# dmlc/xgboost

Hardware: AMD Instinct MI355X
Metric: boosting_rounds_per_sec (higher is better)
Workload: dtype fp32; 1 GPU; model=higgs-1m-hist, rows_per_gpu=1000000, n_features=28, max_depth=8, max_bin=256, objective=binary:logistic, parallelism=dp1, device=cuda

## Files before the change

xgboost_amd/backend/gpu.py:

```python
from __future__ import annotations

from typing import List, Optional, Sequence, Tuple

import numpy as np
import torch

from .. import collective
from ..data import QuantizedMatrix
from ..params import TrainParam
from ..splits import SplitEntry, feature_set_mask
from .cpu import GradQuantizer

LDS_MAX_GROUP_BINS = 8192
TARGET_HIST_TASKS = 2048
MIN_ROWS_PER_TASK = 1024
HIST_MAX_GROUP_FEATURES = 1024


def _check_bin_dtype(gidx: torch.Tensor) -> None:
    if gidx.dtype not in (torch.uint8, torch.int16):
        raise ValueError(
            f"GPU kernels take uint8 or 16-bit bin matrices, got "
            f"{gidx.dtype}: a feature has more than 65535 local bin ids "
            f"(lower max_bin or the category count, or train on the CPU)")
# ... 172 lines not shown
                   out: Optional[torch.Tensor] = None) -> torch.Tensor:
        k = len(segments)
        if out is not None:
            assert out.is_contiguous()
            out.zero_()
            return self._build_hist_into(qgpair, ridx, segments, out)
        out = torch.zeros((k, self.n_bins, 2), dtype=torch.int64,
                          device=self.device)
        return self._build_hist_into(qgpair, ridx, segments, out)

    def _build_hist_into(self, qgpair, ridx, segments, out):
        tasks_np = _chunk_tasks(segments, target_tasks=512)
        (tasks,) = self.stager.upload([tasks_np])
        p8, p16 = self._gidx_ptrs()
        self.lib.gbt_hist(
            p8, p16, self.qm.n_features, self.hip.ptr(qgpair),
            self.hip.ptr(ridx), self.hip.ptr(tasks), len(tasks_np),
            self.hip.ptr(out), self.n_bins,
            self.hip.ptr(self.feat_group_start),
            self.hip.ptr(self.bin_group_start), self.n_groups,
            self.max_group_bins, self.hip.ptr(self.cut_ptrs),
            self.use_shared, None, self.hip.stream())
        return out

    def allreduce_hist(self, hist: torch.Tensor) -> torch.Tensor:
        collective.allreduce_sum_(hist)
        return hist

    def _mt_grouping(self, T: int):
        cache = self.__dict__.setdefault("_mt_group_cache", {})
        if T in cache:
            return cache[T]
        budget = LDS_MAX_GROUP_BINS // T
        widths = np.diff(self.qm.cuts.ptrs)
        if int(widths.max()) > budget:
            cache[T] = None
            return None
        groups_f, groups_b, acc = [0], [0], 0
        for f, w in enumerate(widths):
            if acc > 0 and (acc + w > budget or
                            f - groups_f[-1] >= HIST_MAX_GROUP_FEATURES):
                groups_f.append(f)
                groups_b.append(int(self.qm.cuts.ptrs[f]))
                acc = 0
            acc += int(w)
        groups_f.append(len(widths))
        groups_b.append(int(self.qm.cuts.ptrs[-1]))
        dev = self.device
        out = (torch.tensor(groups_f, dtype=torch.int32, device=dev),
               torch.tensor(groups_b, dtype=torch.int32, device=dev),
               len(groups_f) - 1,
               int(np.max(np.diff(groups_b))))
        cache[T] = out
        return out

    def build_hist_nodes_mt(self, qg_mt: torch.Tensor, nids):
        T = int(qg_mt.shape[1])
        if T > 8 or not hasattr(self.lib, "gbt_hist_mt"):
            return None
        grouping = self._mt_grouping(T)
        if grouping is None:
            return None
        fg, bg, n_groups, max_gb = grouping
        segs = [self.segments[n] for n in nids]
        tasks_np = _chunk_tasks(segs, target_tasks=512)
        (tasks,) = self.stager.upload([tasks_np])
        k = len(nids)
        out = torch.zeros((T, k, self.n_bins, 2), dtype=torch.int64,
                          device=self.device)
        p8, p16 = self._gidx_ptrs()
        self.lib.gbt_hist_mt(
            p8, p16, self.qm.n_features, self.hip.ptr(qg_mt), T,
            self.hip.ptr(self.ridx), self.hip.ptr(tasks), len(tasks_np),
            self.hip.ptr(out), self.n_bins, k,
            self.hip.ptr(fg), self.hip.ptr(bg), n_groups, max_gb,
            self.hip.ptr(self.cut_ptrs), self.hip.stream())
        return out

    def evaluate_splits(self, hist: torch.Tensor, quantizer: GradQuantizer,
                        parent_sums: Sequence[Tuple[int, int]],
                        nids: Sequence[int], param: TrainParam,
                        feature_sets=None, monotone=None, cat_mask=None,
                        node_bounds=None) -> List[SplitEntry]:
        k = len(nids)
        f = self.qm.n_features
        dev = self.device
        gain = torch.empty((k, f), dtype=torch.float64, device=dev)
        bins = torch.empty((k, f), dtype=torch.int32, device=dev)
        dirs = torch.empty((k, f), dtype=torch.uint8, device=dev)
        lsum = torch.empty((k, f, 2), dtype=torch.int64, device=dev)
        parents_np = np.asarray(parent_sums, dtype=np.int64).reshape(k, 2)
        mono_np = (np.asarray(monotone, np.int8)
                   if monotone is not None else None)
        bounds_np = (np.ascontiguousarray(node_bounds, np.float64)
                     if node_bounds is not None else None)
        mask_np = feature_set_mask(feature_sets, k, f)
        wide_feats = None
        if cat_mask is not None:
            widths = np.diff(self.qm.cuts.ptrs)
            wm = np.asarray(cat_mask, bool) & (
                widths > param.max_cat_to_onehot)
            if wm.any():
                wide_feats = np.nonzero(wm)[0]
                if mask_np is None:
                    mask_np = np.ones((k, f), dtype=np.uint8)
                mask_np[:, wide_feats] = 0
        parents, mono_t, bounds_t, mask_t = self.stager.upload(
            [parents_np, mono_np, bounds_np, mask_np])
        self.lib.gbt_evaluate_masked(
            self.hip.ptr(hist), k, self.n_bins, f,
            self.hip.ptr(self.cut_ptrs), self.hip.ptr(parents), None,
            quantizer.g_scale, quantizer.h_scale,
            param.reg_lambda, param.reg_alpha, param.max_delta_step,
            param.min_child_weight, self.hip.ptr(mono_t),
            self.hip.ptr(bounds_t), f, self.hip.ptr(mask_t),
            self.hip.ptr(self.cat_feature),
            self.hip.ptr(gain), self.hip.ptr(bins), self.hip.ptr(dirs),
            self.hip.ptr(lsum), None,
            8 if f > 4096 else 0,
            self.hip.stream())
        out_best = torch.empty((k, 6), dtype=torch.int64, device=dev)
        self.lib.gbt_select_best(
            self.hip.ptr(gain), self.hip.ptr(bins), self.hip.ptr(dirs),
            self.hip.ptr(lsum), k, f, self.hip.ptr(out_best), None,
            self.hip.stream())
        host = out_best.cpu().numpy()
        sel_gain = host[:, 0].view(np.float64)
        sel_bin = host[:, 1]
        sel_dir = host[:, 2]
        sel_lsum = host[:, 3:5]
        best_f = host[:, 5]
        cuts = self.qm.cuts
        out = []
        for i, nid in enumerate(nids):
            e = SplitEntry(nid=int(nid), g_scale=quantizer.g_scale,
                           h_scale=quantizer.h_scale)
            if np.isfinite(sel_gain[i]) and sel_bin[i] >= 0:
                fidx = int(best_f[i])
                e.gain = float(sel_gain[i])
                e.feature = fidx
                e.split_bin = int(sel_bin[i])
                e.default_left = bool(sel_dir[i])
                e.left_gq = int(sel_lsum[i, 0])
                e.left_hq = int(sel_lsum[i, 1])
                e.right_gq = int(parent_sums[i][0]) - e.left_gq
                e.right_hq = int(parent_sums[i][1]) - e.left_hq
                e.is_cat = bool(cat_mask is not None and cat_mask[fidx])
                if e.is_cat:
                    e.cat_bits = np.array(
                        [e.split_bin - int(cuts.ptrs[fidx])], dtype=np.int32)
            out.append(e)
        if wide_feats is not None:
            self._host_sorted_cat(out, hist, parents_np, quantizer, param,
                                  wide_feats, feature_sets)
        return out

    def _host_sorted_cat(self, out, hist, parents_np, quantizer, param,
                         wide_feats, feature_sets) -> None:
        from ..splits import calc_gain_given_weight, calc_weight
        cuts = self.qm.cuts
        k = len(out)
        inv_g = 1.0 / quantizer.g_scale
        inv_h = 1.0 / quantizer.h_scale
        pgq_v = parents_np[:, 0].astype(np.int64)
        phq_v = parents_np[:, 1].astype(np.int64)
        pw_v = calc_weight(pgq_v * inv_g, phq_v * inv_h, param)
        pgain_v = calc_gain_given_weight(pgq_v * inv_g, phq_v * inv_h,
                                         pw_v, param)
        allowed = [None] * k
        if feature_sets is not None:
            for i, fs in enumerate(feature_sets):
                if fs is not None:
                    allowed[i] = set(int(x) for x in fs)
        mct = param.max_cat_threshold + 1
        for fi in wide_feats:
            b0, b1 = int(cuts.ptrs[fi]), int(cuts.ptrs[fi + 1])
            w = b1 - b0
            Gc = hist[:, b0:b1, 0]
            Hc = hist[:, b0:b1, 1]
            present = Hc != 0
            ratio = torch.where(
                present,
                (Gc.double() * inv_g) / (Hc.double() * inv_h
                                         + param.reg_lambda),
                torch.full_like(Gc, float("inf"), dtype=torch.float64))
            order = torch.argsort(ratio, dim=1, stable=True)
            Gs = Gc.gather(1, order)
            Hs = Hc.gather(1, order)
            cg_t = torch.cumsum(Gs, 1)
            ch_t = torch.cumsum(Hs, 1)
            npres_t = present.sum(1)
            cg = cg_t.cpu().numpy()
            ch = ch_t.cpu().numpy()
            order_h = order.cpu().numpy()
            npres = npres_t.cpu().numpy()
            featG = cg[:, -1]
            featH = ch[:, -1]
            missG = pgq_v - featG
            missH = phq_v - featH
            pos = np.arange(w)[None, :]
            limit = np.minimum(npres, mct)[:, None]
            pos_ok = pos < limit
            for missing_left in (False, True):
                gl = cg + (missG[:, None] if missing_left else 0)
                hl = ch + (missH[:, None] if missing_left else 0)
                gr = pgq_v[:, None] - gl
                hr = phq_v[:, None] - hl
                glf, hlf = gl * inv_g, hl * inv_h
                grf, hrf = gr * inv_g, hr * inv_h
                wl = calc_weight(glf, hlf, param)
                wr = calc_weight(grf, hrf, param)
                gains = (calc_gain_given_weight(glf, hlf, wl, param)
                         + calc_gain_given_weight(grf, hrf, wr, param)
                         - pgain_v[:, None])
                ok = (pos_ok & (hlf >= param.min_child_weight)
                      & (hrf >= param.min_child_weight)
                      & (hl > 0) & (hr > 0))
                gains = np.where(ok, gains, -np.inf)
                for i, e in enumerate(out):
                    if npres[i] < 2:
                        continue
                    if allowed[i] is not None and int(fi) not in allowed[i]:
                        continue
                    row = gains[i]
                    if not np.isfinite(row).any():
                        continue
                    j = int(np.argmax(row))
                    gv = float(row[j])
                    if gv > e.gain:
                        e.gain = gv
                        e.feature = int(fi)
                        e.split_bin = b0
                        e.default_left = missing_left
                        e.left_gq = int(gl[i, j])
                        e.left_hq = int(hl[i, j])
                        e.right_gq = int(pgq_v[i]) - e.left_gq
                        e.right_hq = int(phq_v[i]) - e.left_hq
                        e.is_cat = True
                        left_set = set(int(c) for c in order_h[i, :j + 1])
                        e.cat_bits = np.array(
                            sorted(c for c in range(w)
                                   if c not in left_set), dtype=np.int32)

    def partition(self, ridx: torch.Tensor,
                  segments: Sequence[Tuple[int, int]],
                  splits: Sequence[SplitEntry]
                  ) -> List[Tuple[Tuple[int, int], Tuple[int, int]]]:
        k = len(segments)
        dev = self.device
        cuts = self.qm.cuts
        feat = np.empty(k, np.int32)
        sbin = np.empty(k, np.int32)
        dleft = np.empty(k, np.uint8)
        counters = np.empty((k, 2), np.int32)
        cat_words: List[np.ndarray] = []
        cat_offsets = np.zeros(k + 1, np.int32)
        any_cat = False
        for i, ((s, e), sp) in enumerate(zip(segments, splits)):
            feat[i] = sp.feature
            dleft[i] = 1 if sp.default_left else 0
            counters[i] = (s, e)
            if sp.is_cat:
                any_cat = True
                sbin[i] = -1
                nw = (int(self.qm.cuts.ptrs[sp.feature + 1]
                          - self.qm.cuts.ptrs[sp.feature]) + 31) // 32
                w = np.zeros(nw, np.uint32)
                for c in sp.cat_bits:
                    w[c >> 5] |= np.uint32(1 << (c & 31))
                cat_words.append(w)
                cat_offsets[i + 1] = cat_offsets[i] + nw
            else:
                sbin[i] = sp.split_bin - int(cuts.ptrs[sp.feature])
                cat_words.append(np.zeros(0, np.uint32))
                cat_offsets[i + 1] = cat_offsets[i]
        tasks_np = _chunk_tasks(segments)
        cat_bits_np = (np.concatenate(cat_words).view(np.int32)
                       if any_cat else None)
        cat_off_np = cat_offsets if any_cat else None
        tasks, feat_t, sbin_t, dleft_t, cnt_t, cat_bits_t, cat_off_t = \
            self.stager.upload([tasks_np, feat, sbin, dleft, counters,
                                cat_bits_np, cat_off_np])
        p8, p16 = self._gidx_ptrs()
        c8, c16, cld = self._gidx_col_args()
        self.lib.gbt_partition(
            p8, p16, self.qm.n_features, c8, c16, cld, self.hip.ptr(ridx),
            self.hip.ptr(self._ridx_out), self.hip.ptr(tasks), len(tasks_np),
            self.hip.ptr(feat_t), self.hip.ptr(sbin_t), self.hip.ptr(dleft_t),
            self.hip.ptr(cat_bits_t), self.hip.ptr(cat_off_t),
            self.hip.ptr(self.n_bins_feat), self.hip.ptr(cnt_t),
            self.hip.stream())
        self.lib.gbt_copy_ranges(
            self.hip.ptr(self._ridx_out), self.hip.ptr(ridx),
            self.hip.ptr(tasks), len(tasks_np), self.hip.stream())
        final = cnt_t.cpu().numpy()
        out = []
        for i, (s, e) in enumerate(segments):
            mid = int(final[i, 0])
            assert mid == int(final[i, 1]), (
                f"partition counters disagree: {final[i]}")
            out.append(((s, mid), (mid, e)))
        return out

    def grow_tree_native(self, qgpair: torch.Tensor, tree, param,
                         quantizer, monotone: Optional[np.ndarray],
                         root_sums: torch.Tensor,
                         feature_mask: Optional[np.ndarray] = None):
        import ctypes
        if not hasattr(self.lib, "gbt_grow_tree"):
            return None
        if param.max_depth <= 0 or param.max_depth > 14:
            return None
        n_rows = qgpair.shape[0]
        max_build = max(1, 1 << max(param.max_depth - 2, 0))
        pool_rows = 2 * max_build
        pool_bytes = pool_rows * self.n_bins * 16
        if pool_bytes > (32 << 30):
            return None
        dev = self.device
        ws = getattr(self, "_native_ws", None)
        if ws is None or ws["pool_rows"] < pool_rows or ws["n"] < n_rows:
            ws = {
                "pool_rows": pool_rows, "n": n_rows,
                "ridx": torch.empty(n_rows, dtype=torch.int32, device=dev),
                "ridx_out": torch.empty(n_rows, dtype=torch.int32,
                                        device=dev),
                "pool_a": torch.empty((pool_rows, self.n_bins, 2),
                                      dtype=torch.int64, device=dev),
                "pool_b": torch.empty((pool_rows, self.n_bins, 2),
                                      dtype=torch.int64, device=dev),
                "eval_gain": torch.empty((pool_rows, self.qm.n_features),
                                         dtype=torch.float64, device=dev),
                "eval_bin": torch.empty((pool_rows, self.qm.n_features),
                                        dtype=torch.int32, device=dev),
                "eval_dir": torch.empty((pool_rows, self.qm.n_features),
                                        dtype=torch.uint8, device=dev),
                "eval_lsum": torch.empty((pool_rows, self.qm.n_features, 2),
                                         dtype=torch.int64, device=dev),
                "eval_best": torch.empty((pool_rows, 6), dtype=torch.int64,
                                         device=dev),
                "pos": torch.zeros(n_rows, dtype=torch.int32, device=dev),
                "hist_tasks_cap": 16384 + max_build + 8,
                "hist_tasks": torch.empty((16384 + max_build + 8, 4),
                                          dtype=torch.int32, device=dev),
                "qg_stage": torch.empty((n_rows, 2), dtype=torch.int32,
                                        device=dev),
                "rs_stage": torch.empty(2, dtype=torch.int64, device=dev),
                "ma_stage": torch.empty(2, dtype=torch.float32,
                                        device=dev),
                "fm_stage": torch.empty(self.qm.n_features,
                                        dtype=torch.uint8, device=dev),
                "driver": self.lib.gbt_driver_create(),
            }
            pool = 2 * max_build
            if pool <= 2048:
                mp = n_rows // 1024 + pool + 2
                wt_bytes = self.lib.gbt_wt_arena_bytes(param.max_depth,
                                                       max_build, mp)
                ws["wt_max_ptasks"] = mp
                ws["wt_ws"] = torch.empty(wt_bytes, dtype=torch.uint8,
                                          device=dev)
            else:
                ws["wt_max_ptasks"] = 0
                ws["wt_ws"] = None
            self._native_ws = ws
        cap = 1 << (param.max_depth + 1)
        host = {name: np.zeros(cap, dt) for name, dt in [
            ("left", np.int32), ("right", np.int32), ("parent", np.int32),
            ("split_index", np.int32), ("split_cond", np.float32),
            ("default_left", np.uint8), ("loss_chg", np.float64),
            ("sum_hess", np.float32), ("base_weight", np.float32)]}
        fmask_ptr = None
        if feature_mask is not None:
            fm = np.ascontiguousarray(feature_mask, np.uint8)
            ws["fm_stage"].copy_(
                torch.from_numpy(fm), non_blocking=True)
            fmask_ptr = self.hip.ptr(ws["fm_stage"])
        mono_dev = mono_host = None
        if monotone is not None:
            m8 = np.ascontiguousarray(monotone, np.int8)
            key = m8.tobytes()
            if getattr(self, "_mono_key", None) != key:
                self._mono_dev_t = torch.from_numpy(m8).to(dev)
                self._mono_host = m8
                self._mono_key = key
            mono_dev = self.hip.ptr(self._mono_dev_t)
            mono_host = self._mono_host.ctypes.data_as(ctypes.c_void_p)
        cuts = self.qm.cuts
        cut_ptrs_host = np.ascontiguousarray(cuts.ptrs, np.int32)
        cut_values_host = np.ascontiguousarray(cuts.values, np.float32)
        cb = None
        if collective.is_distributed():
            regions = [(t.data_ptr(), t.numel() * t.element_size(), t)
                       for t in (ws["pool_a"], ws["pool_b"])]
            if ws["wt_ws"] is not None:
                w = ws["wt_ws"]
                regions.append((w.data_ptr(), w.numel(), w))

            def _allreduce(ptr, n_elems):
                addr = ctypes.addressof(ptr.contents)
                for base, nbytes, t in regions:
                    if base <= addr < base + nbytes:
                        off = addr - base
                        i64 = t.view(torch.uint8).view(-1)[
                            off:off + 8 * n_elems].view(torch.int64)
                        collective.allreduce_sum_(i64)
                        return
                raise RuntimeError("allreduce pointer outside workspaces")

            cb = self.hip.ALLREDUCE_FN(_allreduce)
        p8, p16 = self._gidx_ptrs()
        c8, c16, cld = self._gidx_col_args()
        ma = getattr(quantizer, "maxabs_dev", None)
        out_scales = np.zeros(2, dtype=np.float64)
        gsc = quantizer.g_scale if ma is None else 0.0
        hsc = quantizer.h_scale if ma is None else 0.0
        qg_st = ws["qg_stage"][:n_rows]
        qg_st.copy_(qgpair.view(n_rows, 2))
        ws["rs_stage"].copy_(root_sums.view(-1)[:2])
        if ma is not None:
            ws["ma_stage"].copy_(ma.view(-1)[:2])
        rc = self.lib.gbt_grow_tree(
            ws["driver"], p8, p16, self.qm.n_features, c8, c16, n_rows,
            self.hip.ptr(qg_st),
            self.hip.ptr(self.cut_ptrs),
            cut_values_host.ctypes.data_as(ctypes.c_void_p),
            cut_ptrs_host.ctypes.data_as(ctypes.c_void_p),
            self.hip.ptr(self.n_bins_feat),
            self.hip.ptr(self.feat_group_start),
            self.hip.ptr(self.bin_group_start), self.n_groups,
            self.max_group_bins, self.use_shared, self.n_bins,
            self.hip.ptr(ws["ridx"]), self.hip.ptr(ws["ridx_out"]),
            self.hip.ptr(ws["pool_a"]), self.hip.ptr(ws["pool_b"]),
            self.hip.ptr(ws["eval_gain"]), self.hip.ptr(ws["eval_bin"]),
            self.hip.ptr(ws["eval_dir"]), self.hip.ptr(ws["eval_lsum"]),
            self.hip.ptr(ws["eval_best"]), self.hip.ptr(ws["pos"]),
            max_build,
            self.hip.ptr(ws["hist_tasks"]), ws["hist_tasks_cap"],
            self.hip.ptr(ws["wt_ws"]),
            0 if ws["wt_ws"] is None else ws["wt_ws"].numel(),
            ws["wt_max_ptasks"],
            self.hip.ptr(ws["rs_stage"]),
            self.hip.ptr(ws["ma_stage"]) if ma is not None else None,
            out_scales.ctypes.data_as(ctypes.c_void_p),
            gsc, hsc,
            param.reg_lambda, param.reg_alpha, param.max_delta_step,
            param.min_child_weight, param.gamma, param.eta, param.max_depth,
            mono_dev, mono_host, fmask_ptr, cb,
            *[host[k].ctypes.data_as(ctypes.c_void_p) for k in (
                "left", "right", "parent", "split_index", "split_cond",
                "default_left", "loss_chg", "sum_hess", "base_weight")],
            self.hip.stream())
        if rc in (-9998, -9999):
            return None
        if rc <= 0:
            raise RuntimeError(f"gbt_grow_tree failed: rc={rc}")
        if ma is not None:
            quantizer.g_scale = float(out_scales[0])
            quantizer.h_scale = float(out_scales[1])
        n = rc
        tree._ensure(n)
        tree.n_nodes = n
        tree.left[:n] = host["left"][:n]
        tree.right[:n] = host["right"][:n]
        tree.parent[:n] = host["parent"][:n]
        tree.split_index[:n] = host["split_index"][:n]
        tree.split_cond[:n] = host["split_cond"][:n]
        tree.default_left[:n] = host["default_left"][:n]
        tree.loss_chg[:n] = host["loss_chg"][:n]
        tree._gain64 = host["loss_chg"][:n].copy()
        tree.sum_hess[:n] = host["sum_hess"][:n]
        tree.base_weight[:n] = host["base_weight"][:n]
        return tree, ws["pos"]

    def leaf_partition(self, ridx: torch.Tensor,
                       leaf_segments: Sequence[Tuple[int, int, int]],
                       n_rows: int) -> torch.Tensor:
        pos = torch.zeros(n_rows, dtype=torch.int32, device=self.device)
        if not leaf_segments:
            return pos
        segs = [(s, e) for _, s, e in leaf_segments]
        tasks_np = _chunk_tasks(segs)
        leaf_np = np.asarray([nid for nid, _, _ in leaf_segments], np.int32)
        tasks, leaf_ids = self.stager.upload([tasks_np, leaf_np])
        self.lib.gbt_leaf_partition(
            self.hip.ptr(ridx), self.hip.ptr(tasks), len(tasks_np),
            self.hip.ptr(leaf_ids), self.hip.ptr(pos), self.hip.stream())
        return pos




class _ForestArrays:

    def __init__(self, booster, lo: int, hi: int, device, idxs=None,
                 fold_weights: bool = False):
        if idxs is None:
            idxs = range(lo, hi)
        idxs = list(idxs)
        trees = [booster.trees[i] for i in idxs]
        offs = np.zeros(len(trees) + 1, np.int32)
        for i, t in enumerate(trees):
            offs[i + 1] = offs[i] + t.n_nodes
        total = int(offs[-1])
        left = np.empty(total, np.int32)
        right = np.empty(total, np.int32)
        sidx = np.empty(total, np.int32)
        cond = np.empty(total, np.float32)
        dft = np.empty(total, np.uint8)
        stype = np.empty(total, np.uint8)
        hess = np.empty(total, np.float32)
        cat_off = np.zeros(total + 1, np.int32)
        cat_bits: List[np.ndarray] = []
        pos = 0
        for i, t in enumerate(trees):
            n = t.n_nodes
            o = offs[i]
            left[o:o + n] = t.left[:n]
            right[o:o + n] = t.right[:n]
            sidx[o:o + n] = t.split_index[:n]
            cond[o:o + n] = t.split_cond[:n]
            w = (booster._tw(idxs[i])
                 if fold_weights and hasattr(booster, "_tw") else 1.0)
            if w != 1.0:
                leaf_mask = t.left[:n] == -1
                cond[o:o + n][leaf_mask] *= np.float32(w)
            dft[o:o + n] = t.default_left[:n]
            stype[o:o + n] = t.split_type[:n]
            hess[o:o + n] = t.sum_hess[:n]
            for nid in range(n):
                if t.split_type[nid] == 1 and nid in t.cat_segments:
                    cats = t.cat_segments[nid]
                    nw = (int(cats.max()) >> 5) + 1 if len(cats) else 0
                    w = np.zeros(nw, np.uint32)
                    for c in cats:
                        w[c >> 5] |= np.uint32(1 << (c & 31))
                    cat_bits.append(w)
                    pos += nw
                cat_off[o + nid + 1] = pos
        self.tree_offsets = torch.from_numpy(offs).to(device)
        self.left = torch.from_numpy(left).to(device)
        self.right = torch.from_numpy(right).to(device)
        self.split_index = torch.from_numpy(sidx).to(device)
        self.split_cond = torch.from_numpy(cond).to(device)
        self.default_left = torch.from_numpy(dft).to(device)
        self.split_type = torch.from_numpy(stype).to(device)
        self.sum_hess = torch.from_numpy(hess).to(device)
        self.cat_offsets = torch.from_numpy(cat_off).to(device)
        if cat_bits:
            self.cat_bits = torch.from_numpy(
                np.concatenate(cat_bits).view(np.int32)).to(device)
        else:
            self.cat_bits = torch.zeros(1, dtype=torch.int32, device=device)
        self.tree_group = torch.tensor(
            [booster.tree_info[t] for t in idxs],
            dtype=torch.int32, device=device)
        self.n_trees = len(trees)


def shap_gpu(booster, dmat, lo: int, hi: int, phi: np.ndarray) -> np.ndarray:
    from .. import ops as hip_ops
    from ..shap import _expected_value
    lib = hip_ops.load()
    has_cat = any(
        t.split_type[:t.n_nodes].any() for t in booster.trees[lo:hi]
        if hasattr(t, "split_type"))
    if not has_cat and hasattr(lib, "gbt_shap_paths"):
        return _shap_gpu_paths(booster, dmat, lo, hi, phi)
    if not hasattr(lib, "gbt_shap"):
        raise ImportError("gbt_shap kernel not built")
    max_depth = max((t.max_depth() for t in booster.trees[lo:hi]), default=0)
    n, n_groups, n_cols = phi.shape
    if max_depth > 16 or n_cols > 129:
        raise ShapDeviceLimit(
            "GPU SHAP limits exceeded; falling back to CPU")
    device = booster.device
    fa = _ForestArrays(booster, lo, hi, device)
    dd = dmat.device_data() if hasattr(dmat, 'device_data') else None
    X = dd if dd is not None else torch.from_numpy(dmat.raw_data()).to(device)
    expected = torch.tensor(
        [_expected_value(booster.trees[t]) for t in range(lo, hi)],
        dtype=torch.float64, device=device)
    out = torch.from_numpy(
        np.ascontiguousarray(phi, np.float32)).to(device)
    _launch_shap_dfs(fa, X, n, dmat.num_col(), dmat.missing, expected,
                     n_groups, n_cols, out)
    res = out.cpu().numpy()
    if n_groups == 1:
        return res[:, 0, :]
    return res


class ShapDeviceLimit(ImportError):
    """The forest is outside what the SHAP kernels handle (categorical
    splits past the DFS kernel's caps, a path of more than 16 features,
    no room for one row): the caller runs the exact host recursion.  An
    ImportError so that the dense entry points keep catching it."""


def _launch_shap_dfs(fa: _ForestArrays, X: torch.Tensor, n: int,
                     n_features: int, missing: float,
                     expected: torch.Tensor, n_groups: int, n_cols: int,
                     out: torch.Tensor) -> None:
    from .. import ops as hip_ops
    lib = hip_ops.load()
    missing_is_nan = 1 if np.isnan(missing) else 0
    lib.gbt_shap(
        hip_ops.ptr(X), n, n_features,
        float(0.0 if missing_is_nan else missing), missing_is_nan,
        hip_ops.ptr(fa.tree_offsets), hip_ops.ptr(fa.left),
        hip_ops.ptr(fa.right), hip_ops.ptr(fa.split_index),
        hip_ops.ptr(fa.split_cond), hip_ops.ptr(fa.default_left),
        hip_ops.ptr(fa.split_type), hip_ops.ptr(fa.cat_offsets),
        hip_ops.ptr(fa.cat_bits), hip_ops.ptr(fa.sum_hess),
        hip_ops.ptr(fa.tree_group), fa.n_trees, n_groups, n_cols,
        hip_ops.ptr(expected), hip_ops.ptr(out), hip_ops.stream())


class _PathTable:

    def __init__(self, booster, lo: int, hi: int, device, col_map=None):
        from ..shap_paths import build_path_table
        pp, pg, ef, elo, ehi, emiss, ez, pv, bias = build_path_table(
            booster.trees[lo:hi], booster.tree_info[lo:hi])
        self.max_elems = int(np.diff(pp).max()) if len(pg) else 0
        if self.max_elems > 16:
            raise ShapDeviceLimit("GPU SHAP path length > 16; CPU fallback")
        if col_map is not None:
            ef = col_map[ef].astype(np.int32)
        self.n_paths = len(pg)
        self.bias = bias
        rz = np.where(ez > 0, 1.0 / np.maximum(ez, 1e-300), 0.0)
        self.t = {}
        for name, arr in (("pp", pp), ("pg", pg), ("ef", ef), ("elo", elo),
                          ("ehi", ehi), ("emiss", emiss), ("ez", ez),
                          ("rz", rz), ("pv", pv)):
            self.t[name] = torch.from_numpy(
                np.ascontiguousarray(arr)).to(device)

    def args(self):
        from .. import ops as hip_ops
        t = self.t
        return (hip_ops.ptr(t["pp"]), hip_ops.ptr(t["pg"]),
                hip_ops.ptr(t["ef"]), hip_ops.ptr(t["elo"]),
                hip_ops.ptr(t["ehi"]), hip_ops.ptr(t["emiss"]),
                hip_ops.ptr(t["ez"]), hip_ops.ptr(t["rz"]),
                hip_ops.ptr(t["pv"]), self.n_paths)


def _launch_shap_paths(tab: _PathTable, Xt: torch.Tensor, n: int,
                       n_features: int, missing: float, n_groups: int,
                       n_cols: int, out: torch.Tensor) -> None:
    from .. import ops as hip_ops
    lib = hip_ops.load()
    missing_is_nan = 1 if np.isnan(missing) else 0
    fn = lib.gbt_shap_paths if tab.max_elems <= 8 else lib.gbt_shap_paths16
    fn(hip_ops.ptr(Xt), n, n_features,
       float(0.0 if missing_is_nan else missing), missing_is_nan,
       *tab.args(), n_groups, n_cols, hip_ops.ptr(out), hip_ops.stream())


def _launch_shap_ix(tab: _PathTable, Xt: torch.Tensor, n: int,
                    n_features: int, missing: float, n_groups: int,
                    n_cols: int, out: torch.Tensor) -> None:
    from .. import ops as hip_ops
    lib = hip_ops.load()
    missing_is_nan = 1 if np.isnan(missing) else 0
    lib.gbt_shap_ix(
        hip_ops.ptr(Xt), n, n_features,
        float(0.0 if missing_is_nan else missing), missing_is_nan,
        *tab.args(), n_groups, n_cols, hip_ops.ptr(out), hip_ops.stream())


def _complete_diagonal(cube: torch.Tensor, base: torch.Tensor) -> torch.Tensor:
    ix = cube.permute(3, 0, 1, 2)
    off_sum = ix.sum(dim=-1) - torch.diagonal(ix, dim1=-2, dim2=-1)
    diag = base - off_sum
    res = ix.clone()
    res.diagonal(dim1=-2, dim2=-1).copy_(diag)
    return res


def _shap_gpu_paths(booster, dmat, lo: int, hi: int,
                    phi: np.ndarray) -> np.ndarray:
    n, n_groups, n_cols = phi.shape
    device = booster.device
    tab = _PathTable(booster, lo, hi, device)
    dd = dmat.device_data() if hasattr(dmat, "device_data") else None
    X = dd if dd is not None else torch.from_numpy(dmat.raw_data()).to(device)
    X = X.t().contiguous()
    out = torch.from_numpy(
        np.ascontiguousarray(phi, np.float64)).to(device)
    for grp in range(n_groups):
        out[:, grp, n_cols - 1] += (float(tab.bias[grp])
                                    if grp < len(tab.bias) else 0.0)
    out = out.permute(1, 2, 0).contiguous()
    _launch_shap_paths(tab, X, n, dmat.num_col(), dmat.missing, n_groups,
                       n_cols, out)
    res = out.permute(2, 0, 1).contiguous().cpu().numpy()
    if n_groups == 1:
        return res[:, 0, :]
    return res


def shap_interactions_gpu(booster, dmat, lo: int, hi: int,
                          iteration_range=(0, 0)) -> np.ndarray:
    from .. import ops as hip_ops
    from ..shap import shap_values
    lib = hip_ops.load()
    if not hasattr(lib, "gbt_shap_ix"):
        raise ImportError("gbt_shap_ix kernel not built")
    if _has_categorical(booster, lo, hi):
        raise ShapDeviceLimit("GPU SHAP interactions: categorical fallback")
    n = dmat.num_row()
    f = dmat.num_col()
    n_groups = booster.n_outputs
    C = f + 1
    device = booster.device
    tab = _PathTable(booster, lo, hi, device)
    out_bytes = n * n_groups * C * C * 8
    free, _total = torch.cuda.mem_get_info()
    if out_bytes > free - (2 << 30):
        raise ShapDeviceLimit("GPU SHAP interactions: output exceeds HBM")
    dd = dmat.device_data() if hasattr(dmat, "device_data") else None
    X = dd if dd is not None else torch.from_numpy(dmat.raw_data()).to(device)
    X = X.t().contiguous()
    out = torch.zeros((n_groups, C, C, n), dtype=torch.float64,
                      device=device)
    _launch_shap_ix(tab, X, n, f, dmat.missing, n_groups, C, out)
    base = shap_values(booster, dmat, iteration_range)
    base_t = torch.as_tensor(np.ascontiguousarray(base, np.float64),
                             device=device)
    if n_groups == 1:
        base_t = base_t[:, None, :]
    res = _complete_diagonal(out, base_t).cpu().numpy()
    if n_groups == 1:
        return res[:, 0].astype(np.float32)
    return res.astype(np.float32)


def _has_categorical(booster, lo: int, hi: int) -> bool:
    return any(
        t.split_type[:t.n_nodes].any() for t in booster.trees[lo:hi]
        if hasattr(t, "split_type"))



_SHAP_CSR_CHUNK_ROWS: Optional[int] = None


def _shap_csr_chunk_rows(n: int, bytes_per_row: int) -> int:
# ... 428 lines not shown
```

xgboost_amd/core.py:

```python
from __future__ import annotations

import json
import os
from typing import Any, Dict, List, Optional, Sequence, Tuple

import numpy as np
import torch

from . import collective
from .backend.cpu import CpuOps, GradQuantizer
from .data import DMatrix
from .grower import TreeGrower
from .metrics import create_metric
from .objectives import Objective, create_objective
from .params import (TrainParam, canonicalize, check_unknown,
                     make_train_param)
from .tree_model import RegTree

VERSION = (3, 5, 0)


def _resolve_device(params: Dict[str, Any]) -> torch.device:
    dev = str(params.get("device", "cpu"))
    if "device" not in params and params.get("gpu_id") is not None:
# ... 201 lines not shown
    def _dart_configured(self) -> bool:
        dp = self.dart_params
        return dp["rate_drop"] != 0.0 or dp["one_drop"] or \
            dp["skip_drop"] != 0.0

    def _dart_track(self) -> bool:
        return bool(self.weight_drop) or self._dart_configured()

    def _tw(self, t: int) -> float:
        return self.weight_drop[t] if t < len(self.weight_drop) else 1.0

    def _dart_drop_trees(self) -> List[int]:
        dp = self.dart_params
        self._idx_drop = []
        if not self._dart_configured() or not self.trees:
            return []
        if not self.weight_drop:
            self.weight_drop = [1.0] * len(self.trees)
        elif len(self.weight_drop) < len(self.trees):
            self.weight_drop.extend(
                [1.0] * (len(self.trees) - len(self.weight_drop)))
        rng = self._dart_rng
        if dp["skip_drop"] > 0.0 and rng.uniform() < dp["skip_drop"]:
            return []
        wd = self.weight_drop
        if dp["sample_type"] == "weighted":
            sw = float(sum(wd))
            for i, w in enumerate(wd):
                if rng.uniform() < dp["rate_drop"] * len(wd) * w / sw:
                    self._idx_drop.append(i)
            if dp["one_drop"] and not self._idx_drop and wd:
                p = np.asarray(wd, np.float64)
                self._idx_drop.append(int(rng.choice(len(wd), p=p / p.sum())))
        else:
            for i in range(len(wd)):
                if rng.uniform() < dp["rate_drop"]:
                    self._idx_drop.append(i)
            if dp["one_drop"] and not self._idx_drop and wd:
                self._idx_drop.append(int(rng.randint(len(wd))))
        return list(self._idx_drop)

    def _dart_new_weight(self) -> float:
        if not self._dart_track():
            return 1.0
        k = len(self._idx_drop)
        if k == 0:
            return 1.0
        lr = float(self.tparam.eta)
        if self.dart_params["normalize_type"] == "forest":
            return 1.0 / (1.0 + lr)
        return 1.0 / (k + lr)

    def _dart_commit(self, margin: torch.Tensor, n_new: int) -> None:
        if not self._dart_track():
            return
        n_old = len(self.trees) - n_new
        if len(self.weight_drop) < n_old:
            self.weight_drop.extend([1.0] * (n_old - len(self.weight_drop)))
        k = len(self._idx_drop)
        lr = float(self.tparam.eta)
        if k == 0:
            self.weight_drop.extend([1.0] * n_new)
        else:
            factor = (1.0 / (1.0 + lr)
                      if self.dart_params["normalize_type"] == "forest"
                      else k / (k + lr))
            for i in self._idx_drop:
                self.weight_drop[i] *= factor
            if self._dart_dc is not None:
                margin += (factor - 1.0) * self._dart_dc
            self.weight_drop.extend([self._dart_new_weight()] * n_new)
        self._idx_drop = []
        self._dart_dc = None
        self._forest_dev_cache = {}

    def _predict_tree_subset(self, dmat: DMatrix,
                             idxs: List[int]) -> torch.Tensor:
        n = dmat.num_row()
        out = torch.zeros((n, self.n_outputs), dtype=torch.float32,
                          device=self.device)
        if getattr(dmat, "_sparse_data", None) is not None:
            if self.device.type == "cuda" and len(idxs) > 0:
                from .backend.gpu import predict_margin_csr_gpu
                return predict_margin_csr_gpu(self, dmat, out, 0, 0,
                                              idxs=list(idxs))
            return self._sparse_margin_add(dmat, out, list(idxs))
        from .extmem import ExtMemQuantileDMatrix
        if isinstance(dmat, ExtMemQuantileDMatrix):
            if self.device.type == "cuda":
                from .backend.gpu import (predict_margin_q_gpu,
                                          predict_q_supported)
                if predict_q_supported(dmat):
                    return predict_margin_q_gpu(self, dmat, out, 0, 0,
                                                idxs=list(idxs))
            for pi in range(len(dmat.pages)):
                qm = dmat.page_qm(pi)
                s, e = dmat.page_offsets[pi], dmat.page_offsets[pi + 1]
                gg = qm.global_gidx().cpu().numpy()
                for t in idxs:
                    tree = self.trees[t]
                    pos = tree.predict_leaf_bins(gg, dmat.cuts)
                    if tree.leaf_values is not None:
                        out[s:e] += self._tw(t) * torch.as_tensor(
                            tree.leaf_values[:tree.n_nodes][pos],
                            device=out.device)
                        continue
                    vals = tree.split_cond[:tree.n_nodes][pos] * self._tw(t)
                    out[s:e, self.tree_info[t]] += torch.as_tensor(
                        vals, device=out.device)
            return out
        if self.device.type == "cuda" and not any(
                self.trees[t].leaf_values is not None for t in idxs):
            from .backend.gpu import predict_subset_gpu
            return predict_subset_gpu(self, dmat, idxs, out)
        X = dmat.raw_data()
        for t in idxs:
            tree = self.trees[t]
            pos = tree.predict_leaf_np(X, dmat.missing)
            if tree.leaf_values is not None:
                out += self._tw(t) * torch.as_tensor(
                    tree.leaf_values[:tree.n_nodes][pos],
                    device=out.device)
            else:
                vals = tree.split_cond[:tree.n_nodes][pos] * self._tw(t)
                out[:, self.tree_info[t]] += torch.as_tensor(
                    vals, device=out.device)
        return out

    def update(self, dtrain: DMatrix, iteration: int,
               fobj=None) -> None:
        self._maybe_set_meta(dtrain)
        self._init_base_score(dtrain)
        if self.tparam.process_type == "update":
            self._update_existing(dtrain, iteration)
            return
        margin = self._cached_margin(dtrain)
        from .monitor import TrainingObserver
        if TrainingObserver.enabled():
            TrainingObserver.observe_predictions(iteration, margin)
        use_margin = margin
        if self.booster_kind != "gblinear" and self._dart_configured():
            dropped = self._dart_drop_trees()
            if dropped:
                self._dart_dc = self._predict_tree_subset(dtrain, dropped)
                use_margin = margin - self._dart_dc
        elif fobj is None and self._boost_fused(dtrain, margin, iteration):
            if TrainingObserver.enabled():
                TrainingObserver.observe_tree(iteration, self.trees[-1])
            return
        if fobj is not None:
            preds = use_margin.detach().cpu().numpy()
            from .objective import Objective as _ClsObj, TreeObjective
            if isinstance(fobj, TreeObjective):
                vgrad, vhess = fobj(iteration, preds, dtrain)
                sg = fobj.split_grad(iteration, vgrad, vhess)
                if sg is not None:
                    self._boost_split_grad(dtrain, sg[0], sg[1], vgrad,
                                           vhess, iteration)
                    return
                grad, hess = vgrad, vhess
            elif isinstance(fobj, _ClsObj):
                grad, hess = fobj(iteration, preds, dtrain)
            else:
                grad, hess = fobj(np.squeeze(preds), dtrain)
            grad = torch.as_tensor(np.asarray(grad, np.float32),
                                   device=margin.device).view(margin.shape)
            hess = torch.as_tensor(np.asarray(hess, np.float32),
                                   device=margin.device).view(margin.shape)
        else:
            grad, hess = self.objective.get_gradient(use_margin, dtrain.info,
                                                     iteration)
            TrainingObserver.observe_gradient(iteration, grad, hess)
        self.boost_gpair(dtrain, grad, hess, iteration)

    def boost(self, dtrain: DMatrix, iteration: int = 0, grad=None, hess=None) -> None:
        self._maybe_set_meta(dtrain)
        if self.base_score is None:
            self.base_score = 0.5
            self._base_score_estimated = True
        dev = self.device
        g = torch.as_tensor(np.asarray(grad, np.float32), device=dev)
        h = torch.as_tensor(np.asarray(hess, np.float32), device=dev)
        n = dtrain.num_row()
        g = g.view(n, -1)
        h = h.view(n, -1)
        self.boost_gpair(dtrain, g, h, iteration)

    def boost_gpair(self, dtrain: DMatrix, grad: torch.Tensor,
                    hess: torch.Tensor, iteration: int) -> None:
        if self.booster_kind == "gblinear":
            self._boost_linear(dtrain, grad, hess, iteration)
            return
        from .data import QuantileDMatrix as _QDM
        if self.tparam.tree_method in ("exact", "approx") and \
                type(dtrain) is _QDM:
            raise ValueError(
                f"tree_method={self.tparam.tree_method} does not support "
                "QuantileDMatrix; use hist or a plain DMatrix")
        if self.tparam.tree_method == "exact":
            if str(self.raw_params.get(
                    "multi_strategy", "one_output_per_tree")) ==                     "multi_output_tree" and                     (grad.dim() > 1 and grad.shape[1] > 1):
                raise ValueError(
                    "Only the hist tree method is supported for building "
                    "multi-target trees with vector leaf.")
            self._boost_exact(dtrain, grad, hess, iteration)
            return
        ops = self._ops_for(dtrain)
        n = dtrain.num_row()
        n_out = grad.shape[1] if grad.dim() > 1 else 1
        grad = grad.view(n, n_out)
        hess = hess.view(n, n_out)
        margin, version = self._cache[id(dtrain)]
        seed = (self.seed + iteration if not self.seed_per_iteration
                else self.seed + iteration * 2654435761)
        new_trees = 0
        eta_scale = 1.0 / max(1, self.tparam.num_parallel_tree)
        multi_strategy = str(self.raw_params.get("multi_strategy",
                                                 "one_output_per_tree"))
        if multi_strategy == "multi_output_tree" and n_out > 1:
            if self.tparam.tree_method not in ("auto", "hist"):
                raise ValueError(
                    "Only the hist tree method is supported for building "
                    "multi-target trees with vector leaf.")
            self._boost_multi_target(dtrain, ops, grad, hess, margin, seed)
            return
        is_approx = self.tparam.tree_method == "approx"
        w_new = self._dart_new_weight()
        for k in range(n_out):
            if is_approx:
                ops = self._ops_for(
                    dtrain, hess=hess[:, k].detach())
            for ptree in range(self.tparam.num_parallel_tree):
                gpair = torch.stack([grad[:, k], hess[:, k]], dim=1).contiguous()
                gpair = self._subsample(gpair, seed + 7919 * ptree + 104729 * k)
                gpair = gpair.to(ops.device)
                quantizer = GradQuantizer(gpair)
                qg = quantizer.quantize(gpair)
                tree = RegTree(self.n_features)
                grower = TreeGrower(
                    ops, self._scaled_param(eta_scale), quantizer, n,
                    seed=seed + 31 * ptree + 17 * k,
                    monotone=self._monotone_array(),
                    interaction=self.tparam.interaction_constraints,
                    feature_weights=dtrain.info.feature_weights)
                tree, positions = grower.grow(qg, tree)
                self.trees.append(tree)
                self.tree_info.append(k)
                new_trees += 1
                leaf_np = tree.split_cond[:tree.n_nodes].copy()
                if hasattr(ops, "stager"):
                    (leaf_vals,) = ops.stager.upload([leaf_np])
                else:
                    leaf_vals = torch.as_tensor(leaf_np, device=margin.device)
                add = leaf_vals[positions.to(margin.device).long()]
                margin[:, k] += add if w_new == 1.0 else w_new * add
        self._dart_commit(margin, new_trees)
        self.iteration_indptr.append(self.iteration_indptr[-1] + new_trees)
        self._cache[id(dtrain)] = (margin, len(self.trees))
        from .monitor import TrainingObserver
        if TrainingObserver.enabled() and self.trees:
            TrainingObserver.observe_tree(iteration, self.trees[-1])
        if self.tparam.debug_synchronize:
            collective.check_synchronized(
                json.dumps(self.trees[-1].to_json()).encode(), "tree")

    def _boost_fused(self, dtrain: DMatrix, margin: torch.Tensor,
                     iteration: int) -> bool:
        if self.device.type != "cuda":
            return False
        obj_id = {"binary:logistic": 0, "reg:squarederror": 1}.get(
            self.objective.name)
        if obj_id is None or self.n_outputs != 1:
            return False
        tp = self.tparam
        if (tp.subsample < 1.0 or tp.num_parallel_tree != 1
                or tp.tree_method not in ("auto", "hist")
                or self.booster_kind == "gblinear"
                or tp.process_type == "update"
                or str(self.raw_params.get("multi_strategy",
                                           "one_output_per_tree"))
                != "one_output_per_tree"):
            return False
        from . import ops as hip_ops
        try:
            lib = hip_ops.load()
        except RuntimeError:
            return False
        if not hasattr(lib, "gbt_gpair_fused"):
            return False
        ops = self._ops_for(dtrain)
        n = dtrain.num_row()
        key = self._pin(dtrain)
        fc = self.__dict__.setdefault("_fused_cache", {})
        ent = fc.get(key)
        if ent is None:
            dev = self.device
            labels = torch.as_tensor(
                np.ascontiguousarray(dtrain.get_label(), np.float32),
                device=dev)
            w = dtrain.info.weights
            weights = (torch.as_tensor(np.ascontiguousarray(w, np.float32),
                                       device=dev) if w is not None else None)
            ent = {"labels": labels, "weights": weights,
                   "gh": torch.empty((n, 2), dtype=torch.float32, device=dev),
                   "qg": torch.empty((n, 2), dtype=torch.int32, device=dev),
                   "maxabs": torch.zeros(2, dtype=torch.float32, device=dev)}
            fc[key] = ent
        ent["maxabs"].zero_()
        spw = float(self.raw_params.get("scale_pos_weight", 1.0))
        lib.gbt_gpair_fused(
            obj_id, hip_ops.ptr(margin.contiguous().view(-1)),
            hip_ops.ptr(ent["labels"]), hip_ops.ptr(ent["weights"]),
            spw, n, hip_ops.ptr(ent["gh"]), hip_ops.ptr(ent["maxabs"]),
            hip_ops.stream())
        m = ent["maxabs"]
        if collective.is_distributed():
            collective.allreduce_max_(m)
        quantizer = GradQuantizer.__new__(GradQuantizer)
        quantizer.g_scale = None
        quantizer.h_scale = None
        quantizer.maxabs_dev = m
        if "rootsum" not in ent:
            ent["rootsum"] = torch.zeros(2, dtype=torch.int64,
                                         device=margin.device)
        else:
            ent["rootsum"].zero_()
        lib.gbt_quantize(hip_ops.ptr(ent["gh"]), n, 0.0, 0.0,
                         hip_ops.ptr(m), hip_ops.ptr(ent["qg"]),
                         hip_ops.ptr(ent["rootsum"]), hip_ops.stream())
        if collective.is_distributed():
            collective.allreduce_sum_(ent["rootsum"])
        quantizer.root_sums_dev = ent["rootsum"]
        seed = (self.seed + iteration if not self.seed_per_iteration
                else self.seed + iteration * 2654435761)
        tree = RegTree(self.n_features)
        grower = TreeGrower(ops, self.tparam, quantizer, n, seed=seed,
                            monotone=self._monotone_array(),
                            interaction=tp.interaction_constraints,
                            feature_weights=dtrain.info.feature_weights)
        tree, positions = grower.grow(ent["qg"], tree)
        self.trees.append(tree)
        self.tree_info.append(0)
        self.iteration_indptr.append(self.iteration_indptr[-1] + 1)
        leaf_np = tree.split_cond[:tree.n_nodes].copy()
        if hasattr(ops, "stager") and hasattr(lib, "gbt_margin_add") \
                and positions.device == margin.device:
            (leaf_vals,) = ops.stager.upload([leaf_np])
            mc = margin.contiguous()
            lib.gbt_margin_add(hip_ops.ptr(mc), hip_ops.ptr(positions),
                               hip_ops.ptr(leaf_vals), n,
                               mc.stride(0), 0, hip_ops.stream())
            if mc.data_ptr() != margin.data_ptr():
                margin.copy_(mc)
        else:
            leaf_vals = torch.as_tensor(leaf_np, device=margin.device)
            margin[:, 0] += leaf_vals[positions.to(margin.device).long()]
        self._cache[key] = (margin, len(self.trees))
        if self.tparam.debug_synchronize:
            collective.check_synchronized(
                json.dumps(self.trees[-1].to_json()).encode(), "tree")
        return True

    def _boost_linear(self, dtrain: DMatrix, grad: torch.Tensor,
                      hess: torch.Tensor, iteration: int) -> None:
        from .linear import GBLinearModel
        ft = dtrain.feature_types or []
        if any(t in ("c", "categorical") for t in ft) or \
                getattr(dtrain, "categories_", None):
            raise ValueError("`gblinear` does not support categorical data")
        if self._linear is None:
            self._linear = GBLinearModel(self.n_features, self.n_outputs,
                                         self.raw_params, self.device)
        X = torch.as_tensor(dtrain.raw_data(), device=self.device)
        siw = float(np.sum(dtrain.get_weight()))
        self._linear.update(X, grad, hess, iteration, siw)
        margin = self._linear.predict_margin(X) + self._base_margin_value()
        self.iteration_indptr.append(self.iteration_indptr[-1])
        self._cache[id(dtrain)] = (margin, len(self.trees))

    def _boost_multi_target(self, dtrain: DMatrix, ops, grad, hess,
                            margin, seed: int) -> None:
        from .grower import MultiTargetGrower
        n, n_out = grad.shape
        qgpairs, quantizers = [], []
        for k in range(n_out):
            gp = torch.stack([grad[:, k], hess[:, k]], dim=1).contiguous()
            gp = gp.to(ops.device)
            q = GradQuantizer(gp)
            quantizers.append(q)
            qgpairs.append(q.quantize(gp))
        tree = RegTree(self.n_features, n_out)
        grower = MultiTargetGrower(
            ops, self.tparam, quantizers, n, seed,
            feature_weights=dtrain.info.feature_weights)
        tree, positions = grower.grow(qgpairs, tree)
        self.trees.append(tree)
        self.tree_info.append(0)
        self.iteration_indptr.append(self.iteration_indptr[-1] + 1)
        leaf_vals = torch.as_tensor(
            tree.leaf_values[:tree.n_nodes].copy(), device=margin.device)
        w_new = self._dart_new_weight()
        add = leaf_vals[positions.to(margin.device).long()]
        margin += add if w_new == 1.0 else w_new * add
        self._dart_commit(margin, 1)
        self._cache[id(dtrain)] = (margin, len(self.trees))

    def _boost_split_grad(self, dtrain: DMatrix, sgrad, shess, vgrad,
                          vhess, iteration: int) -> None:
        dev = self.device
        n = dtrain.num_row()

        def t2(a):
            return torch.as_tensor(np.asarray(a, np.float32),
                                   device=dev).view(n, -1)

        sg, sh = t2(sgrad), t2(shess)
        vg, vh = t2(vgrad), t2(vhess)
        if vg.shape[1] < 2:
            raise ValueError(
                "split_grad requires vector-leaf trees: configure the "
                "booster with num_target matching the full gradient "
                "width (reference gbtree.cc:192)")
        if vg.shape[1] != self.n_outputs:
            raise ValueError(
                f"value gradient width {vg.shape[1]} != model outputs "
                f"{self.n_outputs}")
        if self.tparam.monotone_constraints:
            raise ValueError("monotone constraints are not supported "
                             "with reduced gradients (gbtree.cc:194)")
        margin, _ = self._cache[id(dtrain)]
        ops = self._ops_for(dtrain)
        seed = self.seed + iteration
        if sg.shape[1] == 1:
            gpair = torch.stack([sg[:, 0], sh[:, 0]],
                                dim=1).contiguous().to(ops.device)
            quant = GradQuantizer(gpair)
            qg = quant.quantize(gpair)
            tree = RegTree(self.n_features)
            grower = TreeGrower(ops, self.tparam, quant, n, seed=seed,
                                feature_weights=dtrain.info.feature_weights)
            tree, positions = grower.grow(qg, tree)
        else:
            from .grower import MultiTargetGrower
            qgpairs, quantizers = [], []
            for k in range(sg.shape[1]):
                gp = torch.stack([sg[:, k], sh[:, k]],
                                 dim=1).contiguous().to(ops.device)
                q = GradQuantizer(gp)
                quantizers.append(q)
                qgpairs.append(q.quantize(gp))
            tree = RegTree(self.n_features, sg.shape[1])
            grower = MultiTargetGrower(
                ops, self.tparam, quantizers, n, seed,
                feature_weights=dtrain.info.feature_weights)
            tree, positions = grower.grow(qgpairs, tree)
        C = vg.shape[1]
        nn = tree.n_nodes
        pos = positions.to(dev).long()
        ps, pperm = torch.sort(pos)
        bnd = torch.searchsorted(ps, torch.arange(nn + 1, device=dev))
        Gv = torch.zeros((nn, C), dtype=torch.float64, device=dev)
        Hv = torch.zeros((nn, C), dtype=torch.float64, device=dev)
        cs = torch.zeros(n + 1, dtype=torch.float64, device=dev)
        for c in range(C):
            torch.cumsum(vg[:, c].double()[pperm], 0, out=cs[1:])
            Gv[:, c] = cs[bnd[1:]] - cs[bnd[:-1]]
            torch.cumsum(vh[:, c].double()[pperm], 0, out=cs[1:])
            Hv[:, c] = cs[bnd[1:]] - cs[bnd[:-1]]
        lam = self.tparam.reg_lambda
        alpha = self.tparam.reg_alpha
        w = -torch.sign(Gv) * torch.clamp(Gv.abs() - alpha, min=0.0) \
            / (Hv + lam)
        mds = self.tparam.max_delta_step
        if mds > 0:
            w = w.clamp(-mds, mds)
        w = (w * self.tparam.eta).float()
        leaf_mask = torch.as_tensor(tree.left[:nn] == -1, device=dev)
        w = torch.where(leaf_mask[:, None], w, torch.zeros_like(w))
        lv = np.zeros((len(tree.split_cond), C), dtype=np.float32)
        lv[:nn] = w.cpu().numpy()
        tree.n_targets = C
        tree.leaf_values = lv
        self.trees.append(tree)
        self.tree_info.append(0)
        self.iteration_indptr.append(self.iteration_indptr[-1] + 1)
        w_new = self._dart_new_weight()
        add = torch.as_tensor(lv[:nn], device=margin.device)[pos]
        margin += add if w_new == 1.0 else w_new * add
        self._dart_commit(margin, 1)
        self._cache[id(dtrain)] = (margin, len(self.trees))

    def _update_existing(self, dtrain: DMatrix, iteration: int) -> None:
        from .updaters import prune_tree, refresh_tree
        if iteration >= self.num_boosted_rounds():
            raise ValueError(
                "process_type=update requires an existing model with at "
                f"least {iteration + 1} boosted rounds")
        updater_seq = (self.tparam.updater or "refresh").split(",")
        margin = self._cached_margin(dtrain)
        grad, hess = self.objective.get_gradient(margin, dtrain.info,
                                                 iteration)
        lo, hi = (self.iteration_indptr[iteration],
                  self.iteration_indptr[iteration + 1])
        X = dtrain.raw_data()
        for t in range(lo, hi):
            k = self.tree_info[t]
            gpair = torch.stack([grad[:, k], hess[:, k]],
                                dim=1).cpu().numpy()
            for upd in updater_seq:
                upd = upd.strip()
                if upd == "prune":
                    self.trees[t] = prune_tree(self.trees[t], self.tparam)
                elif upd == "refresh":
                    refresh_tree(self.trees[t], X, gpair, self.tparam,
                                 dtrain.missing,
                                 refresh_leaf=self.tparam.refresh_leaf)
                else:
                    raise ValueError(
                        f"unsupported updater for process_type=update: {upd}")
        self._cache.clear()

    def _boost_exact(self, dtrain: DMatrix, grad: torch.Tensor,
                     hess: torch.Tensor, iteration: int) -> None:
        from .exact import grow_exact
        if self.device.type == "cuda":
            raise ValueError("tree_method=exact is CPU-only; use hist on GPU")
        ft = dtrain.feature_types or []
        if any(t in ("c", "categorical") for t in ft) or \
                getattr(dtrain, "categories_", None):
            raise ValueError(
                "Updater `grow_colmaker` or `exact` tree method does not"
                " support categorical data")
        from .extmem import ExtMemQuantileDMatrix
        if isinstance(dtrain, ExtMemQuantileDMatrix):
            raise ValueError(
                "Updater `grow_colmaker` or `exact` tree method doesn't "
                "support external memory training")
        if self.tparam.colsample_bynode != 1.0:
            raise ValueError("column sample by node is not yet supported "
                             "by the exact tree method")
        n = dtrain.num_row()
        n_out = grad.shape[1]
        margin, _ = self._cache[id(dtrain)]
        seed = self.seed + iteration
        cache = self.__dict__.setdefault("_exact_cache", {}).setdefault(
            id(dtrain), {})
        new_trees = 0
        w_new = self._dart_new_weight()
        for k in range(n_out):
            for ptree in range(self.tparam.num_parallel_tree):
                gpair = torch.stack([grad[:, k], hess[:, k]], dim=1)
                gpair = self._subsample(gpair, seed + 7919 * ptree + 11 * k)
                tree = RegTree(self.n_features)
                positions = grow_exact(dtrain.raw_data(),
                                       gpair.cpu().numpy(),
                                       self._scaled_param(
                                           1.0 / max(1, self.tparam.num_parallel_tree)),
                                       tree, dtrain.missing, cache)
                self.trees.append(tree)
                self.tree_info.append(k)
                new_trees += 1
                leaf_vals = torch.as_tensor(
                    tree.split_cond[:tree.n_nodes].copy(), device=margin.device)
                pos_t = torch.as_tensor(positions.astype(np.int64),
                                        device=margin.device)
                add = leaf_vals[pos_t]
                margin[:, k] += add if w_new == 1.0 else w_new * add
        self._dart_commit(margin, new_trees)
        self.iteration_indptr.append(self.iteration_indptr[-1] + new_trees)
        self._cache[id(dtrain)] = (margin, len(self.trees))

    def _scaled_param(self, eta_scale: float) -> TrainParam:
        if eta_scale == 1.0:
            return self.tparam
        import dataclasses as dc
        p = dc.replace(self.tparam)
        p.eta = self.tparam.eta * eta_scale
        return p

    def _monotone_array(self) -> Optional[np.ndarray]:
        mc = self.tparam.monotone_constraints
        if mc is None:
            return None
        if isinstance(mc, str):
            mc = [int(x) for x in mc.strip("()[] ").split(",") if x.strip()]
        arr = np.zeros(self.n_features, dtype=np.int64)
        arr[:len(mc)] = np.asarray(list(mc), dtype=np.int64)[:self.n_features]
        return arr

    def _subsample(self, gpair: torch.Tensor, seed: int) -> torch.Tensor:
        p = self.tparam.subsample
        if p >= 1.0:
            return gpair
        gen = torch.Generator(device="cpu").manual_seed(seed & 0x7FFFFFFF)
        if self.tparam.sampling_method == "gradient_based":
            g = gpair[:, 0].cpu()
            h = gpair[:, 1].cpu()
            score = torch.sqrt(g * g + self.tparam.reg_lambda * h * h)
            n = g.numel()
            threshold = _sample_rate_threshold(score, p)
            u = torch.rand(n, generator=gen)
            keep_prob = torch.clamp(score / threshold, max=1.0)
            keep = u < keep_prob
            out = gpair.clone()
            scale = (1.0 / keep_prob.clamp(min=1e-16)).to(gpair.device)
            out[:, 0] = torch.where(keep.to(gpair.device),
                                    gpair[:, 0] * scale, torch.zeros_like(gpair[:, 0]))
            out[:, 1] = torch.where(keep.to(gpair.device),
                                    gpair[:, 1] * scale, torch.zeros_like(gpair[:, 1]))
            return out
        mask = (torch.rand(gpair.shape[0], generator=gen) < p).to(gpair.device)
        out = gpair.clone()
        out[~mask] = 0.0
        return out

    def _cached_margin(self, dmat: DMatrix) -> torch.Tensor:
        key = self._pin(dmat)
        n = dmat.num_row()
        entry = self._cache.get(key)
        if entry is not None and entry[1] == len(self.trees):
            return entry[0]
        margin = self._predict_margin(dmat)
        self._cache[key] = (margin, len(self.trees))
        return margin

    def _predict_margin(self, dmat: DMatrix,
                        iteration_range: Tuple[int, int] = (0, 0)
                        ) -> torch.Tensor:
        n = dmat.num_row()
        out = torch.full((n, self.n_outputs), self._base_margin_value(),
                         dtype=torch.float32, device=self.device)
        if dmat.info.base_margin is not None:
            bm = torch.as_tensor(dmat.info.base_margin, dtype=torch.float32,
                                 device=self.device)
            out = bm.view(n, -1).expand(n, self.n_outputs).clone()
        if self.booster_kind == "gblinear":
            if self._linear is not None:
                X = torch.as_tensor(dmat.raw_data(), device=self.device)
                out = out + self._linear.predict_margin(X)
            return out
        lo, hi = self._tree_range(iteration_range)
        from .extmem import ExtMemQuantileDMatrix
        if isinstance(dmat, ExtMemQuantileDMatrix):
# ... 688 lines not shown
```

xgboost_amd/grower.py:

```python
from __future__ import annotations

import dataclasses
import heapq
from typing import Dict, List, Optional, Sequence, Tuple

import numpy as np
import torch

from .backend.cpu import GradQuantizer
from .params import TrainParam
from .splits import SplitEntry, calc_weight, feature_set_mask
from .tree_model import RegTree


class ColumnSampler:

    def __init__(self, n_features: int, param: TrainParam, seed: int,
                 feature_weights: Optional[np.ndarray] = None):
        self.rng = np.random.RandomState(seed & 0x7FFFFFFF)
        self.n_features = n_features
        self.param = param
        self.weights = (np.asarray(feature_weights, dtype=np.float64)
                        if feature_weights is not None else None)
        feats = np.arange(n_features)
        if param.colsample_bytree < 1.0:
            k = max(1, int(round(param.colsample_bytree * n_features)))
            feats = self._sample(feats, k)
        self.tree_set = feats
        self._level_cache: Dict[int, np.ndarray] = {}

    def _sample(self, feats: np.ndarray, k: int) -> np.ndarray:
        if self.weights is None:
            return np.sort(self.rng.choice(feats, size=k, replace=False))
        w = self.weights[feats]
        pos = w > 0
        feats, w = feats[pos], w[pos]
        if feats.size == 0:
            raise ValueError("all sampled feature_weights are zero")
        k = min(k, feats.size)
        keys = self.rng.random_sample(feats.size) ** (1.0 / w)
        return np.sort(feats[np.argsort(-keys)[:k]])

    def level_set(self, depth: int) -> np.ndarray:
        if self.param.colsample_bylevel >= 1.0:
            return self.tree_set
        if depth not in self._level_cache:
            k = max(1, int(round(self.param.colsample_bylevel * len(self.tree_set))))
            self._level_cache[depth] = self._sample(self.tree_set, k)
        return self._level_cache[depth]

    def node_set(self, depth: int) -> Optional[np.ndarray]:
        base = self.level_set(depth)
        if self.param.colsample_bynode >= 1.0:
            if (self.param.colsample_bytree >= 1.0
                    and self.param.colsample_bylevel >= 1.0):
                return None
            return base
        k = max(1, int(round(self.param.colsample_bynode * len(base))))
        return self._sample(base, k)


class InteractionConstraints:

    def __init__(self, spec: Sequence[Sequence[int]], n_features: int):
        self.sets = [frozenset(int(f) for f in s) for s in spec]
        self.n_features = n_features
        self.node_path: Dict[int, frozenset] = {0: frozenset()}

    def split(self, nid: int, left: int, right: int, feature: int) -> None:
        path = self.node_path.get(nid, frozenset()) | {int(feature)}
        self.node_path[left] = path
        self.node_path[right] = path

    def allowed(self, nid: int) -> Optional[np.ndarray]:
        path = self.node_path.get(nid, frozenset())
        if not path:
            return None
        allowed = set(path)
        for s in self.sets:
            if path <= s:
                allowed |= s
        return np.array(sorted(allowed), dtype=np.int64)


@dataclasses.dataclass(order=True)
class _QueueEntry:
    sort_key: float
    seq: int
    nid: int = dataclasses.field(compare=False)
    depth: int = dataclasses.field(compare=False)
    split: SplitEntry = dataclasses.field(compare=False)


class TreeGrower:

    def __init__(self, ops, param: TrainParam, quantizer: GradQuantizer,
                 n_rows: int, seed: int = 0,
                 monotone: Optional[np.ndarray] = None,
                 interaction: Optional[Sequence[Sequence[int]]] = None,
                 feature_weights: Optional[np.ndarray] = None):
        self.ops = ops
        self.param = param
        self.quantizer = quantizer
        self.n_rows = n_rows
        self.col_sampler = ColumnSampler(ops.qm.n_features, param, seed,
                                         feature_weights)
        self.monotone = monotone
        self.interaction = (InteractionConstraints(interaction, ops.qm.n_features)
                            if interaction else None)
        cuts = ops.qm.cuts
        if cuts.feature_types is not None:
            self.cat_mask = np.array([t == "c" for t in cuts.feature_types])
            if not self.cat_mask.any():
                self.cat_mask = None
        else:
            self.cat_mask = None

    _monitor = None

    @classmethod
    def monitor(cls):
        if cls._monitor is None:
            from .monitor import Monitor
            cls._monitor = Monitor("TreeGrower")
        return cls._monitor

    def grow(self, qgpair: torch.Tensor, tree: RegTree
             ) -> Tuple[RegTree, torch.Tensor]:
        mon = self.monitor()
        mon.start("grow")
        try:
            native = self._try_native(qgpair, tree)
            if native is not None:
                return native
            return self._grow(qgpair, tree)
        finally:
            mon.stop("grow")

    def _try_native(self, qgpair, tree):
        p = self.param
        ops = self.ops
        if not hasattr(ops, "grow_tree_native"):
            return None
        if (self.cat_mask is not None or self.interaction is not None
                or p.colsample_bylevel < 1.0 or p.colsample_bynode < 1.0):
            return None
        fmask = None
        if p.colsample_bytree < 1.0:
            fmask = np.zeros(ops.qm.n_features, np.uint8)
            fmask[self.col_sampler.tree_set] = 1
        needs_replay = p.grow_policy == "lossguide" or p.max_leaves > 0
        if needs_replay:
            if p.max_depth <= 0 or p.max_depth > 14:
                return None
            if p.max_leaves > 0 and (1 << p.max_depth) > 16 * p.max_leaves:
                return None
        rs = getattr(self.quantizer, "root_sums_dev", None)
        if rs is None:
            from . import collective
            rs = qgpair.to(torch.int64).sum(dim=0).contiguous()
            if collective.is_distributed():
                collective.allreduce_sum_(rs)
        out = ops.grow_tree_native(qgpair, tree, p, self.quantizer,
                                   self.monotone, rs, feature_mask=fmask)
        if out is None or not needs_replay:
            return out
        dtree, pos = out
        return self._policy_replay(dtree, pos, p)

    def _policy_replay(self, dt: RegTree, pos: torch.Tensor,
                       param) -> Tuple[RegTree, torch.Tensor]:
        import heapq
        n = dt.n_nodes
        internal = dt.left[:n] >= 0
        gains = getattr(dt, "_gain64", None)
        if gains is None:
            gains = dt.loss_chg[:n].astype(np.float64)
        nt = RegTree(dt.n_features)
        nt._ensure(n)
        new_of = np.full(n, -1, np.int32)
        new_of[0] = 0
        nt.base_weight[0] = dt.base_weight[0]
        nt.sum_hess[0] = dt.sum_hess[0]
        nt.left[0] = nt.right[0] = nt.parent[0] = -1
        state = {"n_new": 1, "n_leaves": 1, "seq": 0}
        heap: List[Tuple[float, int, int, int]] = []

        def push(dnid: int, depth: int) -> None:
            if not internal[dnid]:
                return
            if param.max_depth > 0 and depth >= param.max_depth:
                return
            if param.max_leaves > 0 and state["n_leaves"] >= param.max_leaves:
                return
            key = (float(depth) if param.grow_policy == "depthwise"
                   else -float(gains[dnid]))
            heapq.heappush(heap, (key, state["seq"], dnid, depth))
            state["seq"] += 1

        push(0, 0)
        while heap:
            batch = [heapq.heappop(heap)]
            if param.grow_policy == "depthwise":
                while heap and heap[0][0] == batch[0][0]:
                    batch.append(heapq.heappop(heap))
            if param.max_leaves > 0:
                batch = batch[:max(0, param.max_leaves - state["n_leaves"])]
            if not batch:
                continue
            for _key, _sq, dnid, _depth in batch:
                nn = int(new_of[dnid])
                l, r = state["n_new"], state["n_new"] + 1
                state["n_new"] += 2
                dl, dr = int(dt.left[dnid]), int(dt.right[dnid])
                new_of[dl], new_of[dr] = l, r
                nt.left[nn], nt.right[nn] = l, r
                nt.parent[l] = nt.parent[r] = nn
                nt.split_index[nn] = dt.split_index[dnid]
                nt.split_cond[nn] = dt.split_cond[dnid]
                nt.default_left[nn] = dt.default_left[dnid]
                nt.loss_chg[nn] = dt.loss_chg[dnid]
                nt.sum_hess[nn] = dt.sum_hess[dnid]
                for c_new, c_d in ((l, dl), (r, dr)):
                    nt.base_weight[c_new] = dt.base_weight[c_d]
                    nt.sum_hess[c_new] = dt.sum_hess[c_d]
                    nt.left[c_new] = nt.right[c_new] = -1
                state["n_leaves"] += 1
            for _key, _sq, dnid, depth in batch:
                push(int(dt.left[dnid]), depth + 1)
                push(int(dt.right[dnid]), depth + 1)
        nt.n_nodes = state["n_new"]
        for i in range(nt.n_nodes):
            if nt.left[i] == -1:
                nt.split_cond[i] = np.float32(
                    float(nt.base_weight[i]) * param.eta)
        lut = np.zeros(n, np.int32)
        stack = [(0, -1)]
        while stack:
            dnid, cover = stack.pop()
            if cover < 0:
                nn = int(new_of[dnid])
                if nn >= 0 and nt.left[nn] == -1:
                    cover = nn
            lut[dnid] = cover if cover >= 0 else 0
            if internal[dnid]:
                stack.append((int(dt.left[dnid]), cover))
                stack.append((int(dt.right[dnid]), cover))
        lut_t = torch.from_numpy(lut).to(pos.device)
        return nt, lut_t[pos.long()].to(torch.int32)

    def _grow(self, qgpair: torch.Tensor, tree: RegTree
              ) -> Tuple[RegTree, torch.Tensor]:
        param = self.param
        ops = self.ops
        if getattr(self.quantizer, "g_scale", 1.0) is None:
            ma = self.quantizer.maxabs_dev.cpu()
            mg, mh = float(ma[0]), float(ma[1])
            self.quantizer.g_scale = (1 << 30) / mg if mg > 0 else 1.0
            self.quantizer.h_scale = (1 << 30) / mh if mh > 0 else 1.0
        ops.reset(self.n_rows)
        node_sums: Dict[int, Tuple[int, int]] = {}
        node_bounds: Dict[int, Tuple[float, float]] = {0: (-np.inf, np.inf)}
        hists: Dict[int, torch.Tensor] = {}

        qg, qh = ops.root_sum(qgpair)
        root_g = qg / self.quantizer.g_scale
        root_h = qh / self.quantizer.h_scale
        node_sums[0] = (qg, qh)
        root_w = float(calc_weight(root_g, root_h, param))
        tree.base_weight[0] = root_w
        tree.sum_hess[0] = root_h
        hist = ops.build_hist_nodes(qgpair, [0])
        ops.allreduce_hist(hist)
        hists[0] = hist[0]
        root_entry = self._evaluate([0], node_sums, hists, node_bounds, depth=0)[0]

        n_leaves = 1
        seq = 0
        heap: List[_QueueEntry] = []

        def push(nid, depth, split):
            nonlocal seq
            if not self._expandable(split, depth, n_leaves):
                return
            key = (float(depth) if param.grow_policy == "depthwise"
                   else -split.gain)
            heapq.heappush(heap, _QueueEntry(key, seq, nid, depth, split))
            seq += 1

        push(0, 0, root_entry)

        while heap:
            batch = [heapq.heappop(heap)]
            if param.grow_policy == "depthwise":
                while heap and heap[0].sort_key == batch[0].sort_key:
                    batch.append(heapq.heappop(heap))
            batch = [b for b in batch
                     if self._expandable(b.split, b.depth, n_leaves + 0)]
            if param.max_leaves > 0:
                keep = []
                for b in batch:
                    if n_leaves + len(keep) + 1 <= param.max_leaves:
                        keep.append(b)
                batch = keep
            if not batch:
                continue

            children = []
            for b in batch:
                sp = b.split
                cuts = ops.qm.cuts
                if sp.is_cat:
                    cond = np.nan
                    cats_right = sp.cat_bits
                else:
                    cond = float(cuts.values[sp.split_bin])
                    cats_right = None
                wl = float(calc_weight(sp.left_g, sp.left_h, param))
                wr = float(calc_weight(sp.right_g, sp.right_h, param))
                lo, hi = node_bounds.get(b.nid, (-np.inf, np.inf))
                wl, wr = self._clip_bounds(wl, wr, lo, hi)
                l, r = tree.add_split(
                    b.nid, sp.feature, cond, sp.default_left, sp.gain,
                    float(tree.base_weight[b.nid]), wl, wr,
                    sp.left_h + sp.right_h, sp.left_h, sp.right_h,
                    categories_go_right=cats_right)
                node_sums[l] = (sp.left_gq, sp.left_hq)
                node_sums[r] = (sp.right_gq, sp.right_hq)
                self._propagate_bounds(node_bounds, b.nid, l, r, sp, wl, wr)
                if self.interaction is not None:
                    self.interaction.split(b.nid, l, r, sp.feature)
                children.append((b, l, r))
                n_leaves += 1

            parents = [b.nid for b, _, _ in children]
            splits = [b.split for b, _, _ in children]
            child_pairs = [(l, r) for _, l, r in children]
            ops.partition_nodes(parents, splits, child_pairs)

            build_nodes = []
            for (b, l, r) in children:
                expand_more = (b.depth + 1 < (param.max_depth or 10 ** 9)
                               or param.grow_policy == "lossguide")
                if not expand_more and param.max_depth > 0:
                    continue
                if node_sums[l][1] <= node_sums[r][1]:
                    build_nodes.append((l, b.nid, r))
                else:
                    build_nodes.append((r, b.nid, l))
            if build_nodes:
                kb = len(build_nodes)
                stack = (ops.alloc_hist(2 * kb)
                         if hasattr(ops, "alloc_hist") else None)
                bnids = [n for n, _, _ in build_nodes]
                if stack is None:
                    bh = ops.build_hist_nodes(qgpair, bnids)
                else:
                    bh = ops.build_hist_nodes(qgpair, bnids,
                                              out=stack[:kb])
                ops.allreduce_hist(bh)
                parent_stack = torch.stack(
                    [hists[p] for _, p, _ in build_nodes])
                if stack is None:
                    sib_stack = parent_stack - bh
                    hist_stack = torch.cat([bh, sib_stack], dim=0)
                else:
                    torch.sub(parent_stack, bh, out=stack[kb:])
                    sib_stack = stack[kb:]
                    hist_stack = stack
                for i, (n, parent, sib) in enumerate(build_nodes):
                    hists[n] = bh[i]
                    hists[sib] = sib_stack[i]
                    del hists[parent]
                eval_nids = ([n for n, _, _ in build_nodes]
                             + [s for _, _, s in build_nodes])
                depth = children[0][0].depth + 1
                entries = self._evaluate(eval_nids, node_sums, hists,
                                         node_bounds, depth,
                                         hist_stack=hist_stack)
                entry_of = dict(zip(eval_nids, entries))
                for (b, l, r) in children:
                    if l in entry_of:
                        push(l, depth, entry_of[l])
                    if r in entry_of:
                        push(r, depth, entry_of[r])

        leaf_nids = []
        for nid in range(tree.n_nodes):
            if tree.is_leaf(nid):
                w = float(tree.base_weight[nid])
                tree.set_leaf(nid, w * param.eta)
                leaf_nids.append(nid)
        positions = ops.leaf_positions(leaf_nids)
        return tree, positions

    def _expandable(self, split: SplitEntry, depth: int, n_leaves: int) -> bool:
        param = self.param
        if not split.is_valid or split.gain < param.gamma:
            return False
        if param.max_depth > 0 and depth >= param.max_depth:
            return False
        if param.max_leaves > 0 and n_leaves >= param.max_leaves:
            return False
        return True

    def _evaluate(self, nids, node_sums, hists, node_bounds, depth,
                  hist_stack: Optional[torch.Tensor] = None
                  ) -> List[SplitEntry]:
        param = self.param
        hist = (hist_stack if hist_stack is not None
                else torch.stack([hists[n] for n in nids]))
        parent_sums = [node_sums[n] for n in nids]
        feature_sets = None
        node_feats = self.col_sampler.node_set(depth)
        inter_sets = ([self.interaction.allowed(n) for n in nids]
                      if self.interaction is not None else None)
        if node_feats is not None or inter_sets is not None:
            feature_sets = []
            for i, n in enumerate(nids):
                fs = node_feats
                if self.param.colsample_bynode < 1.0:
                    fs = self.col_sampler.node_set(depth)
                if inter_sets is not None and inter_sets[i] is not None:
                    fs = (np.intersect1d(fs, inter_sets[i]) if fs is not None
                          else inter_sets[i])
                feature_sets.append(fs)
        bounds = (np.array([node_bounds.get(n, (-np.inf, np.inf)) for n in nids])
                  if self.monotone is not None else None)
        return self.ops.evaluate_splits(
            hist, self.quantizer,
            [(g, h) for g, h in parent_sums], nids, param,
            feature_sets=feature_sets, monotone=self.monotone,
            cat_mask=self.cat_mask, node_bounds=bounds)

    def _clip_bounds(self, wl, wr, lo, hi):
        return float(np.clip(wl, lo, hi)), float(np.clip(wr, lo, hi))

    def _propagate_bounds(self, node_bounds, nid, l, r, sp, wl, wr) -> None:
        lo, hi = node_bounds.get(nid, (-np.inf, np.inf))
        node_bounds[l] = (lo, hi)
        node_bounds[r] = (lo, hi)
        if self.monotone is None:
            return
        c = int(self.monotone[sp.feature]) if sp.feature < len(self.monotone) else 0
        if c == 0:
            return
        mid = (wl + wr) / 2.0
        if c > 0:
            node_bounds[l] = (lo, min(hi, mid))
            node_bounds[r] = (max(lo, mid), hi)
        else:
            node_bounds[l] = (max(lo, mid), hi)
            node_bounds[r] = (lo, min(hi, mid))


class MultiTargetGrower:

    def __init__(self, ops, param: TrainParam, quantizers, n_rows: int,
                 seed: int = 0,
                 feature_weights: Optional[np.ndarray] = None):
        self.ops = ops
        self.param = param
        self.quantizers = quantizers
        self.n_rows = n_rows
        self.col_sampler = ColumnSampler(ops.qm.n_features, param, seed,
                                         feature_weights)

# ... 205 lines not shown
```

xgboost_amd/ops/__init__.py:

```python
from __future__ import annotations

import ctypes
import os
from typing import Optional

import torch

_HERE = os.path.dirname(os.path.abspath(__file__))
_LIB_PATH = os.path.join(_HERE, "libgbt_hip.so")
_lib: Optional[ctypes.CDLL] = None

_c = ctypes
_p = _c.c_void_p
_i = _c.c_int
_i64 = _c.c_int64
_f = _c.c_float
_d = _c.c_double

_SIGS = {
    "gbt_hist": [_p, _p, _i, _p, _p, _p, _i, _p, _i, _p, _p, _i, _i, _p, _i, _p, _p],
    "gbt_partition": [_p, _p, _i, _p, _p, _i64, _p, _p, _p, _i, _p, _p, _p,
                      _p, _p, _p, _p, _p],
    "gbt_evaluate_masked": [_p, _i, _i, _i, _p, _p, _p, _d, _d, _d, _d, _d,
                            _d, _p, _p, _i, _p, _p, _p, _p, _p, _p, _p, _i,
                            _p],
    "gbt_evaluate_ref": [_p, _i, _i, _i, _p, _p, _p, _d, _d, _d, _d, _d,
                         _d, _p, _p, _i, _p, _p, _p, _p, _p, _p, _p, _i,
                         _p],
    "gbt_compress": [_p, _i64, _i, _p, _p, _p, _f, _i, _p, _p, _p],
    "gbt_predict": [_p, _i64, _i, _f, _i, _p, _p, _p, _p, _p, _p, _p, _p,
                    _p, _p, _i, _i, _p, _p, _p],
    "gbt_predict_q": [_p, _i, _i64, _i, _f, _i, _p, _p, _p, _p, _p, _p, _p,
                      _p, _i, _i, _p, _p, _p],
    "gbt_predict_csr": [_p, _p, _p, _i64, _i, _p, _p, _p, _p, _p, _p, _p,
                        _i, _i, _p, _p, _i, _i, _p],
    "gbt_leaf_partition": [_p, _p, _i, _p, _p, _p],
    "gbt_leaf_decide": [_p, _p, _i, _p, _p, _i64, _p, _p, _i, _p, _p, _p,
                        _p, _p, _p, _p],
    "gbt_copy_ranges": [_p, _p, _p, _i, _p],
    "gbt_select_best": [_p, _p, _p, _p, _i, _i, _p, _p, _p],
    "gbt_mt_evaluate": [_p, _i, _i, _i, _i, _p, _p, _p, _p,
                        _d, _d, _d, _d, _p, _p, _p, _p, _p],
    "gbt_gpair_fused": [_i, _p, _p, _p, _f, _i64, _p, _p, _p],
    "gbt_quantize": [_p, _i64, _d, _d, _p, _p, _p, _p],
    "gbt_margin_add": [_p, _p, _p, _i64, _i, _i, _p],
    "gbt_hist_cpu": [_p, _p, _i, _p, _p, _p, _p, _i, _p, _p, _i],
    "gbt_partition_cpu": [_p, _p, _i, _p, _i64, _i64, _i, _i, _i, _p, _i,
                          _i, _p],
    "gbt_evaluate_cpu": [_p, _i, _i, _i, _p, _p, _d, _d, _d, _d, _d, _d,
                         _p, _p, _p, _p],
    "gbt_hist_csr": [_p, _p, _p, _p, _p, _i, _p, _i, _p],
    "gbt_partition_csr": [_p, _p, _p, _p, _p, _i, _p, _p, _p, _p, _p, _p],
    "gbt_driver_create": [],
    "gbt_driver_destroy": [_p],
    "gbt_root_tasks_check": [_i64, _i64, _i64, _p],
    "gbt_wt_arena_bytes": [_i, _i, _i],
    "gbt_grow_tree": [
        _p,
        _p, _p, _i,
        _p, _p,
        _i64, _p,
        _p, _p, _p, _p,
        _p, _p, _i, _i, _i, _i,
        _p, _p, _p, _p,
        _p, _p, _p, _p, _p, _p,
        _i,
        _p, _i,
        _p, _i64, _i,
        _p,
        _p, _p,
        _d, _d,
        _d, _d, _d, _d, _d, _d,
        _i,
        _p, _p,
        _p,
        _p,
        _p, _p, _p, _p, _p, _p, _p, _p, _p,
        _p,
    ],
    "gbt_shap": [_p, _i64, _i, _f, _i, _p, _p, _p, _p, _p, _p, _p, _p, _p,
                 _p, _p, _i, _i, _i, _p, _p, _p],
    "gbt_shap_paths": [_p, _i64, _i, _f, _i, _p, _p, _p, _p, _p, _p,
                       _p, _p, _p, _i64, _i, _i, _p, _p],
    "gbt_shap_paths16": [_p, _i64, _i, _f, _i, _p, _p, _p, _p, _p, _p,
                         _p, _p, _p, _i64, _i, _i, _p, _p],
    "gbt_shap_ix": [_p, _i64, _i, _f, _i, _p, _p, _p, _p, _p, _p, _p, _p,
                    _p, _i64, _i, _i, _p, _p],
    "gbt_csr_gather_columns": [_p, _p, _p, _i64, _i64, _p, _i, _i, _p, _p],
    "gbt_hist_mt": [_p, _p, _i, _p, _i, _p, _p, _i, _p, _i, _i,
                    _p, _p, _i, _i, _p, _p],
}


def load() -> ctypes.CDLL:
    global _lib
    if _lib is not None:
        return _lib
    if not os.path.exists(_LIB_PATH):
        try:
            from .build_ext import build
            build()
        except Exception as e:
            raise RuntimeError(
                f"HIP kernel library missing and build failed: {e}. "
                f"Run `python {os.path.join(_HERE, 'build_ext.py')}`."
            ) from e
    _lib = ctypes.CDLL(_LIB_PATH)
    for name, argtypes in _SIGS.items():
        try:
            fn = getattr(_lib, name)
        except AttributeError:
            continue
        fn.argtypes = argtypes
        fn.restype = None
    if hasattr(_lib, "gbt_driver_create"):
        _lib.gbt_driver_create.restype = _p
        _lib.gbt_grow_tree.restype = _c.c_int
    if hasattr(_lib, "gbt_root_tasks_check"):
        _lib.gbt_root_tasks_check.restype = _c.c_int
    if hasattr(_lib, "gbt_wt_arena_bytes"):
        _lib.gbt_wt_arena_bytes.restype = _c.c_longlong
    if hasattr(_lib, "gbt_partition_cpu"):
        _lib.gbt_partition_cpu.restype = _c.c_longlong
    return _lib


ALLREDUCE_FN = _c.CFUNCTYPE(None, _c.POINTER(_c.c_longlong), _c.c_longlong)


def available() -> bool:
    try:
        load()
        return True
    except RuntimeError:
        return False


def ptr(t: Optional[torch.Tensor]):
    if t is None:
        return None
    assert t.is_contiguous(), "kernel arg tensors must be contiguous"
    return _c.c_void_p(t.data_ptr())


def stream() -> _c.c_void_p:
    return _c.c_void_p(torch.cuda.current_stream().cuda_stream)
```

xgboost_amd/ops/cpp/driver.hip:

```cpp
#include "gbt_kernels.h"

#include <hip/hip_runtime.h>

#include <algorithm>
#include <cmath>
#include <cstdio>
#include <cstdlib>
#include <cstring>
#include <vector>

namespace {

#define HIP_CHECK(x)                                    \
  do {                                                  \
    hipError_t err__ = (x);                             \
    if (err__ != hipSuccess) return -(int)err__;        \
  } while (0)

constexpr int kErrReplayDiverged = -9991;
constexpr int kErrRootTasksCap = -9996;
constexpr int kErrArenaTooSmall = -9997;
constexpr int kCapacityTaskGenLds = -9998;
constexpr int kCapacityHistPool = -9999;

bool WtGraphDebug() {
  static int v = [] {
    const char* e = getenv("GBT_WT_GRAPH_DEBUG");
    return e ? atoi(e) : 0;
  }();
  return v != 0;
}

struct PinnedRing {
  static constexpr int kSlots = 6;
  void* host[kSlots] = {};
  void* dev[kSlots] = {};
  size_t cap[kSlots] = {};
  int cur = 0;

  int ensure(int slot, size_t bytes) {
    if (cap[slot] >= bytes) return 0;
    size_t want = 4096;
    while (want < bytes) want <<= 1;
    if (host[slot]) hipHostFree(host[slot]);
    if (dev[slot]) hipFree(dev[slot]);
    HIP_CHECK(hipHostMalloc(&host[slot], want));
    HIP_CHECK(hipMalloc(&dev[slot], want));
    cap[slot] = want;
    return 0;
  }
  int next() {
    int s = cur;
    cur = (cur + 1) % kSlots;
    return s;
  }
};

typedef std::vector<unsigned long long> GraphKey;

struct DriverCtx {
  PinnedRing ring;
  void* readback_host = nullptr;
  size_t readback_cap = 0;

  hipGraphExec_t wt_graph = nullptr;
  GraphKey wt_key;
  GraphKey wt_seen_key;
  hipStream_t gstream = nullptr;
  hipEvent_t gevent = nullptr;

  int ensure_gstream() {
    if (gstream == nullptr)
      HIP_CHECK(hipStreamCreateWithFlags(&gstream, hipStreamNonBlocking));
    if (gevent == nullptr)
      HIP_CHECK(hipEventCreateWithFlags(&gevent, hipEventDisableTiming));
    return 0;
  }

  int wait_for(hipStream_t caller) {
    HIP_CHECK(hipEventRecord(gevent, caller));
    HIP_CHECK(hipEventSynchronize(gevent));
    return 0;
  }

  void drop_graph() {
    if (wt_graph) (void)hipGraphExecDestroy(wt_graph);
    wt_graph = nullptr;
    wt_key.clear();
  }

  bool try_replay(const GraphKey& key) {
    if (wt_graph == nullptr || key != wt_key) return false;
    if (hipGraphLaunch(wt_graph, gstream) == hipSuccess) {
      if (WtGraphDebug()) fprintf(stderr, "[wtgraph] replay\n");
      return true;
    }
    (void)hipGetLastError();
    drop_graph();
    return false;
  }

  template <typename Enqueue>
  int capture_and_launch(const GraphKey& key, Enqueue&& enqueue,
                         bool* launched) {
    *launched = false;
    if (key != wt_seen_key) {
      wt_seen_key = key;
    } else if (hipStreamBeginCapture(gstream, hipStreamCaptureModeRelaxed) !=
               hipSuccess) {
      (void)hipGetLastError();
    } else {
      int ec = enqueue(gstream);
      hipGraph_t g = nullptr;
      hipError_t ce = hipStreamEndCapture(gstream, &g);
      if (WtGraphDebug())
        fprintf(stderr, "[wtgraph] capture ec=%d end=%d\n", ec, (int)ce);
      if (ec != 0) {
        if (g) (void)hipGraphDestroy(g);
        return ec;
      }
      if (ce == hipSuccess && g != nullptr) {
        drop_graph();
        hipError_t ie = hipGraphInstantiate(&wt_graph, g, nullptr, nullptr, 0);
        hipError_t le = ie == hipSuccess ? hipGraphLaunch(wt_graph, gstream)
                                         : hipErrorUnknown;
        if (WtGraphDebug())
          fprintf(stderr, "[wtgraph] inst=%d launch=%d\n", (int)ie, (int)le);
        if (ie == hipSuccess && le == hipSuccess) {
          wt_key = key;
          *launched = true;
        } else {
          drop_graph();
        }
        (void)hipGraphDestroy(g);
      } else {
        (void)hipGetLastError();
      }
    }
    if (!*launched) {
      hipStreamCaptureStatus st = hipStreamCaptureStatusNone;
      if (hipStreamIsCapturing(gstream, &st) == hipSuccess &&
          st != hipStreamCaptureStatusNone) {
        hipGraph_t junk = nullptr;
        (void)hipStreamEndCapture(gstream, &junk);
        if (junk) (void)hipGraphDestroy(junk);
      }
    }
    return 0;
  }

  int ensure_readback(size_t bytes) {
    if (readback_cap >= bytes) return 0;
    size_t want = 4096;
    while (want < bytes) want <<= 1;
    if (readback_host) hipHostFree(readback_host);
    HIP_CHECK(hipHostMalloc(&readback_host, want));
    readback_cap = want;
    return 0;
  }
  ~DriverCtx() {
    for (int i = 0; i < PinnedRing::kSlots; ++i) {
      if (ring.host[i]) hipHostFree(ring.host[i]);
      if (ring.dev[i]) hipFree(ring.dev[i]);
    }
    if (readback_host) hipHostFree(readback_host);
    if (wt_graph) (void)hipGraphExecDestroy(wt_graph);
    if (gstream) (void)hipStreamDestroy(gstream);
    if (gevent) (void)hipEventDestroy(gevent);
  }
};

bool WtGraphEnabled() {
  static int v = [] {
    const char* e = getenv("GBT_WT_GRAPH");
    return e ? atoi(e) : 1;
  }();
  return v != 0;
}

constexpr long long kHistMinRows = 2048;
long long HistTasksTarget() {
  static long long v = [] {
    const char* e = getenv("GBT_HIST_TASKS");
    long long t = e ? atoll(e) : 256;
    return t >= 64 && t <= 16384 ? t : 256;
  }();
  return v;
}

long long PartMinRows() {
  static long long v = [] {
    const char* e = getenv("GBT_PART_ROWS");
    long long r = e ? atoll(e) : 4096;
    return r >= 1024 && r <= 65536 && (r & (r - 1)) == 0 ? r : 4096;
  }();
  return v;
}

struct Node {
  int nid;
  int seg_begin, seg_end;
  long long gq, hq;
  int hist_slot;
  double lo, hi;
  double gain;
  int bin, dir, feature;
  long long lgq, lhq;
};

__host__ __device__ inline double CalcWeight(double g, double h, double lam,
                                             double alpha, double mds) {
  double t = g;
  if (alpha != 0.0) {
    double s = (g > 0.0) ? 1.0 : ((g < 0.0) ? -1.0 : 0.0);
    double m = fabs(g) - alpha;
    if (m < 0.0) m = 0.0;
    t = s * m;
  }
  double w = -t / (h + lam);
  if (mds > 0.0) w = fmin(fmax(w, -mds), mds);
  return w;
}

__host__ __device__ inline double ScaleFromMaxAbs(float maxabs) {
  return maxabs > 0.f ? 1073741824.0 / (double)maxabs : 1.0;
}

bool ShouldExpand(double gain, double gamma) {
  return gain > 0.0 && gain >= gamma && std::isfinite(gain);
}
__device__ inline bool DevShouldExpand(long long bin, double gain,
                                       double gamma) {
  return bin >= 0 && isfinite(gain) && gain > 0.0 && gain >= gamma;
}

void DecodeBest(const int64_t rec[6], Node* nd) {
  double gain;
  memcpy(&gain, &rec[0], sizeof(double));
  nd->bin = (int)rec[1];
  nd->dir = (int)rec[2];
  nd->lgq = rec[3];
  nd->lhq = rec[4];
  nd->feature = (int)rec[5];
  nd->gain = (nd->bin >= 0 && std::isfinite(gain)) ? gain : -INFINITY;
}

void ChunkTasks(const std::vector<Node*>& nodes, std::vector<BlockTask>* out,
                long long min_rows = 1024, long long target_tasks = 2048) {
  out->clear();
  long long total = 0;
  for (auto* n : nodes) total += n->seg_end - n->seg_begin;
  long long rows_per_task =
      std::max<long long>(min_rows, (total + target_tasks - 1) / target_tasks);
  for (size_t i = 0; i < nodes.size(); ++i) {
    int b = nodes[i]->seg_begin;
    while (b < nodes[i]->seg_end) {
      int e = (int)std::min<long long>(b + rows_per_task, nodes[i]->seg_end);
      out->push_back(BlockTask{(int)i, b, e, 0});
      b = e;
    }
  }
  if (out->empty()) out->push_back(BlockTask{0, 0, 0, 0});
}

__global__ void ZeroI64Kernel(int64_t* p, long long n) {
  long long i = (long long)blockIdx.x * blockDim.x + threadIdx.x;
  long long stride = (long long)gridDim.x * blockDim.x;
  for (; i < n; i += stride) p[i] = 0;
}

__global__ void IotaKernel(int32_t* r, long long n) {
  long long i = (long long)blockIdx.x * blockDim.x + threadIdx.x;
  for (; i < n; i += (long long)gridDim.x * blockDim.x) r[i] = (int)i;
}

long long RootRowsPerTask(long long n_rows, long long min_rows,
                          long long target_tasks) {
  return std::max<long long>(min_rows,
                             (n_rows + target_tasks - 1) / target_tasks);
}
int RootTaskCount(long long n_rows, long long rpt) {
  return (int)std::max<long long>(1, (n_rows + rpt - 1) / rpt);
}

__global__ void WtInitKernel(int32_t* r, long long n, int64_t* zero,
                             long long zero_n, int32_t* kn, int32_t* kp,
                             int32_t* seg, BlockTask* root_tasks,
                             int n_root_tasks, long long rpt,
                             const int64_t* __restrict__ root_sums,
                             const float* __restrict__ maxabs,
                             int64_t* rs_out ) {
  const long long stride = (long long)gridDim.x * blockDim.x;
  const long long i0 = (long long)blockIdx.x * blockDim.x + threadIdx.x;
  for (long long i = i0; i < n; i += stride) r[i] = (int)i;
  for (long long i = i0; i < zero_n; i += stride) zero[i] = 0;
  if (blockIdx.x != 0) return;
  if (threadIdx.x == 0) {
    kn[0] = 1;
    kp[0] = 0;
    seg[0] = 0;
    seg[1] = (int)n;
    rs_out[0] = root_sums[0];
    rs_out[1] = root_sums[1];
    float* ma = (float*)(rs_out + 2);
    ma[0] = maxabs[0];
    ma[1] = maxabs[1];
  }
  for (int t = threadIdx.x; t < n_root_tasks; t += blockDim.x) {
    const long long b = (long long)t * rpt;
    root_tasks[t] =
        BlockTask{0, (int)b, (int)std::min<long long>(b + rpt, n), 0};
  }
}

__global__ void SubtractHistKernel(const int64_t* __restrict__ parents,
                                   const int64_t* __restrict__ built,
                                   int64_t* __restrict__ out,
                                   const int32_t* __restrict__ parent_slot,
                                   int n_bins2, int k,
                                   int64_t* __restrict__ ps,
                                   const int64_t* __restrict__ parent_ps,
                                   const int32_t* __restrict__ kp_dev) {
  if (kp_dev != nullptr) {
    k = *kp_dev;
    out += (long long)k * n_bins2;
  }
  const long long idx = (long long)blockIdx.x * blockDim.x + threadIdx.x;
  if (ps != nullptr && idx < k) {
    ps[2 * (k + idx)] = parent_ps[2 * idx] - ps[2 * idx];
    ps[2 * (k + idx) + 1] = parent_ps[2 * idx + 1] - ps[2 * idx + 1];
  }
  const long long total = (long long)k * n_bins2;
  for (long long i = idx; i < total; i += (long long)gridDim.x * blockDim.x) {
    const int row = (int)(i / n_bins2);
    const int col = (int)(i % n_bins2);
    out[(long long)row * n_bins2 + col] =
        parents[(long long)parent_slot[row] * n_bins2 + col] -
        built[(long long)row * n_bins2 + col];
  }
}

constexpr int kMaxSplitNodes = 2048;

__device__ inline void SplitSegmentsIntoTasks(
    const int* s_begin, const int* s_end, int k, long long min_rows,
    long long target_tasks, int max_tasks, BlockTask* __restrict__ out_tasks) {
  __shared__ int s_pref[kMaxSplitNodes];
  __shared__ long long s_rpt;
  __shared__ int s_total_tasks;
  __syncthreads();
  if (threadIdx.x == 0) {
    long long total = 0;
    for (int j = 0; j < k; ++j) total += s_end[j] - s_begin[j];
    long long rpt0 =
        std::max(min_rows, (total + target_tasks - 1) / target_tasks);
    int shift = 0;
    while ((1LL << shift) < rpt0) ++shift;
    for (;;) {
      long long need = 0;
      for (int j = 0; j < k; ++j) {
        const long long sz = s_end[j] - s_begin[j];
        need += (sz + (1LL << shift) - 1) >> shift;
      }
      if (need <= max_tasks) break;
      ++shift;
    }
    const long long rpt = 1LL << shift;
    int pref = 0;
    for (int j = 0; j < k; ++j) {
      s_pref[j] = pref;
      const long long sz = s_end[j] - s_begin[j];
      pref += (int)((sz + rpt - 1) >> shift);
    }
    s_rpt = rpt;
    s_total_tasks = pref;
  }
  __syncthreads();
  const long long rpt = s_rpt;
  const int total_tasks = s_total_tasks;
  for (int t = threadIdx.x; t < max_tasks; t += blockDim.x) {
    if (t >= total_tasks) {
      out_tasks[t] = BlockTask{0, 0, 0, 0};
      continue;
    }
    int lo = 0, hi = k - 1;
    while (lo < hi) {
      const int mid = (lo + hi + 1) >> 1;
      if (s_pref[mid] <= t) lo = mid; else hi = mid - 1;
    }
    const int j = lo;
    const long long idx = t - s_pref[j];
    const int b = s_begin[j] + (int)(idx * rpt);
    const int e = (int)std::min<long long>((long long)b + rpt,
                                           (long long)s_end[j]);
    out_tasks[t] = BlockTask{j, b, e, 0};
  }
}

__global__ void HistTaskGenKernel(const int32_t* __restrict__ counters,
                                  const int32_t* __restrict__ desc, int k,
                                  long long min_rows, long long target_tasks,
                                  int max_tasks,
                                  BlockTask* __restrict__ out_tasks,
                                  int64_t* __restrict__ ps ,
                                  const int32_t* __restrict__ kp_dev,
                                  int32_t* __restrict__ seg_out,
                                  int zero_n,
                                  uint8_t* __restrict__ mode_out
                                  ) {
  if (kp_dev != nullptr) k = *kp_dev;
  if (ps != nullptr) {
    const int zn = max(4 * k, zero_n);
    for (int i = threadIdx.x; i < zn; i += blockDim.x) ps[i] = 0;
  }
  __shared__ int s_begin[kMaxSplitNodes], s_end[kMaxSplitNodes];
  for (int j = threadIdx.x; j < k; j += blockDim.x) {
    const int pb = desc[4 * j], pe = desc[4 * j + 1];
    const int split = counters[2 * desc[4 * j + 2]];
    int mode = desc[4 * j + 3];
    if (mode == 2) mode = (split - pb) <= (pe - split) ? 1 : 0;
    s_begin[j] = mode ? pb : split;
    s_end[j] = mode ? split : pe;
    if (mode_out != nullptr) mode_out[j] = (uint8_t)mode;
    if (seg_out != nullptr) {
      seg_out[2 * j] = s_begin[j];
      seg_out[2 * j + 1] = s_end[j];
      seg_out[2 * (k + j)] = mode ? split : pb;
      seg_out[2 * (k + j) + 1] = mode ? pe : split;
    }
  }
  SplitSegmentsIntoTasks(s_begin, s_end, k, min_rows, target_tasks, max_tasks,
                         out_tasks);
}

__global__ __launch_bounds__(256) void ApplyKernel(
    const int64_t* __restrict__ best,
    const int32_t* __restrict__ segs,
    const int32_t* __restrict__ kn_dev,
    const int32_t* __restrict__ kp_prev_dev,
    const int64_t* __restrict__ ps_prev,
    double gamma_, const int32_t* __restrict__ cut_ptrs,
    long long min_rows, long long target_tasks, int max_ptasks,
    int32_t* __restrict__ kn_out, int32_t* __restrict__ kp_out,
    int32_t* __restrict__ feat, int32_t* __restrict__ sbin,
    uint8_t* __restrict__ dl, int32_t* __restrict__ cnt,
    BlockTask* __restrict__ out_tasks, int32_t* __restrict__ desc,
    int64_t* __restrict__ parent_ps, int32_t* __restrict__ parent_slot,
    int choice_global,
    const float* __restrict__ maxabs,
    const int8_t* __restrict__ monotone,
    double lam, double alpha, double mds,
    const double* __restrict__ bounds_prev,
    double* __restrict__ bounds_out,
    const uint8_t* __restrict__ mode_prev) {
  __shared__ int s_order[kMaxSplitNodes];
  __shared__ uint8_t s_flag[kMaxSplitNodes];
  __shared__ int s_exp[kMaxSplitNodes];
  __shared__ int s_b[kMaxSplitNodes], s_e[kMaxSplitNodes];
  __shared__ int s_kb;
  const int kn = *kn_dev;
  const int kp_prev = *kp_prev_dev;
  if (kp_prev == 0) {
    if (threadIdx.x == 0) s_order[0] = 0;
  } else {
    for (int p = threadIdx.x; p < kp_prev; p += blockDim.x) {
      const int a = p, b = kp_prev + p;
      const bool a_left = mode_prev != nullptr
                              ? (mode_prev[p] != 0)
                              : (segs[2 * a + 1] == segs[2 * b]);
      s_order[2 * p] = a_left ? a : b;
      s_order[2 * p + 1] = a_left ? b : a;
    }
  }
  __syncthreads();
  for (int i = threadIdx.x; i < kn; i += blockDim.x) {
    const int slot = s_order[i];
    s_flag[i] = DevShouldExpand(best[6 * slot + 1],
                                __longlong_as_double(best[6 * slot]), gamma_)
                    ? 1 : 0;
  }
  __syncthreads();
  if (threadIdx.x == 0) {
    int kb = 0;
    for (int i = 0; i < kn; ++i) {
      if (s_flag[i]) s_exp[kb++] = s_order[i];
    }
    s_kb = kb;
    *kp_out = kb;
    *kn_out = 2 * kb;
  }
  __syncthreads();
  const int kb = s_kb;
  for (int j = threadIdx.x; j < kb; j += blockDim.x) {
    const int e = s_exp[j];
    const int f = (int)best[6 * e + 5];
    const int sb = segs[2 * e], se = segs[2 * e + 1];
    feat[j] = f;
    sbin[j] = (int)best[6 * e + 1] - cut_ptrs[f];
    dl[j] = (uint8_t)best[6 * e + 2];
    cnt[2 * j] = sb;
    cnt[2 * j + 1] = se;
    desc[4 * j] = sb;
    desc[4 * j + 1] = se;
    desc[4 * j + 2] = j;
    const long long pgq = ps_prev[2 * e], phq = ps_prev[2 * e + 1];
    const long long lgq = best[6 * e + 3], lhq = best[6 * e + 4];
    int mode = 2;
    if (choice_global) {
      mode = (lhq <= phq - lhq) ? 1 : 0;
    }
    desc[4 * j + 3] = mode;
    parent_ps[2 * j] = pgq;
    parent_ps[2 * j + 1] = phq;
    parent_slot[j] = e;
    s_b[j] = sb;
    s_e[j] = se;
    if (bounds_out != nullptr) {
      double lo = bounds_prev ? bounds_prev[2 * e] : -INFINITY;
      double hi = bounds_prev ? bounds_prev[2 * e + 1] : INFINITY;
      double llo = lo, lhi = hi, rlo = lo, rhi = hi;
      const int c = monotone ? (int)monotone[f] : 0;
      if (c != 0) {
        const double ig = 1.0 / ScaleFromMaxAbs(maxabs[0]);
        const double ih = 1.0 / ScaleFromMaxAbs(maxabs[1]);
        double wl = CalcWeight(lgq * ig, lhq * ih, lam, alpha, mds);
        double wr = CalcWeight((pgq - lgq) * ig, (phq - lhq) * ih, lam,
                               alpha, mds);
        wl = fmin(fmax(wl, lo), hi);
        wr = fmin(fmax(wr, lo), hi);
        const double mid = (wl + wr) / 2.0;
        if (c > 0) {
          lhi = fmin(hi, mid);
          rlo = fmax(lo, mid);
        } else {
          llo = fmax(lo, mid);
          rhi = fmin(hi, mid);
        }
      }
      const bool built_left = (mode == 1);
      bounds_out[2 * j] = built_left ? llo : rlo;
      bounds_out[2 * j + 1] = built_left ? lhi : rhi;
      bounds_out[2 * (kb + j)] = built_left ? rlo : llo;
      bounds_out[2 * (kb + j) + 1] = built_left ? rhi : lhi;
    }
  }
  SplitSegmentsIntoTasks(s_b, s_e, kb, min_rows, target_tasks, max_ptasks,
                         out_tasks);
}

struct LeafSeg {
  int nid, begin, end;
  int parity;
};

typedef void (*AllreduceFn)(long long* dev_ptr, long long n_elems);

struct GrowArgs {
  DriverCtx* ctx;
  const uint8_t* gidx8;
  const uint16_t* gidx16;
  int n_features;
  const uint8_t* gidx8_col;
  const uint16_t* gidx16_col;
  long long n_rows;
  const int32_t* qgpair;
  const int32_t* cut_ptrs_dev;
  const float* cut_values_host;
  const int32_t* cut_ptrs_host;
  const int32_t* n_bins_feat_dev;
  const int32_t* feat_group_start_dev;
  const int32_t* bin_group_start_dev;
  int n_groups, max_group_bins, use_shared, n_bins;
  int32_t* ridx;
  int32_t* ridx_out;
  int64_t* hist_pool_a;
  int64_t* hist_pool_b;
  double* eval_gain;
  int32_t* eval_bin;
  uint8_t* eval_dir;
  int64_t* eval_lsum;
  int64_t* eval_best;
  int32_t* pos_out;
  int max_nodes_level;
  BlockTask* hist_tasks_dev;
  int hist_tasks_cap;
  void* wt_ws;
  long long wt_ws_bytes;
  int wt_max_ptasks;
  const int64_t* root_sums_dev;
  const float* maxabs_dev;
  double* out_scales;
  double g_scale, h_scale;
  double reg_lambda, reg_alpha, max_delta_step, min_child_weight, gamma, eta;
  int max_depth;
  const int8_t* monotone_dev;
  const int8_t* monotone_host;
  const uint8_t* fmask_dev;
  AllreduceFn allreduce;
  hipStream_t stream;

  bool has_mono() const { return monotone_host != nullptr; }
  long long hist_row() const { return (long long)n_bins * 2; }
};

struct TreeOut {
  int32_t* left;
  int32_t* right;
  int32_t* parent;
  int32_t* split_index;
  float* split_cond;
  uint8_t* default_left;
  double* loss_chg;
  float* sum_hess;
  float* base_weight;
  int n_tree_nodes;
};

struct Scales {
  double g, h, inv_g, inv_h;
  Scales(double g_scale, double h_scale)
      : g(g_scale), h(h_scale), inv_g(1.0 / g_scale), inv_h(1.0 / h_scale) {}
};

void FinishRoot(const GrowArgs& a, const int64_t* root_sums,
                const float* maxabs , const int64_t* best,
                Scales* sc, Node* root, TreeOut* out) {
  if (maxabs != nullptr) {
    *sc = Scales(ScaleFromMaxAbs(maxabs[0]), ScaleFromMaxAbs(maxabs[1]));
    if (a.out_scales != nullptr) {
      a.out_scales[0] = sc->g;
      a.out_scales[1] = sc->h;
    }
  }
  root->gq = root_sums[0];
  root->hq = root_sums[1];
  out->base_weight[0] =
      (float)CalcWeight(root->gq * sc->inv_g, root->hq * sc->inv_h,
                        a.reg_lambda, a.reg_alpha, a.max_delta_step);
  out->sum_hess[0] = (float)(root->hq * sc->inv_h);
  DecodeBest(best, root);
}

void ApplySplitHost(const GrowArgs& a, const Scales& sc, const Node& nd,
                    TreeOut* out, Node* ln, Node* rn) {
  const int l = out->n_tree_nodes, r = out->n_tree_nodes + 1;
  out->n_tree_nodes += 2;
  out->left[nd.nid] = l;
  out->right[nd.nid] = r;
  out->left[l] = out->right[l] = -1;
  out->left[r] = out->right[r] = -1;
  out->parent[l] = nd.nid;
  out->parent[r] = nd.nid;
  out->split_index[nd.nid] = nd.feature;
  out->split_cond[nd.nid] = a.cut_values_host[nd.bin];
  out->default_left[nd.nid] = (uint8_t)nd.dir;
  out->loss_chg[nd.nid] = nd.gain;
  const long long rgq = nd.gq - nd.lgq, rhq = nd.hq - nd.lhq;
  double wl = CalcWeight(nd.lgq * sc.inv_g, nd.lhq * sc.inv_h, a.reg_lambda,
                         a.reg_alpha, a.max_delta_step);
  double wr = CalcWeight(rgq * sc.inv_g, rhq * sc.inv_h, a.reg_lambda,
                         a.reg_alpha, a.max_delta_step);
  wl = std::fmin(std::fmax(wl, nd.lo), nd.hi);
  wr = std::fmin(std::fmax(wr, nd.lo), nd.hi);
  out->sum_hess[nd.nid] = (float)((nd.lhq + rhq) * sc.inv_h);
  out->base_weight[l] = (float)wl;
  out->base_weight[r] = (float)wr;
  out->sum_hess[l] = (float)(nd.lhq * sc.inv_h);
  out->sum_hess[r] = (float)(rhq * sc.inv_h);
  *ln = Node{};
  *rn = Node{};
  ln->nid = l;
  rn->nid = r;
  ln->gq = nd.lgq;
  ln->hq = nd.lhq;
  rn->gq = rgq;
  rn->hq = rhq;
  ln->seg_begin = ln->seg_end = -1;
  rn->seg_begin = rn->seg_end = -1;
  ln->lo = rn->lo = nd.lo;
  ln->hi = rn->hi = nd.hi;
  ln->gain = rn->gain = -INFINITY;
  ln->bin = rn->bin = -1;
  if (a.has_mono() && nd.feature < a.n_features) {
    const int c = a.monotone_host[nd.feature];
    if (c != 0) {
      const double mid = (wl + wr) / 2.0;
      if (c > 0) {
        ln->hi = std::fmin(nd.hi, mid);
        rn->lo = std::fmax(nd.lo, mid);
      } else {
        ln->lo = std::fmax(nd.lo, mid);
        rn->hi = std::fmin(nd.hi, mid);
      }
    }
  }
}

void ExpandLevel(const GrowArgs& a, const Scales& sc,
                 std::vector<Node>& level_nodes, int parity, TreeOut* out,
                 std::vector<LeafSeg>* leaves, std::vector<Node*>* expand,
                 std::vector<Node>* next_level) {
  expand->clear();
  for (auto& nd : level_nodes) {
    if (ShouldExpand(nd.gain, a.gamma)) {
      expand->push_back(&nd);
    } else {
      leaves->push_back({nd.nid, nd.seg_begin, nd.seg_end, parity});
    }
  }
  next_level->assign(2 * expand->size(), Node{});
  for (size_t i = 0; i < expand->size(); ++i) {
    ApplySplitHost(a, sc, *(*expand)[i], out, &(*next_level)[2 * i],
                   &(*next_level)[2 * i + 1]);
  }
}

int StageLeafDecide(const GrowArgs& a, const int32_t* cur_ridx,
                    const std::vector<Node*>& expand,
                    const std::vector<Node>& next_level) {
  const int k = (int)expand.size();
  std::vector<BlockTask> tasks;
  ChunkTasks(expand, &tasks);
  PinnedRing& ring = a.ctx->ring;
  const int slot = ring.next();
  size_t off_feat = (tasks.size() * sizeof(BlockTask) + 7) & ~7ULL;
  size_t off_sbin = (off_feat + (size_t)k * 4 + 7) & ~7ULL;
  size_t off_dl = (off_sbin + (size_t)k * 4 + 7) & ~7ULL;
  size_t off_kids = (off_dl + (size_t)k + 7) & ~7ULL;
  size_t bytes = off_kids + (size_t)k * 8;
  if (int e = ring.ensure(slot, bytes)) return e;
  char* h = (char*)ring.host[slot];
  memcpy(h, tasks.data(), tasks.size() * sizeof(BlockTask));
  int32_t* feat = (int32_t*)(h + off_feat);
  int32_t* sbin = (int32_t*)(h + off_sbin);
  uint8_t* dl = (uint8_t*)(h + off_dl);
  int32_t* kids = (int32_t*)(h + off_kids);
  for (int j = 0; j < k; ++j) {
    const Node* nd = expand[j];
    feat[j] = nd->feature;
    sbin[j] = nd->bin - a.cut_ptrs_host[nd->feature];
    dl[j] = (uint8_t)nd->dir;
    kids[2 * j] = next_level[2 * j].nid;
    kids[2 * j + 1] = next_level[2 * j + 1].nid;
  }
  HIP_CHECK(hipMemcpyAsync(ring.dev[slot], h, bytes, hipMemcpyHostToDevice,
                           a.stream));
  char* d = (char*)ring.dev[slot];
  gbt_leaf_decide(a.gidx8, a.gidx16, a.n_features, a.gidx8_col, a.gidx16_col,
                  a.n_rows, cur_ridx, (const BlockTask*)d, (int)tasks.size(),
                  (const int32_t*)(d + off_feat),
                  (const int32_t*)(d + off_sbin),
                  (const uint8_t*)(d + off_dl),
                  (const int32_t*)(d + off_kids), a.n_bins_feat_dev,
                  a.pos_out, a.stream);
  return 0;
}


struct WtArena {
  int pool;
  size_t o_best, o_seg, o_kp, o_mode, o_rs, r_total;
  size_t o_kn, o_desc, o_feat, o_sbin, o_dl, o_cnt, o_ptasks, o_pps, o_pslot;
  size_t o_ps[2], o_bnd[2];
  size_t total;

  size_t rec(int L) const { return 1 + (size_t)L * pool; }
};

WtArena MakeWtArena(int max_depth, int pool, int wt_max_ptasks,
                    bool has_mono) {
  WtArena ar{};
  ar.pool = pool;
  const size_t rec_slots = ar.rec(max_depth);
  size_t off = 0;
  auto carve = [&](size_t bytes) {
    size_t o = off;
    off = (off + bytes + 255) & ~255ULL;
    return o;
  };
  ar.o_best = carve(rec_slots * 6 * 8);
  ar.o_seg = carve(rec_slots * 2 * 4);
  ar.o_kp = carve((size_t)(max_depth + 2) * 4);
  ar.o_mode = carve((size_t)max_depth * pool);
  ar.o_rs = carve(24);
  ar.r_total = ar.o_rs + 24;
  ar.o_kn = carve((size_t)(max_depth + 2) * 4);
  ar.o_desc = carve((size_t)pool * 16);
  ar.o_feat = carve((size_t)pool * 4);
  ar.o_sbin = carve((size_t)pool * 4);
  ar.o_dl = carve((size_t)pool);
  ar.o_cnt = carve((size_t)pool * 8);
  ar.o_ptasks = carve((size_t)wt_max_ptasks * sizeof(BlockTask));
  ar.o_pps = carve((size_t)pool * 16);
  ar.o_pslot = carve((size_t)pool * 4);
  ar.o_ps[0] = carve((size_t)pool * 16);
  ar.o_ps[1] = carve((size_t)pool * 16);
  ar.o_bnd[0] = has_mono ? carve((size_t)pool * 16) : 0;
  ar.o_bnd[1] = has_mono ? carve((size_t)pool * 16) : 0;
  ar.total = off;
  return ar;
}

struct WtChain {
  WtArena ar;
  char* w;
  int n_root_tasks;
  long long root_rpt;
  int wt_max_htasks;
  int n_ptasks;
  template <typename T>
  T* at(size_t off) const { return (T*)(w + off); }
};

int EnqueueChain(const GrowArgs& a, const WtChain& c, hipStream_t cs) {
  const WtArena& ar = c.ar;
  const bool has_mono = a.has_mono();
  const int choice_global = (a.allreduce != nullptr || has_mono) ? 1 : 0;
  const long long hist_row = a.hist_row();
  const int pool = ar.pool;
  int64_t* best_rec = c.at<int64_t>(ar.o_best);
  int32_t* seg_rec = c.at<int32_t>(ar.o_seg);
  int32_t* kn_arr = c.at<int32_t>(ar.o_kn);
  int32_t* kp_arr = c.at<int32_t>(ar.o_kp);
  int32_t* d_desc = c.at<int32_t>(ar.o_desc);
  int32_t* d_feat = c.at<int32_t>(ar.o_feat);
  int32_t* d_sbin = c.at<int32_t>(ar.o_sbin);
  uint8_t* d_dl = c.at<uint8_t>(ar.o_dl);
  int32_t* d_cnt = c.at<int32_t>(ar.o_cnt);
  BlockTask* d_pt = c.at<BlockTask>(ar.o_ptasks);
  int64_t* d_pps = c.at<int64_t>(ar.o_pps);
  int32_t* d_pslot = c.at<int32_t>(ar.o_pslot);
  uint8_t* d_mode = c.at<uint8_t>(ar.o_mode);
  int64_t* ps_bufs[2] = {c.at<int64_t>(ar.o_ps[0]), c.at<int64_t>(ar.o_ps[1])};
  double* bnd_bufs[2] = {has_mono ? c.at<double>(ar.o_bnd[0]) : nullptr,
                         has_mono ? c.at<double>(ar.o_bnd[1]) : nullptr};
  const int8_t* mono = has_mono ? a.monotone_dev : nullptr;
  int32_t* cr = a.ridx;
  int32_t* alt = a.ridx_out;
  int64_t* cp = a.hist_pool_a;
  int64_t* np2 = a.hist_pool_b;
  {
    int blocks = (int)std::min<long long>((a.n_rows + 255) / 256, 4096);
    hipLaunchKernelGGL(WtInitKernel, dim3(std::max(blocks, 1)), dim3(256), 0,
                       cs, cr, a.n_rows, cp, hist_row, kn_arr, kp_arr,
                       seg_rec, a.hist_tasks_dev, c.n_root_tasks, c.root_rpt,
                       a.root_sums_dev, a.maxabs_dev,
                       c.at<int64_t>(ar.o_rs));
  }
  gbt_hist(a.gidx8, a.gidx16, a.n_features, a.qgpair, cr, a.hist_tasks_dev,
           c.n_root_tasks, cp, a.n_bins, a.feat_group_start_dev,
           a.bin_group_start_dev, a.n_groups, a.max_group_bins,
           a.cut_ptrs_dev, a.use_shared, nullptr, cs);
  if (a.allreduce) a.allreduce((long long*)cp, hist_row);
  gbt_evaluate_masked(cp, 1, a.n_bins, a.n_features, a.cut_ptrs_dev,
                      a.root_sums_dev, a.maxabs_dev, 0.0, 0.0, a.reg_lambda,
                      a.reg_alpha, a.max_delta_step, a.min_child_weight, mono,
                      nullptr, 0 , a.fmask_dev, nullptr,
                      a.eval_gain, a.eval_bin, a.eval_dir, a.eval_lsum,
                      nullptr, 0, cs);
  gbt_select_best(a.eval_gain, a.eval_bin, a.eval_dir, a.eval_lsum, 1,
                  a.n_features, best_rec, nullptr, cs);
  const int64_t* ps_prev = a.root_sums_dev;
  for (int L = 0; L + 1 < a.max_depth; ++L) {
    const size_t rec_in = L == 0 ? 0 : ar.rec(L - 1);
    const int64_t* bl = best_rec + rec_in * 6;
    const int32_t* sl = seg_rec + rec_in * 2;
    int64_t* bo = best_rec + ar.rec(L) * 6;
    int32_t* so = seg_rec + ar.rec(L) * 2;
    int64_t* ps_next = ps_bufs[L & 1];
    const int cap_kids = (int)std::min<long long>(2LL << L, (long long)pool);
    hipLaunchKernelGGL(ApplyKernel, dim3(1), dim3(256), 0, cs, bl, sl,
                       kn_arr + L, kp_arr + L, ps_prev, a.gamma,
                       a.cut_ptrs_dev, PartMinRows(), (long long)2048,
                       c.n_ptasks, kn_arr + L + 1, kp_arr + L + 1, d_feat,
                       d_sbin, d_dl, d_cnt, d_pt, d_desc, d_pps, d_pslot,
                       choice_global, a.maxabs_dev, mono, a.reg_lambda,
                       a.reg_alpha, a.max_delta_step,
                       (L == 0 || !has_mono) ? nullptr
                                             : bnd_bufs[(L - 1) & 1],
                       bnd_bufs[L & 1],
                       L == 0 ? nullptr : d_mode + (size_t)(L - 1) * pool);
    gbt_partition(a.gidx8, a.gidx16, a.n_features, a.gidx8_col, a.gidx16_col,
                  a.n_rows, cr, alt, d_pt, c.n_ptasks, d_feat, d_sbin,
                  d_dl, nullptr, nullptr, a.n_bins_feat_dev, d_cnt, cs);
    std::swap(cr, alt);
    hipLaunchKernelGGL(HistTaskGenKernel, dim3(1), dim3(256), 0, cs, d_cnt,
                       d_desc, 0, kHistMinRows, HistTasksTarget(),
                       c.wt_max_htasks, a.hist_tasks_dev, ps_next,
                       kp_arr + L + 1, so,
                       a.allreduce != nullptr ? 2 * cap_kids : 0,
                       d_mode + (size_t)L * pool);
    {
      const long long zn = (long long)cap_kids * hist_row;
      int zb = (int)std::min<long long>((zn + 255) / 256, 4096);
      hipLaunchKernelGGL(ZeroI64Kernel, dim3(zb), dim3(256), 0, cs, np2, zn);
    }
    gbt_hist(a.gidx8, a.gidx16, a.n_features, a.qgpair, cr, a.hist_tasks_dev,
             c.wt_max_htasks, np2, a.n_bins, a.feat_group_start_dev,
             a.bin_group_start_dev, a.n_groups, a.max_group_bins,
             a.cut_ptrs_dev, a.use_shared, ps_next, cs);
    if (a.allreduce) {
      a.allreduce((long long*)np2, (long long)(cap_kids / 2) * hist_row);
      a.allreduce((long long*)ps_next, (long long)cap_kids);
    }
    {
      const long long total = (long long)(cap_kids / 2 + 1) * hist_row;
      int blocks = (int)std::min<long long>((total + 255) / 256, 4096);
      hipLaunchKernelGGL(SubtractHistKernel, dim3(blocks), dim3(256), 0, cs,
                         cp, np2, np2, d_pslot, (int)hist_row, 0, ps_next,
                         d_pps, kp_arr + L + 1);
    }
    gbt_evaluate_masked(np2, cap_kids, a.n_bins, a.n_features, a.cut_ptrs_dev,
                        ps_next, a.maxabs_dev, 0.0, 0.0, a.reg_lambda,
                        a.reg_alpha, a.max_delta_step, a.min_child_weight,
                        mono, bnd_bufs[L & 1], 0 , a.fmask_dev,
                        nullptr, a.eval_gain, a.eval_bin, a.eval_dir,
                        a.eval_lsum, kn_arr + L + 1, 0, cs);
    gbt_select_best(a.eval_gain, a.eval_bin, a.eval_dir, a.eval_lsum,
                    cap_kids, a.n_features, bo, kn_arr + L + 1, cs);
    ps_prev = ps_next;
    std::swap(cp, np2);
  }
  return 0;
}

GraphKey ChainKey(const GrowArgs& a, const WtChain& c) {
  typedef unsigned long long U;
  auto db = [](double d) {
    U u;
    memcpy(&u, &d, 8);
    return u;
  };
  return {(U)a.gidx8, (U)a.gidx16, (U)a.gidx8_col, (U)a.gidx16_col,
          (U)a.qgpair, (U)a.cut_ptrs_dev, (U)a.n_bins_feat_dev,
          (U)a.feat_group_start_dev, (U)a.bin_group_start_dev, (U)a.ridx,
          (U)a.ridx_out, (U)a.hist_pool_a, (U)a.hist_pool_b, (U)a.eval_gain,
          (U)a.eval_bin, (U)a.eval_dir, (U)a.eval_lsum, (U)a.hist_tasks_dev,
          (U)a.wt_ws, (U)a.root_sums_dev, (U)a.maxabs_dev, (U)a.monotone_dev,
          (U)a.fmask_dev, (U)a.ctx->readback_host, (U)a.n_rows,
          (U)a.n_features, (U)a.n_bins, (U)a.use_shared, (U)a.n_groups,
          (U)a.max_group_bins, (U)a.max_depth, (U)a.max_nodes_level,
          (U)a.wt_max_ptasks, (U)a.hist_tasks_cap, (U)c.n_root_tasks,
          (U)c.root_rpt, (U)PartMinRows(), (U)c.n_ptasks, (U)c.wt_max_htasks,
          (U)a.has_mono(), db(a.reg_lambda), db(a.reg_alpha),
          db(a.max_delta_step), db(a.min_child_weight), db(a.gamma)};
}

int GrowWholeTree(const GrowArgs& a, TreeOut* out,
                  std::vector<LeafSeg>* leaves) {
  DriverCtx* ctx = a.ctx;
  WtChain c{};
  c.ar = MakeWtArena(a.max_depth, 2 * a.max_nodes_level, a.wt_max_ptasks,
                     a.has_mono());
  const WtArena& ar = c.ar;
  if ((long long)ar.total > a.wt_ws_bytes) return kErrArenaTooSmall;
  c.w = (char*)a.wt_ws;
  c.root_rpt = RootRowsPerTask(a.n_rows, kHistMinRows, HistTasksTarget());
  c.n_root_tasks = RootTaskCount(a.n_rows, c.root_rpt);
  if (c.n_root_tasks > a.hist_tasks_cap) return kErrRootTasksCap;
  c.wt_max_htasks = (int)std::min<long long>(
      std::min<long long>(a.n_rows / kHistMinRows, HistTasksTarget()) +
          a.max_nodes_level + 1,
      (long long)a.hist_tasks_cap);
  c.n_ptasks = (int)std::min<long long>(
      a.n_rows / PartMinRows() + ar.pool + 2, (long long)a.wt_max_ptasks);
  if (int e = ctx->ensure_readback(ar.r_total)) return e;
  char* rb = (char*)ctx->readback_host;

  bool on_gstream = false;
  if (a.allreduce == nullptr && WtGraphEnabled() &&
      ctx->ensure_gstream() == 0) {
    const GraphKey key = ChainKey(a, c);
    if (int e = ctx->wait_for(a.stream)) return e;
    on_gstream = ctx->try_replay(key);
    if (!on_gstream) {
      auto enqueue = [&](hipStream_t cs) { return EnqueueChain(a, c, cs); };
      if (int e = ctx->capture_and_launch(key, enqueue, &on_gstream)) return e;
    }
  }
  hipStream_t chain_stream = on_gstream ? ctx->gstream : a.stream;
  if (!on_gstream) {
    if (WtGraphDebug()) fprintf(stderr, "[wtgraph] direct enqueue\n");
    if (int e = EnqueueChain(a, c, a.stream)) return e;
  }
  HIP_CHECK(hipMemcpyAsync(rb, c.w + ar.o_best, ar.r_total,
                           hipMemcpyDeviceToHost, chain_stream));
  if (on_gstream) HIP_CHECK(hipStreamSynchronize(ctx->gstream));
  HIP_CHECK(hipStreamSynchronize(a.stream));

  const int64_t* h_best = (const int64_t*)(rb + ar.o_best);
  const int32_t* h_seg = (const int32_t*)(rb + ar.o_seg);
  const int32_t* h_kp = (const int32_t*)(rb + ar.o_kp);
  const uint8_t* h_mode = (const uint8_t*)(rb + ar.o_mode);
  Scales sc(a.g_scale, a.h_scale);
  Node root{};
  root.seg_end = (int)a.n_rows;
  root.lo = -INFINITY;
  root.hi = INFINITY;
  FinishRoot(a, (const int64_t*)(rb + ar.o_rs),
             (const float*)(rb + ar.o_rs + 16), h_best, &sc, &root, out);
  std::vector<Node> level_nodes{root}, next_level;
  std::vector<Node*> expand;
  for (int depth = 0; depth < a.max_depth && !level_nodes.empty(); ++depth) {
    ExpandLevel(a, sc, level_nodes, depth & 1, out, leaves, &expand,
                &next_level);
    if (expand.empty()) break;
    const int kb = (int)expand.size();
    if (depth + 1 >= a.max_depth) {
      return StageLeafDecide(a, (depth & 1) ? a.ridx_out : a.ridx, expand,
                             next_level);
    }
    if (h_kp[depth + 1] != kb) return kErrReplayDiverged;
    const int64_t* bo = h_best + ar.rec(depth) * 6;
    const int32_t* so = h_seg + ar.rec(depth) * 2;
    const uint8_t* mo = h_mode + (size_t)depth * ar.pool;
    for (int j = 0; j < kb; ++j) {
      const bool built_left = mo[j] != 0;
      Node& built = next_level[2 * j + (built_left ? 0 : 1)];
      Node& subtracted = next_level[2 * j + (built_left ? 1 : 0)];
      built.seg_begin = so[2 * j];
      built.seg_end = so[2 * j + 1];
      subtracted.seg_begin = so[2 * (kb + j)];
      subtracted.seg_end = so[2 * (kb + j) + 1];
      DecodeBest(bo + 6 * j, &built);
      DecodeBest(bo + 6 * (kb + j), &subtracted);
    }
    level_nodes.swap(next_level);
  }
  return 0;
}


int EvaluateEnqueue(const GrowArgs& a, const Scales& sc, int k,
                    const std::vector<Node*>* nodes, const int64_t* hists,
                    const int64_t* ps_dev, const float* maxabs_eval) {
  const double* bounds_dev = nullptr;
  if (ps_dev == nullptr) {
    const bool has_mono = a.has_mono();
    PinnedRing& ring = a.ctx->ring;
    const int slot = ring.next();
    size_t off_bd = ((size_t)k * 2 * sizeof(int64_t) + 7) & ~7ULL;
    size_t bytes = off_bd + (has_mono ? (size_t)k * 2 * sizeof(double) : 0);
    if (int e = ring.ensure(slot, bytes)) return e;
    char* h = (char*)ring.host[slot];
    int64_t* ps = (int64_t*)h;
    for (int i = 0; i < k; ++i) {
      ps[2 * i] = (*nodes)[i]->gq;
      ps[2 * i + 1] = (*nodes)[i]->hq;
    }
    if (has_mono) {
      double* bd = (double*)(h + off_bd);
      for (int i = 0; i < k; ++i) {
        bd[2 * i] = (*nodes)[i]->lo;
        bd[2 * i + 1] = (*nodes)[i]->hi;
      }
    }
    HIP_CHECK(hipMemcpyAsync(ring.dev[slot], h, bytes, hipMemcpyHostToDevice,
                             a.stream));
    char* d = (char*)ring.dev[slot];
    ps_dev = (const int64_t*)d;
    if (has_mono) bounds_dev = (const double*)(d + off_bd);
  }
  gbt_evaluate_masked(hists, k, a.n_bins, a.n_features, a.cut_ptrs_dev,
                      ps_dev, maxabs_eval, sc.g, sc.h, a.reg_lambda,
                      a.reg_alpha, a.max_delta_step, a.min_child_weight,
                      a.monotone_dev, bounds_dev, 0 ,
                      a.fmask_dev, nullptr, a.eval_gain, a.eval_bin,
                      a.eval_dir, a.eval_lsum, nullptr, 0, a.stream);
  gbt_select_best(a.eval_gain, a.eval_bin, a.eval_dir, a.eval_lsum, k,
                  a.n_features, a.eval_best, nullptr, a.stream);
  return 0;
}

int LevelSync(const GrowArgs& a, int n_eval, int n_expand,
              const int32_t* cnt_dev, const int64_t** best_out,
              const int32_t** cnt_out) {
  size_t off_cnt = ((size_t)n_eval * 6 * sizeof(int64_t) + 63) & ~63ULL;
  size_t bytes = off_cnt + (size_t)n_expand * 2 * sizeof(int32_t);
  if (int e = a.ctx->ensure_readback(bytes)) return e;
  char* h = (char*)a.ctx->readback_host;
  if (n_eval > 0) {
    HIP_CHECK(hipMemcpyAsync(h, a.eval_best,
                             (size_t)n_eval * 6 * sizeof(int64_t),
                             hipMemcpyDeviceToHost, a.stream));
  }
  if (n_expand > 0) {
    HIP_CHECK(hipMemcpyAsync(h + off_cnt, cnt_dev,
                             (size_t)n_expand * 2 * sizeof(int32_t),
                             hipMemcpyDeviceToHost, a.stream));
  }
  HIP_CHECK(hipStreamSynchronize(a.stream));
  *best_out = (const int64_t*)h;
  *cnt_out = (const int32_t*)(h + off_cnt);
  return 0;
}

int GrowPerLevel(const GrowArgs& a, TreeOut* out,
                 std::vector<LeafSeg>* leaves) {
  DriverCtx* ctx = a.ctx;
  PinnedRing& ring = ctx->ring;
  hipStream_t stream = a.stream;
  const long long hist_row = a.hist_row();
  const long long hist_tasks = HistTasksTarget();
  const bool has_mono = a.has_mono();
  Scales sc(a.g_scale, a.h_scale);
  {
    int blocks = (int)std::min<long long>((a.n_rows + 255) / 256, 4096);
    hipLaunchKernelGGL(IotaKernel, dim3(blocks), dim3(256), 0, stream, a.ridx,
                       a.n_rows);
  }
  int32_t* cur_ridx = a.ridx;
  int32_t* alt_ridx = a.ridx_out;
  int64_t* cur_pool = a.hist_pool_a;
  int64_t* next_pool = a.hist_pool_b;

  Node root{};
  root.seg_end = (int)a.n_rows;
  root.lo = -INFINITY;
  root.hi = INFINITY;
  {
    std::vector<Node*> nodes{&root};
    std::vector<BlockTask> tasks;
    ChunkTasks(nodes, &tasks, kHistMinRows, hist_tasks);
    const int slot = ring.next();
    size_t bytes = tasks.size() * sizeof(BlockTask);
    if (int e = ring.ensure(slot, bytes)) return e;
    memcpy(ring.host[slot], tasks.data(), bytes);
    HIP_CHECK(hipMemcpyAsync(ring.dev[slot], ring.host[slot], bytes,
                             hipMemcpyHostToDevice, stream));
    HIP_CHECK(hipMemsetAsync(a.hist_pool_a, 0, hist_row * sizeof(int64_t),
                             stream));
    gbt_hist(a.gidx8, a.gidx16, a.n_features, a.qgpair, a.ridx,
             (const BlockTask*)ring.dev[slot], (int)tasks.size(),
             a.hist_pool_a, a.n_bins, a.feat_group_start_dev,
             a.bin_group_start_dev, a.n_groups, a.max_group_bins,
             a.cut_ptrs_dev, a.use_shared, nullptr, stream);
    if (a.allreduce) a.allreduce((long long*)a.hist_pool_a, hist_row);
  }
  {
    if (int e = EvaluateEnqueue(a, sc, 1, nullptr, a.hist_pool_a,
                                a.root_sums_dev, a.maxabs_dev))
      return e;
    const int rslot = ring.next();
    if (int e = ring.ensure(rslot, 4 * sizeof(int64_t))) return e;
    char* rh = (char*)ring.host[rslot];
    HIP_CHECK(hipMemcpyAsync(rh, a.root_sums_dev, 2 * sizeof(int64_t),
                             hipMemcpyDeviceToHost, stream));
    if (a.maxabs_dev != nullptr) {
      HIP_CHECK(hipMemcpyAsync(rh + 2 * sizeof(int64_t), a.maxabs_dev,
                               2 * sizeof(float), hipMemcpyDeviceToHost,
                               stream));
    }
    const int64_t* best;
    const int32_t* cnt;
    if (int e = LevelSync(a, 1, 0, nullptr, &best, &cnt)) return e;
    FinishRoot(a, (const int64_t*)rh,
               a.maxabs_dev != nullptr
                   ? (const float*)(rh + 2 * sizeof(int64_t))
                   : nullptr,
               best, &sc, &root, out);
  }

  std::vector<Node> level_nodes{root}, next_level;
  std::vector<Node*> expand;
  for (int depth = 0; depth < a.max_depth && !level_nodes.empty(); ++depth) {
    ExpandLevel(a, sc, level_nodes, (cur_ridx == a.ridx) ? 0 : 1, out, leaves,
                &expand, &next_level);
    if (expand.empty()) {
      level_nodes.clear();
      break;
    }
    if (depth + 1 >= a.max_depth) {
      if (int e = StageLeafDecide(a, cur_ridx, expand, next_level)) return e;
      level_nodes.clear();
      break;
    }
    const int kb = (int)expand.size();
    if (2 * kb > 2 * a.max_nodes_level) return kCapacityHistPool;
    if (kb > kMaxSplitNodes) return kCapacityTaskGenLds;
    const bool dev_choice = (a.allreduce == nullptr) && !has_mono;
    std::vector<Node*> eval_nodes(2 * kb);
    std::vector<int32_t> parent_slots;
    std::vector<int32_t> desc;
    desc.reserve(4 * kb);
    for (int i = 0; i < kb; ++i) {
      Node& ln = next_level[2 * i];
      Node& rn = next_level[2 * i + 1];
      parent_slots.push_back(expand[i]->hist_slot);
      desc.push_back(expand[i]->seg_begin);
      desc.push_back(expand[i]->seg_end);
      desc.push_back(i);
      if (dev_choice) {
        desc.push_back(2);
      } else {
        Node* small = (ln.hq <= rn.hq) ? &ln : &rn;
        eval_nodes[i] = small;
        eval_nodes[kb + i] = (small == &ln) ? &rn : &ln;
        desc.push_back(small == &ln ? 1 : 0);
      }
    }

    std::vector<BlockTask> ptasks;
    ChunkTasks(expand, &ptasks);
    const int slot = ring.next();
    size_t off_feat = (ptasks.size() * sizeof(BlockTask) + 7) & ~7ULL;
    size_t off_sbin = (off_feat + (size_t)kb * 4 + 7) & ~7ULL;
    size_t off_dl = (off_sbin + (size_t)kb * 4 + 7) & ~7ULL;
    size_t off_cnt = (off_dl + (size_t)kb + 7) & ~7ULL;
    size_t off_desc = (off_cnt + (size_t)kb * 8 + 7) & ~7ULL;
    size_t off_pslots = (off_desc + desc.size() * 4 + 7) & ~7ULL;
    size_t off_pps = (off_pslots + parent_slots.size() * 4 + 63) & ~63ULL;
    size_t upload_bytes =
        off_pps + (dev_choice ? (size_t)kb * 2 * sizeof(int64_t) : 0);
    size_t off_ps = (upload_bytes + 63) & ~63ULL;
    size_t total_bytes =
        off_ps + (dev_choice ? (size_t)kb * 4 * sizeof(int64_t) : 0);
    if (int e = ring.ensure(slot, total_bytes)) return e;
    char* h = (char*)ring.host[slot];
    memcpy(h, ptasks.data(), ptasks.size() * sizeof(BlockTask));
    {
      int32_t* feat = (int32_t*)(h + off_feat);
      int32_t* sbin = (int32_t*)(h + off_sbin);
      uint8_t* dl = (uint8_t*)(h + off_dl);
      int32_t* cnt = (int32_t*)(h + off_cnt);
      for (int i = 0; i < kb; ++i) {
        Node* nd = expand[i];
        feat[i] = nd->feature;
        sbin[i] = nd->bin - a.cut_ptrs_host[nd->feature];
        dl[i] = (uint8_t)nd->dir;
        cnt[2 * i] = nd->seg_begin;
        cnt[2 * i + 1] = nd->seg_end;
      }
      memcpy(h + off_desc, desc.data(), desc.size() * 4);
      memcpy(h + off_pslots, parent_slots.data(), parent_slots.size() * 4);
      if (dev_choice) {
        int64_t* pp = (int64_t*)(h + off_pps);
        for (int i = 0; i < kb; ++i) {
          pp[2 * i] = expand[i]->gq;
          pp[2 * i + 1] = expand[i]->hq;
        }
      }
    }
    HIP_CHECK(hipMemcpyAsync(ring.dev[slot], h, upload_bytes,
                             hipMemcpyHostToDevice, stream));
    char* d = (char*)ring.dev[slot];
    int32_t* cnt_dev = (int32_t*)(d + off_cnt);
    int64_t* eval_ps = dev_choice ? (int64_t*)(d + off_ps) : nullptr;
    const int64_t* parent_ps_dev =
        dev_choice ? (const int64_t*)(d + off_pps) : nullptr;

    gbt_partition(a.gidx8, a.gidx16, a.n_features, a.gidx8_col, a.gidx16_col,
                  a.n_rows, cur_ridx, alt_ridx, (const BlockTask*)d,
                  (int)ptasks.size(), (const int32_t*)(d + off_feat),
                  (const int32_t*)(d + off_sbin),
                  (const uint8_t*)(d + off_dl), nullptr, nullptr,
                  a.n_bins_feat_dev, cnt_dev, stream);
    std::swap(cur_ridx, alt_ridx);
    long long bound_total = 0;
    for (Node* nd : expand) bound_total += nd->seg_end - nd->seg_begin;
    int max_tasks = (int)std::min<long long>(
        std::min<long long>(bound_total / kHistMinRows, hist_tasks) + kb + 1,
        a.hist_tasks_cap);
    hipLaunchKernelGGL(HistTaskGenKernel, dim3(1), dim3(256), 0, stream,
                       cnt_dev, (const int32_t*)(d + off_desc), kb,
                       kHistMinRows, hist_tasks, max_tasks, a.hist_tasks_dev,
                       eval_ps, nullptr, nullptr, 0, nullptr);
    HIP_CHECK(hipMemsetAsync(next_pool, 0,
                             (size_t)kb * hist_row * sizeof(int64_t), stream));
    gbt_hist(a.gidx8, a.gidx16, a.n_features, a.qgpair, cur_ridx,
             a.hist_tasks_dev, max_tasks, next_pool, a.n_bins,
             a.feat_group_start_dev, a.bin_group_start_dev, a.n_groups,
             a.max_group_bins, a.cut_ptrs_dev, a.use_shared, eval_ps, stream);
    if (a.allreduce) {
      a.allreduce((long long*)next_pool, (long long)kb * hist_row);
    }
    {
      int64_t* sub_out = next_pool + (long long)kb * hist_row;
      const long long total = (long long)kb * hist_row;
      int blocks = (int)std::min<long long>((total + 255) / 256, 4096);
      hipLaunchKernelGGL(SubtractHistKernel, dim3(blocks), dim3(256), 0,
                         stream, cur_pool, next_pool, sub_out,
                         (const int32_t*)(d + off_pslots), (int)hist_row, kb,
                         eval_ps, parent_ps_dev, nullptr);
    }
    if (int e = EvaluateEnqueue(a, sc, 2 * kb,
                                dev_choice ? nullptr : &eval_nodes, next_pool,
                                eval_ps, nullptr))
      return e;
    const int64_t* best;
    const int32_t* cnt;
    if (int e = LevelSync(a, 2 * kb, kb, cnt_dev, &best, &cnt)) return e;
    for (int i = 0; i < kb; ++i) {
      Node& ln = next_level[2 * i];
      Node& rn = next_level[2 * i + 1];
      ln.seg_begin = expand[i]->seg_begin;
      ln.seg_end = cnt[2 * i];
      rn.seg_begin = ln.seg_end;
      rn.seg_end = expand[i]->seg_end;
      if (dev_choice) {
        const int nl = ln.seg_end - ln.seg_begin;
        const int nr = rn.seg_end - rn.seg_begin;
        Node* small = (nl <= nr) ? &ln : &rn;
        eval_nodes[i] = small;
        eval_nodes[kb + i] = (small == &ln) ? &rn : &ln;
      }
    }
    for (int s = 0; s < 2 * kb; ++s) {
      eval_nodes[s]->hist_slot = s;
      DecodeBest(best + 6 * s, eval_nodes[s]);
    }
    level_nodes.swap(next_level);
    std::swap(cur_pool, next_pool);
  }
  const int parity = (cur_ridx == a.ridx) ? 0 : 1;
  for (auto& nd : level_nodes) {
    leaves->push_back({nd.nid, nd.seg_begin, nd.seg_end, parity});
  }
  return 0;
}

int FinishLeaves(const GrowArgs& a, const TreeOut& out,
                 const std::vector<LeafSeg>& leaves) {
  for (int nid = 0; nid < out.n_tree_nodes; ++nid) {
    if (out.left[nid] == -1) {
      out.split_cond[nid] = (float)(out.base_weight[nid] * a.eta);
    }
  }
  PinnedRing& ring = a.ctx->ring;
  for (int par = 0; par < 2; ++par) {
    std::vector<const LeafSeg*> group;
    for (const auto& lf : leaves) {
      if (lf.parity == par) group.push_back(&lf);
    }
    if (group.empty()) continue;
    std::vector<BlockTask> tasks;
    std::vector<Node> lnodes(group.size());
    std::vector<Node*> lptrs(group.size());
    for (size_t i = 0; i < group.size(); ++i) {
      lnodes[i].seg_begin = group[i]->begin;
      lnodes[i].seg_end = group[i]->end;
      lptrs[i] = &lnodes[i];
    }
    ChunkTasks(lptrs, &tasks);
    const int slot = ring.next();
    size_t off_ids = (tasks.size() * sizeof(BlockTask) + 7) & ~7ULL;
    size_t bytes = off_ids + group.size() * sizeof(int32_t);
    if (int e = ring.ensure(slot, bytes)) return e;
    char* h = (char*)ring.host[slot];
    memcpy(h, tasks.data(), tasks.size() * sizeof(BlockTask));
    int32_t* ids = (int32_t*)(h + off_ids);
    for (size_t i = 0; i < group.size(); ++i) ids[i] = group[i]->nid;
    HIP_CHECK(hipMemcpyAsync(ring.dev[slot], h, bytes, hipMemcpyHostToDevice,
                             a.stream));
    char* d = (char*)ring.dev[slot];
    gbt_leaf_partition(par == 0 ? a.ridx : a.ridx_out, (const BlockTask*)d,
                       (int)tasks.size(), (const int32_t*)(d + off_ids),
                       a.pos_out, a.stream);
  }
  return 0;
}

}

extern "C" {

void* gbt_driver_create() { return new DriverCtx(); }
void gbt_driver_destroy(void* ctx) { delete (DriverCtx*)ctx; }

int gbt_root_tasks_check(long long n_rows, long long min_rows,
                         long long target_tasks, void* stream_v) {
  hipStream_t stream = (hipStream_t)stream_v;
  Node root{};
  root.seg_end = (int)n_rows;
  std::vector<Node*> nodes{&root};
  std::vector<BlockTask> want;
  ChunkTasks(nodes, &want, min_rows, target_tasks);
  const long long rpt = RootRowsPerTask(n_rows, min_rows, target_tasks);
  const int nt = RootTaskCount(n_rows, rpt);
  const size_t o_tasks = 192;
  const size_t o_ridx = o_tasks + (size_t)nt * sizeof(BlockTask);
  const size_t bytes = o_ridx + (size_t)std::max<long long>(n_rows, 1) * 4;
  char* d = nullptr;
  HIP_CHECK(hipMalloc((void**)&d, bytes));
  int rc = 0;
  std::vector<BlockTask> got(nt);
  hipError_t e = hipMemsetAsync(d, 0, o_tasks, stream);
  if (e == hipSuccess) {
    int32_t* sc = (int32_t*)d;
    hipLaunchKernelGGL(WtInitKernel, dim3(2), dim3(256), 0, stream,
                       (int32_t*)(d + o_ridx), n_rows, (int64_t*)nullptr,
                       0LL, sc, sc + 1, sc + 2, (BlockTask*)(d + o_tasks),
                       nt, rpt, (const int64_t*)(d + 64),
                       (const float*)(d + 80), (int64_t*)(d + 128));
    e = hipMemcpyAsync(got.data(), d + o_tasks,
                       (size_t)nt * sizeof(BlockTask), hipMemcpyDeviceToHost,
                       stream);
  }
  if (e == hipSuccess) e = hipStreamSynchronize(stream);
  (void)hipFree(d);
  if (e != hipSuccess) return -(int)e;
  if (want.size() != got.size()) return (int)std::max(want.size(), got.size());
  for (size_t i = 0; i < want.size(); ++i) {
    if (want[i].out_slot != got[i].out_slot ||
        want[i].row_begin != got[i].row_begin ||
        want[i].row_end != got[i].row_end)
      ++rc;
  }
  return rc;
}

long long gbt_wt_arena_bytes(int max_depth, int max_nodes_level,
                             int wt_max_ptasks) {
  return (long long)MakeWtArena(max_depth, 2 * max_nodes_level, wt_max_ptasks,
                                true).total;
}

int gbt_grow_tree(
    void* vctx, const uint8_t* gidx8, const uint16_t* gidx16, int n_features,
    const uint8_t* gidx8_col, const uint16_t* gidx16_col,
    long long n_rows, const int32_t* qgpair, const int32_t* cut_ptrs_dev,
    const float* cut_values_host, const int32_t* cut_ptrs_host,
    const int32_t* n_bins_feat_dev, const int32_t* feat_group_start_dev,
    const int32_t* bin_group_start_dev, int n_groups, int max_group_bins,
    int use_shared, int n_bins,
    int32_t* ridx, int32_t* ridx_out, int64_t* hist_pool_a,
    int64_t* hist_pool_b, double* eval_gain, int32_t* eval_bin,
    uint8_t* eval_dir, int64_t* eval_lsum, int64_t* eval_best,
    int32_t* pos_out, int max_nodes_level,
    BlockTask* hist_tasks_dev,
    int hist_tasks_cap,
    void* wt_ws,
    long long wt_ws_bytes, int wt_max_ptasks,
    const int64_t* root_sums_dev,
    const float* maxabs_dev,
    double* out_scales,
    double g_scale, double h_scale,
    double reg_lambda, double reg_alpha, double max_delta_step,
    double min_child_weight, double gamma, double eta, int max_depth,
    const int8_t* monotone_dev, const int8_t* monotone_host,
    const uint8_t* fmask_dev,
    AllreduceFn allreduce,
    int32_t* out_left, int32_t* out_right, int32_t* out_parent,
    int32_t* out_split_index, float* out_split_cond,
    uint8_t* out_default_left,
    double* out_loss_chg,
    float* out_sum_hess,
    float* out_base_weight, void* stream_v) {
  const GrowArgs a{
      (DriverCtx*)vctx, gidx8, gidx16, n_features, gidx8_col, gidx16_col,
      n_rows, qgpair, cut_ptrs_dev, cut_values_host, cut_ptrs_host,
      n_bins_feat_dev, feat_group_start_dev, bin_group_start_dev, n_groups,
      max_group_bins, use_shared, n_bins, ridx, ridx_out, hist_pool_a,
      hist_pool_b, eval_gain, eval_bin, eval_dir, eval_lsum, eval_best,
      pos_out, max_nodes_level, hist_tasks_dev, hist_tasks_cap, wt_ws,
      wt_ws_bytes, wt_max_ptasks, root_sums_dev, maxabs_dev, out_scales,
      g_scale, h_scale, reg_lambda, reg_alpha, max_delta_step,
      min_child_weight, gamma, eta, max_depth, monotone_dev, monotone_host,
      fmask_dev, allreduce, (hipStream_t)stream_v};
  TreeOut out{out_left, out_right, out_parent, out_split_index,
              out_split_cond, out_default_left, out_loss_chg, out_sum_hess,
              out_base_weight, 1};
  out.left[0] = -1;
  out.right[0] = -1;
  out.parent[0] = -1;
  const bool whole_tree = wt_ws != nullptr && maxabs_dev != nullptr &&
                          max_nodes_level <= 1024 && max_depth >= 2 &&
                          wt_max_ptasks > 0;
  std::vector<LeafSeg> leaves;
  if (int e = whole_tree ? GrowWholeTree(a, &out, &leaves)
                         : GrowPerLevel(a, &out, &leaves))
    return e;
  if (int e = FinishLeaves(a, out, leaves)) return e;
  return out.n_tree_nodes;
}

}
```

xgboost_amd/ops/cpp/gbt_kernels.h:

```cpp
#pragma once
#include <hip/hip_runtime.h>
#include <cstdint>

struct BlockTask {
  int32_t out_slot;
  int32_t row_begin;
  int32_t row_end;
  int32_t pad;
};

extern "C" {

void gbt_hist(const uint8_t* gidx8, const uint16_t* gidx16,
              int n_features, const int32_t* qgpair ,
              const int32_t* ridx, const BlockTask* tasks, int n_tasks,
              int64_t* out_hist , int n_bins,
              const int32_t* feat_group_start,
              const int32_t* bin_group_start,
              int n_groups, int max_group_bins,
              const int32_t* cut_ptrs,
              int use_shared,
              int64_t* node_sums,
              hipStream_t stream);

void gbt_partition(const uint8_t* gidx8, const uint16_t* gidx16,
                   int n_features,
                   const uint8_t* gidx8_col,
                   const uint16_t* gidx16_col,
                   int64_t col_ld,
                   const int32_t* ridx_in, int32_t* ridx_out,
                   const BlockTask* tasks, int n_tasks,
                   const int32_t* split_feature,
                   const int32_t* split_bin_local,
                   const uint8_t* default_left,
                   const uint32_t* cat_bits,
                   const int32_t* cat_bits_offset,
                   const int32_t* n_bins_feat,
                   int32_t* counters,
                   hipStream_t stream);

void gbt_evaluate_masked(
    const int64_t* hist , int n_nodes, int n_bins,
    int n_features, const int32_t* cut_ptrs, const int64_t* parent_sums,
    const float* maxabs,
    double g_scale, double h_scale, double reg_lambda, double reg_alpha,
    double max_delta_step, double min_child_weight,
    const int8_t* monotone,
    const double* node_bounds,
    int mask_stride,
    const uint8_t* feature_mask,
    const uint8_t* cat_feature,
    double* out_gain,
    int32_t* out_bin,
    uint8_t* out_dir,
    int64_t* out_lsum,
    const int32_t* k_dev,
    int narrow_max,
    hipStream_t stream);

void gbt_evaluate_ref(const int64_t* hist, int n_nodes, int n_bins,
                      int n_features, const int32_t* cut_ptrs,
                      const int64_t* parent_sums, const float* maxabs,
                      double g_scale, double h_scale, double reg_lambda,
                      double reg_alpha, double max_delta_step,
                      double min_child_weight, const int8_t* monotone,
                      const double* node_bounds, int mask_stride,
                      const uint8_t* feature_mask,
                      const uint8_t* cat_feature, double* out_gain,
                      int32_t* out_bin, uint8_t* out_dir,
                      int64_t* out_lsum, const int32_t* k_dev,
                      int narrow_max, hipStream_t stream);

void gbt_compress(const float* X, int64_t n_rows, int n_features,
                  const float* cut_values, const int32_t* cut_ptrs,
                  const uint8_t* cat_feature, float missing_value,
                  int missing_is_nan,
                  uint8_t* out8, uint16_t* out16, hipStream_t stream);

void gbt_predict(const float* X, int64_t n_rows, int n_features,
                 float missing_value, int missing_is_nan,
                 const int32_t* tree_offsets,
                 const int32_t* left, const int32_t* right,
                 const int32_t* split_index, const float* split_cond,
                 const uint8_t* default_left, const uint8_t* split_type,
                 const int32_t* cat_offsets,
                 const uint32_t* cat_bits,
                 const int32_t* tree_group,
                 int n_trees, int n_groups,
                 float* out_margin,
                 int32_t* out_leaf,
                 hipStream_t stream);

void gbt_predict_q(const void* X, int kind, int64_t n_rows, int n_features,
                   float missing_value, int missing_is_nan,
                   const int32_t* n_bins,
                   const void* nodes,
                   const int32_t* tree_offsets,
                   const int32_t* cat_offsets,
                   const uint32_t* cat_bits,
                   const int32_t* tree_group,
                   const int32_t* vec_offset,
                   const float* leaf_vec,
                   int n_trees, int n_groups,
                   float* out_margin,
                   int32_t* out_leaf,
                   hipStream_t stream);

void gbt_predict_csr(const int64_t* indptr,
                     const int32_t* indices,
                     const float* values,
                     int64_t n_rows, int n_features, const void* nodes,
                     const int32_t* tree_offsets, const int32_t* cat_offsets,
                     const uint32_t* cat_bits, const int32_t* tree_group,
                     const int32_t* vec_offset, const float* leaf_vec,
                     int n_trees, int n_groups, float* out_margin,
                     int32_t* out_leaf, int force_search, int grid_cap,
                     hipStream_t stream);

void gbt_leaf_decide(const uint8_t* gidx8, const uint16_t* gidx16,
                     int n_features,
                     const uint8_t* gidx8_col, const uint16_t* gidx16_col,
                     int64_t col_ld,
                     const int32_t* ridx,
                     const BlockTask* tasks, int n_tasks,
                     const int32_t* split_feature,
                     const int32_t* split_bin_local,
                     const uint8_t* default_left, const int32_t* kids,
                     const int32_t* n_bins_feat, int32_t* out_pos,
                     hipStream_t stream);

void gbt_leaf_partition(const int32_t* ridx, const BlockTask* tasks,
                        int n_tasks, const int32_t* leaf_ids,
                        int32_t* out_pos, hipStream_t stream);

void gbt_copy_ranges(const int32_t* src, int32_t* dst,
                     const BlockTask* tasks, int n_tasks,
                     hipStream_t stream);

void gbt_select_best(const double* gain, const int32_t* bins,
                     const uint8_t* dirs, const int64_t* lsum, int n_nodes,
                     int n_features, int64_t* out_best,
                     const int32_t* k_dev, hipStream_t stream);

}
```

xgboost_amd/ops/cpp/gpair.hip:

```cpp
#include "gbt_kernels.h"

#include <hip/hip_runtime.h>

#include <algorithm>

namespace {

__device__ inline void AtomicMaxAbsF(float* addr, float v) {
  const unsigned int bits = __float_as_uint(fabsf(v));
  atomicMax((unsigned int*)addr, bits);
}

template <int kObj>
__global__ __launch_bounds__(256) void GpairKernel(
    const float* __restrict__ margin, const float* __restrict__ label,
    const float* __restrict__ weight, float scale_pos_weight, long long n,
    float* __restrict__ out_gh ,
    float* __restrict__ out_maxabs ) {
  __shared__ float smax_g, smax_h;
  if (threadIdx.x == 0) {
    smax_g = 0.0f;
    smax_h = 0.0f;
  }
  __syncthreads();
  float mg = 0.0f, mh = 0.0f;
  const long long i0 = (long long)blockIdx.x * blockDim.x + threadIdx.x;
  for (long long i = i0; i < n; i += (long long)gridDim.x * blockDim.x) {
    const float y = label[i];
    float g, h;
    if (kObj == 0) {
      const float p = 1.0f / (1.0f + expf(-margin[i]));
      g = p - y;
      h = fmaxf(p * (1.0f - p), 1e-16f);
      if (scale_pos_weight != 1.0f && y == 1.0f) {
        g *= scale_pos_weight;
        h *= scale_pos_weight;
      }
    } else {
      g = margin[i] - y;
      h = 1.0f;
    }
    if (weight != nullptr) {
      g *= weight[i];
      h *= weight[i];
    }
    out_gh[2 * i] = g;
    out_gh[2 * i + 1] = h;
    mg = fmaxf(mg, fabsf(g));
    mh = fmaxf(mh, fabsf(h));
  }
  for (int off = 32; off > 0; off >>= 1) {
    mg = fmaxf(mg, __shfl_down(mg, off, 64));
    mh = fmaxf(mh, __shfl_down(mh, off, 64));
  }
  if ((threadIdx.x & 63) == 0) {
    AtomicMaxAbsF(&smax_g, mg);
    AtomicMaxAbsF(&smax_h, mh);
  }
  __syncthreads();
  if (threadIdx.x == 0) {
    AtomicMaxAbsF(&out_maxabs[0], smax_g);
    AtomicMaxAbsF(&out_maxabs[1], smax_h);
  }
}

__global__ __launch_bounds__(256) void QuantizeKernel(
    const float* __restrict__ gh, long long n, double g_scale, double h_scale,
    const float* __restrict__ maxabs ,
    int32_t* __restrict__ out,
    int64_t* __restrict__ out_sums ) {
  if (maxabs != nullptr) {
    g_scale = maxabs[0] > 0.f ? 1073741824.0 / (double)maxabs[0] : 1.0;
    h_scale = maxabs[1] > 0.f ? 1073741824.0 / (double)maxabs[1] : 1.0;
  }
  long long sg = 0, sh = 0;
  const long long i0 = (long long)blockIdx.x * blockDim.x + threadIdx.x;
  for (long long i = i0; i < n; i += (long long)gridDim.x * blockDim.x) {
    const int32_t qg = (int32_t)llrint((double)gh[2 * i] * g_scale);
    const int32_t qh = (int32_t)llrint((double)gh[2 * i + 1] * h_scale);
    out[2 * i] = qg;
    out[2 * i + 1] = qh;
    sg += qg;
    sh += qh;
  }
  if (out_sums != nullptr) {
    for (int off = 32; off > 0; off >>= 1) {
      sg += __shfl_down(sg, off, 64);
      sh += __shfl_down(sh, off, 64);
    }
    __shared__ long long wg[256 / 64], wh[256 / 64];
    const int lane = (int)threadIdx.x & 63, wave = (int)threadIdx.x >> 6;
    if (lane == 0) {
      wg[wave] = sg;
      wh[wave] = sh;
    }
    __syncthreads();
    if (threadIdx.x == 0) {
      long long tg = 0, th = 0;
      for (int w = 0; w < (int)blockDim.x / 64; ++w) {
        tg += wg[w];
        th += wh[w];
      }
      if (tg) atomicAdd((unsigned long long*)&out_sums[0],
                        (unsigned long long)tg);
      if (th) atomicAdd((unsigned long long*)&out_sums[1],
                        (unsigned long long)th);
    }
  }
}

}

extern "C" {

void gbt_gpair_fused(int objective, const float* margin, const float* label,
                     const float* weight, float scale_pos_weight, long long n,
                     float* out_gh, float* out_maxabs, hipStream_t stream) {
  const int blocks = (int)std::min<long long>((n + 255) / 256, 512);
  if (objective == 0) {
    hipLaunchKernelGGL((GpairKernel<0>), dim3(blocks), dim3(256), 0, stream,
                       margin, label, weight, scale_pos_weight, n, out_gh,
                       out_maxabs);
  } else {
    hipLaunchKernelGGL((GpairKernel<1>), dim3(blocks), dim3(256), 0, stream,
                       margin, label, weight, scale_pos_weight, n, out_gh,
                       out_maxabs);
  }
}

void gbt_quantize(const float* gh, long long n, double g_scale,
                  double h_scale, const float* maxabs, int32_t* out,
                  int64_t* out_sums, hipStream_t stream) {
  const int blocks = (int)std::min<long long>((n + 255) / 256, 512);
  hipLaunchKernelGGL(QuantizeKernel, dim3(blocks), dim3(256), 0, stream, gh,
                     n, g_scale, h_scale, maxabs, out, out_sums);
}

}

namespace {

__global__ __launch_bounds__(256) void MarginAddKernel(
    float* __restrict__ margin, const int32_t* __restrict__ pos,
    const float* __restrict__ leaf_vals, long long n, int stride, int col) {
  const long long i0 = (long long)blockIdx.x * blockDim.x + threadIdx.x;
  for (long long i = i0; i < n; i += (long long)gridDim.x * blockDim.x) {
    margin[i * stride + col] += leaf_vals[pos[i]];
  }
}

}

extern "C" void gbt_margin_add(float* margin, const int32_t* pos,
                               const float* leaf_vals, long long n,
                               int stride, int col, hipStream_t stream) {
  const int blocks = (int)std::min<long long>((n + 255) / 256, 4096);
  hipLaunchKernelGGL(MarginAddKernel, dim3(blocks), dim3(256), 0, stream,
                     margin, pos, leaf_vals, n, stride, col);
}
```

Before: 1065 rounds/s.

## Fuse gradient computation and quantization into native tree-growth prologue

Moves the per-round gradient/hessian computation and quantization into the native grow-tree driver. Two kernels recompute gradients from the margin (a max-abs pass, then a fused quantize pass) with vectorized loads and per-block partials instead of global atomics. The root sums are folded into the init kernel, which removes the float gh buffer write/read, the separate memsets, and the Python-side launches. This adds complexity and a fallback path, and gradients are now computed twice per round.

```diff
diff --git a/xgboost_amd/backend/gpu.py b/xgboost_amd/backend/gpu.py
--- a/xgboost_amd/backend/gpu.py
+++ b/xgboost_amd/backend/gpu.py
@@ -498,16 +498,11 @@
             out.append(((s, mid), (mid, e)))
         return out
 
-    def grow_tree_native(self, qgpair: torch.Tensor, tree, param,
-                         quantizer, monotone: Optional[np.ndarray],
-                         root_sums: torch.Tensor,
-                         feature_mask: Optional[np.ndarray] = None):
-        import ctypes
+    def _native_workspace(self, param, n_rows: int):
         if not hasattr(self.lib, "gbt_grow_tree"):
             return None
         if param.max_depth <= 0 or param.max_depth > 14:
             return None
-        n_rows = qgpair.shape[0]
         max_build = max(1, 1 << max(param.max_depth - 2, 0))
         pool_rows = 2 * max_build
         pool_bytes = pool_rows * self.n_bins * 16
@@ -560,6 +555,27 @@
                 ws["wt_max_ptasks"] = 0
                 ws["wt_ws"] = None
             self._native_ws = ws
+        return ws
+
+    def native_prologue_ok(self, param, n_rows: int) -> bool:
+        if not hasattr(self.lib, "gbt_round_prologue"):
+            return False
+        ws = self._native_workspace(param, n_rows)
+        return ws is not None and ws["wt_ws"] is not None
+
+    def grow_tree_native(self, qgpair: Optional[torch.Tensor], tree, param,
+                         quantizer, monotone: Optional[np.ndarray],
+                         root_sums: Optional[torch.Tensor],
+                         feature_mask: Optional[np.ndarray] = None,
+                         prologue: Optional[dict] = None):
+        import ctypes
+        n_rows = (qgpair.shape[0] if prologue is None
+                  else prologue["margin"].numel())
+        ws = self._native_workspace(param, n_rows)
+        if ws is None:
+            return None
+        max_build = max(1, 1 << max(param.max_depth - 2, 0))
+        dev = self.device
         cap = 1 << (param.max_depth + 1)
         host = {name: np.zeros(cap, dt) for name, dt in [
             ("left", np.int32), ("right", np.int32), ("parent", np.int32),
@@ -612,10 +628,22 @@
         gsc = quantizer.g_scale if ma is None else 0.0
         hsc = quantizer.h_scale if ma is None else 0.0
         qg_st = ws["qg_stage"][:n_rows]
-        qg_st.copy_(qgpair.view(n_rows, 2))
-        ws["rs_stage"].copy_(root_sums.view(-1)[:2])
-        if ma is not None:
-            ws["ma_stage"].copy_(ma.view(-1)[:2])
+        if prologue is None:
+            qg_st.copy_(qgpair.view(n_rows, 2))
+            ws["rs_stage"].copy_(root_sums.view(-1)[:2])
+            if ma is not None:
+                ws["ma_stage"].copy_(ma.view(-1)[:2])
+            pro_args = (0, None, None, None, 1.0)
+        else:
+            ma = quantizer.maxabs_dev = ws["ma_stage"]
+            quantizer.root_sums_dev = ws["rs_stage"]
+            quantizer.qgpair_staged = qg_st
+            gsc = hsc = 0.0
+            pro_args = (int(prologue["objective"]),
+                        self.hip.ptr(prologue["margin"]),
+                        self.hip.ptr(prologue["label"]),
+                        self.hip.ptr(prologue["weight"]),
+                        float(prologue["scale_pos_weight"]))
         rc = self.lib.gbt_grow_tree(
             ws["driver"], p8, p16, self.qm.n_features, c8, c16, n_rows,
             self.hip.ptr(qg_st),
@@ -642,7 +670,7 @@
             gsc, hsc,
             param.reg_lambda, param.reg_alpha, param.max_delta_step,
             param.min_child_weight, param.gamma, param.eta, param.max_depth,
-            mono_dev, mono_host, fmask_ptr, cb,
+            mono_dev, mono_host, fmask_ptr, cb, *pro_args,
             *[host[k].ctypes.data_as(ctypes.c_void_p) for k in (
                 "left", "right", "parent", "split_index", "split_cond",
                 "default_left", "loss_chg", "sum_hess", "base_weight")],
diff --git a/xgboost_amd/core.py b/xgboost_amd/core.py
--- a/xgboost_amd/core.py
+++ b/xgboost_amd/core.py
@@ -527,35 +527,41 @@
             weights = (torch.as_tensor(np.ascontiguousarray(w, np.float32),
                                        device=dev) if w is not None else None)
             ent = {"labels": labels, "weights": weights,
-                   "gh": torch.empty((n, 2), dtype=torch.float32, device=dev),
-                   "qg": torch.empty((n, 2), dtype=torch.int32, device=dev),
                    "maxabs": torch.zeros(2, dtype=torch.float32, device=dev)}
             fc[key] = ent
-        ent["maxabs"].zero_()
         spw = float(self.raw_params.get("scale_pos_weight", 1.0))
-        lib.gbt_gpair_fused(
-            obj_id, hip_ops.ptr(margin.contiguous().view(-1)),
-            hip_ops.ptr(ent["labels"]), hip_ops.ptr(ent["weights"]),
-            spw, n, hip_ops.ptr(ent["gh"]), hip_ops.ptr(ent["maxabs"]),
-            hip_ops.stream())
-        m = ent["maxabs"]
-        if collective.is_distributed():
-            collective.allreduce_max_(m)
+        margin_flat = margin.contiguous().view(-1)
         quantizer = GradQuantizer.__new__(GradQuantizer)
         quantizer.g_scale = None
         quantizer.h_scale = None
-        quantizer.maxabs_dev = m
-        if "rootsum" not in ent:
-            ent["rootsum"] = torch.zeros(2, dtype=torch.int64,
-                                         device=margin.device)
-        else:
+
+        def separate_kernels() -> torch.Tensor:
+            if "gh" not in ent:
+                ent["gh"] = torch.empty((n, 2), dtype=torch.float32,
+                                        device=margin.device)
+                ent["qg"] = torch.empty((n, 2), dtype=torch.int32,
+                                        device=margin.device)
+                ent["rootsum"] = torch.empty(2, dtype=torch.int64,
+                                             device=margin.device)
+            ent["maxabs"].zero_()
+            lib.gbt_gpair_fused(
+                obj_id, hip_ops.ptr(margin_flat),
+                hip_ops.ptr(ent["labels"]), hip_ops.ptr(ent["weights"]),
+                spw, n, hip_ops.ptr(ent["gh"]), hip_ops.ptr(ent["maxabs"]),
+                hip_ops.stream())
+            m = ent["maxabs"]
+            if collective.is_distributed():
+                collective.allreduce_max_(m)
+            quantizer.maxabs_dev = m
             ent["rootsum"].zero_()
-        lib.gbt_quantize(hip_ops.ptr(ent["gh"]), n, 0.0, 0.0,
-                         hip_ops.ptr(m), hip_ops.ptr(ent["qg"]),
-                         hip_ops.ptr(ent["rootsum"]), hip_ops.stream())
-        if collective.is_distributed():
-            collective.allreduce_sum_(ent["rootsum"])
-        quantizer.root_sums_dev = ent["rootsum"]
+            lib.gbt_quantize(hip_ops.ptr(ent["gh"]), n, 0.0, 0.0,
+                             hip_ops.ptr(m), hip_ops.ptr(ent["qg"]),
+                             hip_ops.ptr(ent["rootsum"]), hip_ops.stream())
+            if collective.is_distributed():
+                collective.allreduce_sum_(ent["rootsum"])
+            quantizer.root_sums_dev = ent["rootsum"]
+            return ent["qg"]
+
         seed = (self.seed + iteration if not self.seed_per_iteration
                 else self.seed + iteration * 2654435761)
         tree = RegTree(self.n_features)
@@ -563,7 +569,17 @@
                             monotone=self._monotone_array(),
                             interaction=tp.interaction_constraints,
                             feature_weights=dtrain.info.feature_weights)
-        tree, positions = grower.grow(ent["qg"], tree)
+        if (os.environ.get("GBT_ROUND_PROLOGUE", "1") != "0"
+                and not collective.is_distributed()
+                and margin_flat.data_ptr() == margin.data_ptr()
+                and grower.prologue_ready()):
+            grower.prologue = {
+                "objective": obj_id, "margin": margin_flat,
+                "label": ent["labels"], "weight": ent["weights"],
+                "scale_pos_weight": spw, "fallback": separate_kernels}
+            tree, positions = grower.grow(None, tree)
+        else:
+            tree, positions = grower.grow(separate_kernels(), tree)
         self.trees.append(tree)
         self.tree_info.append(0)
         self.iteration_indptr.append(self.iteration_indptr[-1] + 1)
diff --git a/xgboost_amd/grower.py b/xgboost_amd/grower.py
--- a/xgboost_amd/grower.py
+++ b/xgboost_amd/grower.py
@@ -133,36 +133,59 @@
             native = self._try_native(qgpair, tree)
             if native is not None:
                 return native
+            if qgpair is None:
+                qgpair = getattr(self.quantizer, "qgpair_staged", None)
+                if qgpair is None:
+                    qgpair = self.prologue["fallback"]()
             return self._grow(qgpair, tree)
         finally:
             mon.stop("grow")
 
+    prologue: Optional[dict] = None
+
+    def _native_config_ok(self) -> bool:
+        p = self.param
+        if not hasattr(self.ops, "grow_tree_native"):
+            return False
+        if (self.cat_mask is not None or self.interaction is not None
+                or p.colsample_bylevel < 1.0 or p.colsample_bynode < 1.0):
+            return False
+        if p.grow_policy == "lossguide" or p.max_leaves > 0:
+            if p.max_depth <= 0 or p.max_depth > 14:
+                return False
+            if p.max_leaves > 0 and (1 << p.max_depth) > 16 * p.max_leaves:
+                return False
+        return True
+
+    def prologue_ready(self) -> bool:
+        return (self._native_config_ok()
+                and hasattr(self.ops, "native_prologue_ok")
+                and self.ops.native_prologue_ok(self.param, self.n_rows))
+
     def _try_native(self, qgpair, tree):
         p = self.param
         ops = self.ops
-        if not hasattr(ops, "grow_tree_native"):
-            return None
-        if (self.cat_mask is not None or self.interaction is not None
-                or p.colsample_bylevel < 1.0 or p.colsample_bynode < 1.0):
+        if not self._native_config_ok():
             return None
         fmask = None
         if p.colsample_bytree < 1.0:
             fmask = np.zeros(ops.qm.n_features, np.uint8)
             fmask[self.col_sampler.tree_set] = 1
         needs_replay = p.grow_policy == "lossguide" or p.max_leaves > 0
-        if needs_replay:
-            if p.max_depth <= 0 or p.max_depth > 14:
-                return None
-            if p.max_leaves > 0 and (1 << p.max_depth) > 16 * p.max_leaves:
-                return None
-        rs = getattr(self.quantizer, "root_sums_dev", None)
-        if rs is None:
-            from . import collective
-            rs = qgpair.to(torch.int64).sum(dim=0).contiguous()
-            if collective.is_distributed():
-                collective.allreduce_sum_(rs)
-        out = ops.grow_tree_native(qgpair, tree, p, self.quantizer,
-                                   self.monotone, rs, feature_mask=fmask)
+        if qgpair is None:
+            out = ops.grow_tree_native(None, tree, p, self.quantizer,
+                                       self.monotone, None,
+                                       feature_mask=fmask,
+                                       prologue=self.prologue)
+        else:
+            rs = getattr(self.quantizer, "root_sums_dev", None)
+            if rs is None:
+                from . import collective
+                rs = qgpair.to(torch.int64).sum(dim=0).contiguous()
+                if collective.is_distributed():
+                    collective.allreduce_sum_(rs)
+            out = ops.grow_tree_native(qgpair, tree, p, self.quantizer,
+                                       self.monotone, rs, feature_mask=fmask)
         if out is None or not needs_replay:
             return out
         dtree, pos = out
diff --git a/xgboost_amd/ops/__init__.py b/xgboost_amd/ops/__init__.py
--- a/xgboost_amd/ops/__init__.py
+++ b/xgboost_amd/ops/__init__.py
@@ -44,6 +44,8 @@
     "gbt_gpair_fused": [_i, _p, _p, _p, _f, _i64, _p, _p, _p],
     "gbt_quantize": [_p, _i64, _d, _d, _p, _p, _p, _p],
     "gbt_margin_add": [_p, _p, _p, _i64, _i, _i, _p],
+    "gbt_round_prologue": [_p, _i, _p, _p, _p, _f, _i64, _p, _p, _p, _i,
+                           _p],
     "gbt_hist_cpu": [_p, _p, _i, _p, _p, _p, _p, _i, _p, _p, _i],
     "gbt_partition_cpu": [_p, _p, _i, _p, _i64, _i64, _i, _i, _i, _p, _i,
                           _i, _p],
@@ -75,6 +77,7 @@
         _p, _p,
         _p,
         _p,
+        _i, _p, _p, _p, _f,
         _p, _p, _p, _p, _p, _p, _p, _p, _p,
         _p,
     ],
@@ -116,6 +119,8 @@
     if hasattr(_lib, "gbt_driver_create"):
         _lib.gbt_driver_create.restype = _p
         _lib.gbt_grow_tree.restype = _c.c_int
+    if hasattr(_lib, "gbt_round_prologue"):
+        _lib.gbt_round_prologue.restype = _c.c_int
     if hasattr(_lib, "gbt_root_tasks_check"):
         _lib.gbt_root_tasks_check.restype = _c.c_int
     if hasattr(_lib, "gbt_wt_arena_bytes"):
diff --git a/xgboost_amd/ops/cpp/driver.hip b/xgboost_amd/ops/cpp/driver.hip
--- a/xgboost_amd/ops/cpp/driver.hip
+++ b/xgboost_amd/ops/cpp/driver.hip
@@ -1,4 +1,5 @@
 #include "gbt_kernels.h"
+#include "prologue_partials.h"
 
 #include <hip/hip_runtime.h>
 
@@ -18,6 +19,7 @@
   } while (0)
 
 constexpr int kErrReplayDiverged = -9991;
+constexpr int kErrPrologueArgs = -9995;
 constexpr int kErrRootTasksCap = -9996;
 constexpr int kErrArenaTooSmall = -9997;
 constexpr int kCapacityTaskGenLds = -9998;
@@ -68,6 +70,13 @@
   GraphKey wt_seen_key;
   hipStream_t gstream = nullptr;
   hipEvent_t gevent = nullptr;
+
+  ProloguePartials* pro_part = nullptr;
+  int ensure_pro_part() {
+    if (pro_part != nullptr) return 0;
+    HIP_CHECK(hipMalloc((void**)&pro_part, sizeof(ProloguePartials)));
+    return 0;
+  }
 
   int ensure_gstream() {
     if (gstream == nullptr)
@@ -164,6 +173,7 @@
       if (ring.dev[i]) hipFree(ring.dev[i]);
     }
     if (readback_host) hipHostFree(readback_host);
+    if (pro_part) (void)hipFree(pro_part);
     if (wt_graph) (void)hipGraphExecDestroy(wt_graph);
     if (gstream) (void)hipStreamDestroy(gstream);
     if (gevent) (void)hipEventDestroy(gevent);
@@ -287,14 +297,18 @@
                              long long zero_n, int32_t* kn, int32_t* kp,
                              int32_t* seg, BlockTask* root_tasks,
                              int n_root_tasks, long long rpt,
-                             const int64_t* __restrict__ root_sums,
-                             const float* __restrict__ maxabs,
-                             int64_t* rs_out ) {
+                             int64_t* root_sums, float* maxabs,
+                             int64_t* rs_out ,
+                             const long long (*part_sums)[2],
+                             int n_part_sums
+                             ) {
   const long long stride = (long long)gridDim.x * blockDim.x;
   const long long i0 = (long long)blockIdx.x * blockDim.x + threadIdx.x;
   for (long long i = i0; i < n; i += stride) r[i] = (int)i;
   for (long long i = i0; i < zero_n; i += stride) zero[i] = 0;
   if (blockIdx.x != 0) return;
+  if (part_sums != nullptr)
+    PrologueSumPartials(part_sums, n_part_sums, root_sums);
   if (threadIdx.x == 0) {
     kn[0] = 1;
     kp[0] = 0;
@@ -597,8 +611,14 @@
   const int8_t* monotone_host;
   const uint8_t* fmask_dev;
   AllreduceFn allreduce;
+  int pro_objective;
+  const float* pro_margin;
+  const float* pro_label;
+  const float* pro_weight;
+  float pro_spw;
   hipStream_t stream;
 
+  bool has_prologue() const { return pro_margin != nullptr; }
   bool has_mono() const { return monotone_host != nullptr; }
   long long hist_row() const { return (long long)n_bins * 2; }
 };
@@ -812,6 +832,14 @@
   T* at(size_t off) const { return (T*)(w + off); }
 };
 
+int EnqueuePrologue(const GrowArgs& a, hipStream_t cs, bool finish) {
+  return gbt_prologue_enqueue(
+      a.pro_objective, a.pro_margin, a.pro_label, a.pro_weight, a.pro_spw,
+      a.n_rows, const_cast<int32_t*>(a.qgpair),
+      const_cast<float*>(a.maxabs_dev), a.ctx->pro_part,
+      finish ? const_cast<int64_t*>(a.root_sums_dev) : nullptr, 0, cs);
+}
+
 int EnqueueChain(const GrowArgs& a, const WtChain& c, hipStream_t cs) {
   const WtArena& ar = c.ar;
   const bool has_mono = a.has_mono();
@@ -839,13 +867,19 @@
   int32_t* alt = a.ridx_out;
   int64_t* cp = a.hist_pool_a;
   int64_t* np2 = a.hist_pool_b;
+  const bool pro = a.has_prologue();
+  const int n_part_sums = pro ? EnqueuePrologue(a, cs, false) : 0;
   {
     int blocks = (int)std::min<long long>((a.n_rows + 255) / 256, 4096);
     hipLaunchKernelGGL(WtInitKernel, dim3(std::max(blocks, 1)), dim3(256), 0,
                        cs, cr, a.n_rows, cp, hist_row, kn_arr, kp_arr,
                        seg_rec, a.hist_tasks_dev, c.n_root_tasks, c.root_rpt,
-                       a.root_sums_dev, a.maxabs_dev,
-                       c.at<int64_t>(ar.o_rs));
+                       const_cast<int64_t*>(a.root_sums_dev),
+                       const_cast<float*>(a.maxabs_dev),
+                       c.at<int64_t>(ar.o_rs),
+                       pro ? (const long long(*)[2])a.ctx->pro_part->sums
+                           : nullptr,
+                       n_part_sums);
   }
   gbt_hist(a.gidx8, a.gidx16, a.n_features, a.qgpair, cr, a.hist_tasks_dev,
            c.n_root_tasks, cp, a.n_bins, a.feat_group_start_dev,
@@ -943,7 +977,9 @@
           (U)a.wt_max_ptasks, (U)a.hist_tasks_cap, (U)c.n_root_tasks,
           (U)c.root_rpt, (U)PartMinRows(), (U)c.n_ptasks, (U)c.wt_max_htasks,
           (U)a.has_mono(), db(a.reg_lambda), db(a.reg_alpha),
-          db(a.max_delta_step), db(a.min_child_weight), db(a.gamma)};
+          db(a.max_delta_step), db(a.min_child_weight), db(a.gamma),
+          (U)a.pro_objective, (U)a.pro_margin, (U)a.pro_label,
+          (U)a.pro_weight, db((double)a.pro_spw), (U)a.ctx->pro_part};
 }
 
 int GrowWholeTree(const GrowArgs& a, TreeOut* out,
@@ -1104,6 +1140,7 @@
   const long long hist_tasks = HistTasksTarget();
   const bool has_mono = a.has_mono();
   Scales sc(a.g_scale, a.h_scale);
+  if (a.has_prologue()) EnqueuePrologue(a, stream, true);
   {
     int blocks = (int)std::min<long long>((a.n_rows + 255) / 256, 4096);
     hipLaunchKernelGGL(IotaKernel, dim3(blocks), dim3(256), 0, stream, a.ridx,
@@ -1390,8 +1427,9 @@
     hipLaunchKernelGGL(WtInitKernel, dim3(2), dim3(256), 0, stream,
                        (int32_t*)(d + o_ridx), n_rows, (int64_t*)nullptr,
                        0LL, sc, sc + 1, sc + 2, (BlockTask*)(d + o_tasks),
-                       nt, rpt, (const int64_t*)(d + 64),
-                       (const float*)(d + 80), (int64_t*)(d + 128));
+                       nt, rpt, (int64_t*)(d + 64), (float*)(d + 80),
+                       (int64_t*)(d + 128),
+                       (const long long(*)[2]) nullptr, 0);
     e = hipMemcpyAsync(got.data(), d + o_tasks,
                        (size_t)nt * sizeof(BlockTask), hipMemcpyDeviceToHost,
                        stream);
@@ -1407,6 +1445,21 @@
       ++rc;
   }
   return rc;
+}
+
+int gbt_round_prologue(void* vctx, int objective, const float* margin,
+                       const float* label, const float* weight,
+                       float scale_pos_weight, long long n, int32_t* out_qg,
+                       int64_t* out_sums, float* out_maxabs, int max_blocks,
+                       void* stream_v) {
+  DriverCtx* ctx = (DriverCtx*)vctx;
+  if (int e = ctx->ensure_pro_part()) return e;
+  (void)gbt_prologue_enqueue(objective, margin, label, weight,
+                             scale_pos_weight, n, out_qg, out_maxabs,
+                             ctx->pro_part, out_sums, max_blocks,
+                             (hipStream_t)stream_v);
+  hipError_t e = hipGetLastError();
+  return e == hipSuccess ? 0 : -(int)e;
 }
 
 long long gbt_wt_arena_bytes(int max_depth, int max_nodes_level,
@@ -1440,6 +1493,8 @@
     const int8_t* monotone_dev, const int8_t* monotone_host,
     const uint8_t* fmask_dev,
     AllreduceFn allreduce,
+    int pro_objective, const float* pro_margin, const float* pro_label,
+    const float* pro_weight, float pro_spw,
     int32_t* out_left, int32_t* out_right, int32_t* out_parent,
     int32_t* out_split_index, float* out_split_cond,
     uint8_t* out_default_left,
@@ -1456,7 +1511,8 @@
       wt_ws_bytes, wt_max_ptasks, root_sums_dev, maxabs_dev, out_scales,
       g_scale, h_scale, reg_lambda, reg_alpha, max_delta_step,
       min_child_weight, gamma, eta, max_depth, monotone_dev, monotone_host,
-      fmask_dev, allreduce, (hipStream_t)stream_v};
+      fmask_dev, allreduce, pro_objective, pro_margin, pro_label, pro_weight,
+      pro_spw, (hipStream_t)stream_v};
   TreeOut out{out_left, out_right, out_parent, out_split_index,
               out_split_cond, out_default_left, out_loss_chg, out_sum_hess,
               out_base_weight, 1};
@@ -1466,6 +1522,11 @@
   const bool whole_tree = wt_ws != nullptr && maxabs_dev != nullptr &&
                           max_nodes_level <= 1024 && max_depth >= 2 &&
                           wt_max_ptasks > 0;
+  if (a.has_prologue()) {
+    if (maxabs_dev == nullptr || root_sums_dev == nullptr || allreduce)
+      return kErrPrologueArgs;
+    if (int e = a.ctx->ensure_pro_part()) return e;
+  }
   std::vector<LeafSeg> leaves;
   if (int e = whole_tree ? GrowWholeTree(a, &out, &leaves)
                          : GrowPerLevel(a, &out, &leaves))
diff --git a/xgboost_amd/ops/cpp/gbt_kernels.h b/xgboost_amd/ops/cpp/gbt_kernels.h
--- a/xgboost_amd/ops/cpp/gbt_kernels.h
+++ b/xgboost_amd/ops/cpp/gbt_kernels.h
@@ -137,6 +137,15 @@
                      const BlockTask* tasks, int n_tasks,
                      hipStream_t stream);
 
+struct ProloguePartials;
+int gbt_prologue_enqueue(int objective, const float* margin,
+                         const float* label, const float* weight,
+                         float scale_pos_weight, long long n,
+                         int32_t* out_qg ,
+                         float* out_maxabs , ProloguePartials* part,
+                         int64_t* finish_sums ,
+                         int max_blocks, hipStream_t stream);
+
 void gbt_select_best(const double* gain, const int32_t* bins,
                      const uint8_t* dirs, const int64_t* lsum, int n_nodes,
                      int n_features, int64_t* out_best,
diff --git a/xgboost_amd/ops/cpp/gpair.hip b/xgboost_amd/ops/cpp/gpair.hip
--- a/xgboost_amd/ops/cpp/gpair.hip
+++ b/xgboost_amd/ops/cpp/gpair.hip
@@ -1,14 +1,41 @@
 #include "gbt_kernels.h"
+#include "prologue_partials.h"
 
 #include <hip/hip_runtime.h>
 
 #include <algorithm>
+#include <cstdlib>
 
 namespace {
 
 __device__ inline void AtomicMaxAbsF(float* addr, float v) {
   const unsigned int bits = __float_as_uint(fabsf(v));
   atomicMax((unsigned int*)addr, bits);
+}
+
+template <int kObj>
+__device__ __forceinline__ void RowGrad(float m, float y, float w, bool has_w,
+                                        float scale_pos_weight, float* g_out,
+                                        float* h_out) {
+  float g, h;
+  if (kObj == 0) {
+    const float p = 1.0f / (1.0f + expf(-m));
+    g = p - y;
+    h = fmaxf(p * (1.0f - p), 1e-16f);
+    if (scale_pos_weight != 1.0f && y == 1.0f) {
+      g *= scale_pos_weight;
+      h *= scale_pos_weight;
+    }
+  } else {
+    g = m - y;
+    h = 1.0f;
+  }
+  if (has_w) {
+    g *= w;
+    h *= w;
+  }
+  *g_out = g;
+  *h_out = h;
 }
 
 template <int kObj>
@@ -26,24 +53,9 @@
   float mg = 0.0f, mh = 0.0f;
   const long long i0 = (long long)blockIdx.x * blockDim.x + threadIdx.x;
   for (long long i = i0; i < n; i += (long long)gridDim.x * blockDim.x) {
-    const float y = label[i];
     float g, h;
-    if (kObj == 0) {
-      const float p = 1.0f / (1.0f + expf(-margin[i]));
-      g = p - y;
-      h = fmaxf(p * (1.0f - p), 1e-16f);
-      if (scale_pos_weight != 1.0f && y == 1.0f) {
-        g *= scale_pos_weight;
-        h *= scale_pos_weight;
-      }
-    } else {
-      g = margin[i] - y;
-      h = 1.0f;
-    }
-    if (weight != nullptr) {
-      g *= weight[i];
-      h *= weight[i];
-    }
+    RowGrad<kObj>(margin[i], label[i], weight != nullptr ? weight[i] : 1.0f,
+                  weight != nullptr, scale_pos_weight, &g, &h);
     out_gh[2 * i] = g;
     out_gh[2 * i + 1] = h;
     mg = fmaxf(mg, fabsf(g));
@@ -109,9 +121,216 @@
   }
 }
 
+
+template <int kObj>
+__device__ __forceinline__ void RowGrad4(const float* __restrict__ margin,
+                                         const float* __restrict__ label,
+                                         const float* __restrict__ weight,
+                                         float scale_pos_weight, long long i4,
+                                         float g[4], float h[4]) {
+  const float4 m = ((const float4*)margin)[i4];
+  const float4 y = ((const float4*)label)[i4];
+  float4 w = make_float4(1.0f, 1.0f, 1.0f, 1.0f);
+  if (weight != nullptr) w = ((const float4*)weight)[i4];
+  const bool hw = weight != nullptr;
+  RowGrad<kObj>(m.x, y.x, w.x, hw, scale_pos_weight, &g[0], &h[0]);
+  RowGrad<kObj>(m.y, y.y, w.y, hw, scale_pos_weight, &g[1], &h[1]);
+  RowGrad<kObj>(m.z, y.z, w.z, hw, scale_pos_weight, &g[2], &h[2]);
+  RowGrad<kObj>(m.w, y.w, w.w, hw, scale_pos_weight, &g[3], &h[3]);
+}
+
+template <int kObj>
+__global__ __launch_bounds__(256) void GradMaxAbsKernel(
+    const float* __restrict__ margin, const float* __restrict__ label,
+    const float* __restrict__ weight, float scale_pos_weight, long long n,
+    int vec, float (*__restrict__ part_maxabs)[2] ) {
+  float mg = 0.0f, mh = 0.0f;
+  const long long i0 = (long long)blockIdx.x * blockDim.x + threadIdx.x;
+  const long long stride = (long long)gridDim.x * blockDim.x;
+  const long long n4 = vec ? (n >> 2) : 0;
+  for (long long i = i0; i < n4; i += stride) {
+    float g[4], h[4];
+    RowGrad4<kObj>(margin, label, weight, scale_pos_weight, i, g, h);
+#pragma unroll
+    for (int k = 0; k < 4; ++k) {
+      mg = fmaxf(mg, fabsf(g[k]));
+      mh = fmaxf(mh, fabsf(h[k]));
+    }
+  }
+  for (long long i = 4 * n4 + i0; i < n; i += stride) {
+    float g, h;
+    RowGrad<kObj>(margin[i], label[i], weight != nullptr ? weight[i] : 1.0f,
+                  weight != nullptr, scale_pos_weight, &g, &h);
+    mg = fmaxf(mg, fabsf(g));
+    mh = fmaxf(mh, fabsf(h));
+  }
+  for (int off = 32; off > 0; off >>= 1) {
+    mg = fmaxf(mg, __shfl_down(mg, off, 64));
+    mh = fmaxf(mh, __shfl_down(mh, off, 64));
+  }
+  __shared__ float wmg[256 / 64], wmh[256 / 64];
+  if ((threadIdx.x & 63) == 0) {
+    wmg[threadIdx.x >> 6] = mg;
+    wmh[threadIdx.x >> 6] = mh;
+  }
+  __syncthreads();
+  if (threadIdx.x == 0) {
+    part_maxabs[blockIdx.x][0] =
+        fmaxf(fmaxf(wmg[0], wmg[1]), fmaxf(wmg[2], wmg[3]));
+    part_maxabs[blockIdx.x][1] =
+        fmaxf(fmaxf(wmh[0], wmh[1]), fmaxf(wmh[2], wmh[3]));
+  }
+}
+
+template <int kObj>
+__global__ __launch_bounds__(256) void GradQuantizeKernel(
+    const float* __restrict__ margin, const float* __restrict__ label,
+    const float* __restrict__ weight, float scale_pos_weight, long long n,
+    int vec, const float (*__restrict__ part_maxabs)[2], int n_part_maxabs,
+    float* __restrict__ out_maxabs ,
+    int32_t* __restrict__ out ,
+    long long (*__restrict__ part_sums)[2] ) {
+  __shared__ float wmg[256 / 64], wmh[256 / 64];
+  {
+    float mg = 0.0f, mh = 0.0f;
+    for (int i = (int)threadIdx.x; i < n_part_maxabs; i += 256) {
+      mg = fmaxf(mg, part_maxabs[i][0]);
+      mh = fmaxf(mh, part_maxabs[i][1]);
+    }
+    for (int off = 32; off > 0; off >>= 1) {
+      mg = fmaxf(mg, __shfl_down(mg, off, 64));
+      mh = fmaxf(mh, __shfl_down(mh, off, 64));
+    }
+    if ((threadIdx.x & 63) == 0) {
+      wmg[threadIdx.x >> 6] = mg;
+      wmh[threadIdx.x >> 6] = mh;
+    }
+    __syncthreads();
+  }
+  const float max_g = fmaxf(fmaxf(wmg[0], wmg[1]), fmaxf(wmg[2], wmg[3]));
+  const float max_h = fmaxf(fmaxf(wmh[0], wmh[1]), fmaxf(wmh[2], wmh[3]));
+  if (blockIdx.x == 0 && threadIdx.x == 0) {
+    out_maxabs[0] = max_g;
+    out_maxabs[1] = max_h;
+  }
+  const double g_scale = max_g > 0.f ? 1073741824.0 / (double)max_g : 1.0;
+  const double h_scale = max_h > 0.f ? 1073741824.0 / (double)max_h : 1.0;
+  long long sg = 0, sh = 0;
+  const long long i0 = (long long)blockIdx.x * blockDim.x + threadIdx.x;
+  const long long stride = (long long)gridDim.x * blockDim.x;
+  const long long n4 = vec ? (n >> 2) : 0;
+  for (long long i = i0; i < n4; i += stride) {
+    float g[4], h[4];
+    RowGrad4<kObj>(margin, label, weight, scale_pos_weight, i, g, h);
+    int32_t q[8];
+#pragma unroll
+    for (int k = 0; k < 4; ++k) {
+      q[2 * k] = (int32_t)llrint((double)g[k] * g_scale);
+      q[2 * k + 1] = (int32_t)llrint((double)h[k] * h_scale);
+      sg += q[2 * k];
+      sh += q[2 * k + 1];
+    }
+    int4* o = (int4*)out + 2 * i;
+    o[0] = make_int4(q[0], q[1], q[2], q[3]);
+    o[1] = make_int4(q[4], q[5], q[6], q[7]);
+  }
+  for (long long i = 4 * n4 + i0; i < n; i += stride) {
+    float g, h;
+    RowGrad<kObj>(margin[i], label[i], weight != nullptr ? weight[i] : 1.0f,
+                  weight != nullptr, scale_pos_weight, &g, &h);
+    const int32_t qg = (int32_t)llrint((double)g * g_scale);
+    const int32_t qh = (int32_t)llrint((double)h * h_scale);
+    out[2 * i] = qg;
+    out[2 * i + 1] = qh;
+    sg += qg;
+    sh += qh;
+  }
+  for (int off = 32; off > 0; off >>= 1) {
+    sg += __shfl_down(sg, off, 64);
+    sh += __shfl_down(sh, off, 64);
+  }
+  __shared__ long long wg[256 / 64], wh[256 / 64];
+  const int lane = (int)threadIdx.x & 63, wave = (int)threadIdx.x >> 6;
+  if (lane == 0) {
+    wg[wave] = sg;
+    wh[wave] = sh;
+  }
+  __syncthreads();
+  if (threadIdx.x == 0) {
+    part_sums[blockIdx.x][0] = wg[0] + wg[1] + wg[2] + wg[3];
+    part_sums[blockIdx.x][1] = wh[0] + wh[1] + wh[2] + wh[3];
+  }
+}
+
+__global__ __launch_bounds__(256) void PrologueFinishKernel(
+    const long long (*__restrict__ part_sums)[2], int n_part_sums,
+    int64_t* __restrict__ out_sums) {
+  PrologueSumPartials(part_sums, n_part_sums, out_sums);
+}
+
+bool Aligned16(const void* p) { return ((uintptr_t)p & 15) == 0; }
+
+int PrologueBlocksDefault() {
+  static int v = [] {
+    const char* e = getenv("GBT_PROLOGUE_BLOCKS");
+    const int b = e ? atoi(e) : kPrologueMaxBlocks;
+    return b >= 1 && b <= kPrologueMaxBlocks ? b : kPrologueMaxBlocks;
+  }();
+  return v;
+}
+int PrologueBlocks(long long items, int max_blocks) {
+  if (max_blocks <= 0) max_blocks = PrologueBlocksDefault();
+  max_blocks = std::min(max_blocks, kPrologueMaxBlocks);
+  return (int)std::max<long long>(
+      1, std::min<long long>((items + 255) / 256, max_blocks));
+}
+
+template <int kObj>
+int LaunchPrologue(const float* margin, const float* label,
+                   const float* weight, float spw, long long n,
+                   int32_t* out_qg, float* out_maxabs, ProloguePartials* part,
+                   int max_blocks, hipStream_t stream) {
+  const bool in_vec = Aligned16(margin) && Aligned16(label) &&
+                      (weight == nullptr || Aligned16(weight));
+  const int vec_a = in_vec ? 1 : 0;
+  const int vec_b = in_vec && Aligned16(out_qg) ? 1 : 0;
+  const int blocks_a =
+      PrologueBlocks(vec_a ? (n >> 2) + 3 : n, max_blocks);
+  const int blocks_b =
+      PrologueBlocks(vec_b ? (n >> 2) + 3 : n, max_blocks);
+  hipLaunchKernelGGL((GradMaxAbsKernel<kObj>), dim3(blocks_a), dim3(256), 0,
+                     stream, margin, label, weight, spw, n, vec_a,
+                     part->maxabs);
+  hipLaunchKernelGGL((GradQuantizeKernel<kObj>), dim3(blocks_b), dim3(256), 0,
+                     stream, margin, label, weight, spw, n, vec_b,
+                     (const float(*)[2])part->maxabs, blocks_a, out_maxabs,
+                     out_qg, part->sums);
+  return blocks_b;
+}
+
 }
 
 extern "C" {
+
+int gbt_prologue_enqueue(int objective, const float* margin,
+                         const float* label, const float* weight,
+                         float scale_pos_weight, long long n,
+                         int32_t* out_qg, float* out_maxabs,
+                         ProloguePartials* part, int64_t* finish_sums,
+                         int max_blocks, hipStream_t stream) {
+  const int n_part_sums =
+      objective == 0
+          ? LaunchPrologue<0>(margin, label, weight, scale_pos_weight, n,
+                              out_qg, out_maxabs, part, max_blocks, stream)
+          : LaunchPrologue<1>(margin, label, weight, scale_pos_weight, n,
+                              out_qg, out_maxabs, part, max_blocks, stream);
+  if (finish_sums != nullptr) {
+    hipLaunchKernelGGL(PrologueFinishKernel, dim3(1), dim3(256), 0, stream,
+                       (const long long(*)[2])part->sums, n_part_sums,
+                       finish_sums);
+  }
+  return n_part_sums;
+}
 
 void gbt_gpair_fused(int objective, const float* margin, const float* label,
                      const float* weight, float scale_pos_weight, long long n,
diff --git a/xgboost_amd/ops/cpp/prologue_partials.h b/xgboost_amd/ops/cpp/prologue_partials.h
--- /dev/null
+++ b/xgboost_amd/ops/cpp/prologue_partials.h
@@ -0,0 +1,33 @@
+#pragma once
+#include <hip/hip_runtime.h>
+#include <cstdint>
+
+constexpr int kPrologueMaxBlocks = 1024;
+
+struct ProloguePartials {
+  float maxabs[kPrologueMaxBlocks][2];
+  long long sums[kPrologueMaxBlocks][2];
+};
+
+__device__ inline void PrologueSumPartials(const long long (*part)[2], int n,
+                                           int64_t* out) {
+  __shared__ long long s_g[256 / 64], s_h[256 / 64];
+  long long sg = 0, sh = 0;
+  for (int i = (int)threadIdx.x; i < n; i += 256) {
+    sg += part[i][0];
+    sh += part[i][1];
+  }
+  for (int off = 32; off > 0; off >>= 1) {
+    sg += __shfl_down(sg, off, 64);
+    sh += __shfl_down(sh, off, 64);
+  }
+  if ((threadIdx.x & 63) == 0) {
+    s_g[threadIdx.x >> 6] = sg;
+    s_h[threadIdx.x >> 6] = sh;
+  }
+  __syncthreads();
+  if (threadIdx.x == 0) {
+    out[0] = s_g[0] + s_g[1] + s_g[2] + s_g[3];
+    out[1] = s_h[0] + s_h[1] + s_h[2] + s_h[3];
+  }
+}
```

New measurement: 1058 rounds/s. No clear change (-0.7%).
